# autonomousvision/LaRa

Hardware: AMD Instinct MI355X
Metric: novel-view frames/sec @512x512 (4-view in, 2DGS fwd+bwd) (higher is better)
Workload: dtype f32 raster + bf16-MFMA/f32-accumulate encoder (+ bf16-autocast coarse decoder MLP, as the reference's bf16-mixed)

## Files before the change

### include/lara_featvol.h

```cpp
#ifndef LARA_FEATVOL_H
#define LARA_FEATVOL_H

#include <stdint.h>

#ifdef __cplusplus
extern "C" {
#endif

#define LARA_FEATVOL_VOLUME 0
#define LARA_FEATVOL_TOKENS 1
#define LARA_FEATVOL_MAX_C 1024
#define LARA_FEATVOL_MAX_HW 8192

typedef struct {
    int32_t B, V, C, E, h, w, R;
    int32_t img_w, img_h;
    float eps;
    int64_t x_stride[4];
} lara_featvol_dims;

int64_t lara_featvol_workspace_bytes(const lara_featvol_dims *d);

int lara_featvol_forward(const lara_featvol_dims *d, const float *img_feats, const float *rays, const float *w2cs, const float *ixts,
                         const float *grid, const float *ln_w, const float *ln_b, const float *mlp_w, const float *mlp_b,
                         const float *view_embed, int32_t layout, void *out, void *workspace, void *stream);

int lara_featvol_backward(const lara_featvol_dims *d, const float *img_feats, const float *rays, const float *w2cs, const float *ixts,
                          const float *grid, const float *ln_w, const float *ln_b, const float *mlp_w, const float *mlp_b,
                          const float *grad, int32_t grad_layout, float *dx, float *d_ln_w, float *d_ln_b, float *d_mlp_w,
                          float *d_mlp_b, float *d_view_embed, void *workspace, void *stream);

#ifdef __cplusplus
}
#endif
#endif
```

### include/lara_groupattn.h

```cpp
#ifndef LARA_GROUPATTN_H
#define LARA_GROUPATTN_H

#include <stdint.h>

#ifdef __cplusplus
extern "C" {
#endif

int64_t lara_groupattn_workspace_bytes(int32_t G);

int lara_groupattn_forward(int32_t G, int32_t cond_dim, const float *x, const uint16_t *cond_bf16,
                           const float *ln_weight, const float *ln_bias, float eps,
                           const uint16_t *wq, const uint16_t *wkv, const uint16_t *wo, float *y,
                           void *workspace, void *stream);


typedef struct lara_groupblock_weights {
    const float *ln1_w, *ln1_b;
    const uint16_t *wq, *wkv, *wo;
    const float *ln2_w, *ln2_b;
    const uint16_t *w1;
    const float *b1;
    const uint16_t *w2;
    const float *b2;
    const float *ln3_w, *ln3_b;
    const uint16_t *wconv;
    float eps;
} lara_groupblock_weights;

int64_t lara_groupblock_workspace_bytes(int32_t scenes, int32_t R);

int lara_groupblock_forward(int32_t scenes, int32_t R, int32_t cond_dim, float *x,
                            const uint16_t *cond_bf16, const lara_groupblock_weights *w,
                            void *workspace, void *stream);

int lara_voltrans_head_forward(int32_t scenes, int32_t R, const float *x, const float *ln_w,
                               const float *ln_b, float eps, const uint16_t *wdeconv,
                               const float *bias, int32_t Cout, float *out, void *workspace,
                               void *stream);

int lara_tokens_from_volume(int32_t scenes, int32_t R, int32_t C, const float *volume, float *tokens,
                            void *stream);
int lara_volume_from_tokens(int32_t scenes, int32_t R, int32_t C, const float *tokens, float *volume,
                            void *stream);

int lara_gemm_nt_bf16(int32_t M, int32_t N, int32_t K, const uint16_t *A, const uint16_t *W, void *C, int32_t c_fp32,
                      void *stream);

int lara_batched_transpose(int32_t batch, int32_t rows, int32_t cols, const float *src, void *dst, int32_t dst_bf16,
                           void *stream);


typedef struct lara_groupblock_weights_t {
    const uint16_t *wq_t;
    const uint16_t *wkv_t;
    const uint16_t *wo_t;
    const uint16_t *w1_t;
    const uint16_t *w2_t;
    const uint16_t *wconv_t;
} lara_groupblock_weights_t;

typedef struct lara_groupblock_grads {
    float *ln1_w, *ln1_b, *wq, *wkv, *wo, *ln2_w, *ln2_b, *w1, *b1, *w2, *b2, *ln3_w, *ln3_b, *wconv;
} lara_groupblock_grads;

int64_t lara_groupblock_backward_workspace_bytes(int32_t scenes, int32_t R);
int64_t lara_groupblock_save_bytes(int32_t scenes, int32_t R);

int lara_groupblock_forward_train(int32_t scenes, int32_t R, int32_t cond_dim, const float *x_in, float *x_out,
                                  const uint16_t *cond_bf16, const lara_groupblock_weights *w, void *saved,
                                  void *stream);

int lara_groupblock_backward(int32_t scenes, int32_t R, int32_t cond_dim, const float *x_in,
                             const uint16_t *cond_bf16, const lara_groupblock_weights *w,
                             const lara_groupblock_weights_t *wt, const void *saved, float *g, float *dcond,
                             const lara_groupblock_grads *dw, int32_t chained, uint16_t *dkv, int32_t lddkv,
                             void *workspace, void *stream);

int64_t lara_voltrans_head_backward_workspace_bytes(int32_t scenes, int32_t R, int32_t Cout);
int lara_voltrans_head_backward(int32_t scenes, int32_t R, const float *x, const float *ln_w, const float *ln_b,
                                float eps, const uint16_t *wdeconv_t, int32_t Cout, const float *dout, float *g,
                                float *d_ln_w, float *d_ln_b, float *d_wdeconv, float *d_bias8, void *workspace,
                                void *stream);

int lara_groupblock_save_offsets(int32_t scenes, int32_t R, int64_t *offsets, int32_t n);
int64_t lara_gemm_tn_workspace_bytes(void);
int lara_gemm_tn_bf16(int32_t M, int32_t N, int32_t Kc, const uint16_t *A, const uint16_t *B, float *dst,
                      void *workspace, void *stream);
int lara_layernorm256_backward(int32_t rows, const float *dy, const float *x, const float *gamma, float eps,
                               const float *skip, float *dx, float *dgamma, float *dbeta, void *workspace,
                               void *stream);
int lara_groupattn_core_backward(int32_t G, const uint16_t *q, const uint16_t *kv, const uint16_t *d_o, uint16_t *dq,
                                 uint16_t *dkv, void *stream);

#ifdef __cplusplus
}
#endif
#endif
```

### lara_amd/_native.py

```python
from __future__ import annotations

import contextlib
import ctypes
import os
import re

import torch

_HERE = os.path.dirname(os.path.abspath(__file__))
LIB_PATH = os.environ.get("LARA2DGS_LIB") or os.path.join(_HERE, "liblara2dgs.so")
ABI_VERSION = 10

_vp, _i32, _i64, _f32 = ctypes.c_void_p, ctypes.c_int32, ctypes.c_int64, ctypes.c_float


def _struct(name, *groups):
    return type(name, (ctypes.Structure,), {"_fields_": [(n, t) for t, names in groups for n in names.split()]})


_BLOCK_FIELDS = "ln1_w ln1_b wq wkv wo ln2_w ln2_b w1 b1 w2 b2 ln3_w ln3_b wconv"

View = _struct("View", (_i32, "P sh_degree sh_coeffs image_height image_width"), (_f32, "tanfovx tanfovy scale_modifier"),
               (_i32, "prefiltered debug forward_only"), (_i64, "capacity"), (_vp, "bg viewmatrix projmatrix campos counts_out"))
StateLayout = _struct("StateLayout", (_i64, "header geom cullbox point_list ranges tile_order pair_base pair_pos final_T n_contrib "
                                            "seg_base seg_cnt bwd_order bwd_items ckpt pair_mask tile_maxc seg_cost total"))
Subset = _struct("Subset", (_vp, "coarse_state"), (_i64, "coarse_state_stride coarse_capacity"),
                 (_i32, "coarse_P coarse_forward_only"), (_vp, "inv"))
GradLayout = _struct("GradLayout", (_i64, "means3D means2D shs colors opacities scales rotations transmat total"))
FeatvolDims = _struct("FeatvolDims", (_i32, "B V C E h w R img_w img_h"), (_f32, "eps"), (_i64 * 4, "x_stride"))
BlockWeights = _struct("BlockWeights", (_vp, _BLOCK_FIELDS), (_f32, "eps"))
BlockWeightsT = _struct("BlockWeightsT", (_vp, "wq_t wkv_t wo_t w1_t w2_t wconv_t"))
BlockGrads = _struct("BlockGrads", (_vp, _BLOCK_FIELDS))
ImageView = _struct("ImageView", (_vp, "p"), (_i64, "sN sC sY sV sX"), (_i32, "Wv"))
LPIPS_MAX_LAYERS, LPIPS_TAPS = 16, 5
LpipsLayer = _struct("LpipsLayer", (_vp, "w bias"), (_i32, "cin cout k stride pad pool_k pool_s tap"))
LpipsNet = _struct("LpipsNet", (_i32, "n_layers"), (LpipsLayer * LPIPS_MAX_LAYERS, "layers"), (_vp * LPIPS_TAPS, "lin"),
                   (_f32 * 3, "shift"), (_f32 * 3, "scale"))
RowsItem = _struct("RowsItem", (_vp, "src dst"), (_i32, "width"))
VitDims = _struct("VitDims", (_i32, "N views H W C heads F depth"), (_f32, "eps"), (_i64 * 5, "img_stride"))

STRUCTS = {"lara2dgs_view": View, "lara2dgs_state_layout": StateLayout, "lara2dgs_subset": Subset,
           "lara2dgs_grad_layout": GradLayout, "lara_featvol_dims": FeatvolDims, "lara_groupblock_weights": BlockWeights,
           "lara_groupblock_weights_t": BlockWeightsT, "lara_groupblock_grads": BlockGrads, "lara_image_view": ImageView,
           "lara_lpips_layer": LpipsLayer, "lara_lpips_net": LpipsNet, "lara_rows_item": RowsItem, "lara_vit_dims": VitDims}

SIGNATURES = """
# include/lara2dgs.h
i lara2dgs_abi_version()
z lara2dgs_error_string(i)
i lara2dgs_last_hip_error()
l lara2dgs_state_bytes(i*3 l i)
l lara2dgs_scratch_bytes(i*3 l i)
i lara2dgs_get_state_layout(i*3 l i StateLayout)
i lara2dgs_forward(View p*12 s)
i lara2dgs_backward(View p*19 s)
i lara2dgs_forward_views(i View p*11 l p l s)
i lara2dgs_forward_views_subset(i View p*11 l p l Subset s)
i lara2dgs_get_grad_layout(i*6 GradLayout)
i lara2dgs_backward_views(i View p*10 l p l p s)
i lara2dgs_mark_visible(i p*4 s)
i lara2dgs_profile_enable(i)
i lara2dgs_selftest(i p p s)
i lara2dgs_profile_collect(p i p i)
# include/lara_batchfinish.h
i lara_batch_finish(p*4 l*4 p*3 s)
i lara_batch_finish_host(p*4 l*4 p*3)
# include/lara_coarsedec.h
l lara_coarse_decoder_padded_rows(l)
i lara_coarse_decoder_forward(i*3 p*7 f f p*5 s)
i lara_coarse_decoder_backward(i*3 p*19 s)
# include/lara_depthsurface.h
l lara_depthsurface_backproject_workspace_bytes(i*3)
i lara_depthsurface_backproject_count(i*3 p p i i f p p s)
i lara_depthsurface_backproject_emit(i*3 p p i i f p p i p f p*4 s)
l lara_depthsurface_thin_workspace_bytes(i i)
i lara_depthsurface_thin(i p p f i p*5 s)
i lara_depthsurface_observe(i p i*3 p p i f p p f i p s)
l lara_depthsurface_reduce_workspace_bytes(i)
i lara_depthsurface_reduce(i i p*5 i p*3 s)
# include/lara_eval.h
l lara_eval_workspace_doubles(i*6)
i lara_eval_scores(i*3 ImageView ImageView p i*3 p*3 i i p*3 s)
i lara_eval_quantize_frames(i*3 l l p*5 s)
# include/lara_featvol.h
l lara_featvol_workspace_bytes(FeatvolDims)
i lara_featvol_forward(FeatvolDims p*10 i p p s)
i lara_featvol_backward(FeatvolDims p*10 i p*7 s)
# include/lara_finedec.h
i lara_fine_decoder_forward(i p*8 s)
i lara_fine_decoder_backward(i p*14 s)
i lara_fine_wgrad_floats()
l lara_fine_wgrad_workspace_bytes(i)
i lara_fine_decoder_wgrad(i p*8 s)
i lara_fine_ln_blocks(i)
i lara_fine_ln_forward(i p*3 f p p s)
i lara_fine_ln_backward(i p*6 s)
# include/lara_groupattn.h
l lara_groupattn_workspace_bytes(i)
i lara_groupattn_forward(i i p*4 f p*5 s)
l lara_groupblock_workspace_bytes(i i)
i lara_groupblock_forward(i*3 p p BlockWeights p s)
i lara_voltrans_head_forward(i i p*3 f p p i p p s)
i lara_tokens_from_volume(i*3 p p s)
i lara_volume_from_tokens(i*3 p p s)
i lara_gemm_nt_bf16(i*3 p*3 i s)
i lara_batched_transpose(i*3 p p i s)
l lara_groupblock_backward_workspace_bytes(i i)
l lara_groupblock_save_bytes(i i)
i lara_groupblock_forward_train(i*3 p*3 BlockWeights p s)
i lara_groupblock_backward(i*3 p p BlockWeights BlockWeightsT p*3 BlockGrads i p i p s)
l lara_voltrans_head_backward_workspace_bytes(i*3)
i lara_voltrans_head_backward(i i p*3 f p i p*7 s)
i lara_groupblock_save_offsets(i i p i)
# ... 314 lines not shown
```

### lara_amd/csrc/attention.hip

```cpp
#include "mfma_gemm.h"
#include "group_attn.h"
#include "../../include/lara_groupattn.h"

extern "C" {

int64_t lara_groupattn_workspace_bytes(int32_t G) {
    if (G < 0) return LARA2DGS_E_INVALID;
    return (int64_t)G * (8 * 256 * 3 + 4 * 512) * 2 + 1024 + 262144;
}

int lara_groupattn_forward(int32_t G, int32_t cond_dim, const float *x, const uint16_t *cond_bf16,
                           const float *ln_weight, const float *ln_bias, float eps,
                           const uint16_t *wq, const uint16_t *wkv, const uint16_t *wo, float *y,
                           void *workspace, void *stream) {
    if (G < 0 || cond_dim <= 0 || (cond_dim % 32) != 0) return LARA2DGS_E_INVALID;
    if (G == 0) return LARA2DGS_OK;
    if (!x || !cond_bf16 || !ln_weight || !ln_bias || !wq || !wkv || !wo || !y || !workspace)
        return LARA2DGS_E_INVALID;
    hipStream_t s = (hipStream_t)stream;
    unsigned short *kvf = (unsigned short *)((char *)workspace + 262144) + (size_t)G * 8 * 256 * 2;
    {
        L2D_PROF("ga_gemm_kv", s);
        GemmP p{};
        p.A = cond_bf16; p.W = wkv; p.C = kvf; p.M = G * 4; p.N = 512; p.K = cond_dim;
        L2D_HIP(launch_gemm_ring<0, 0>(p, s));
    }
    {
        L2D_PROF("ga_fused", s);
        const int units = (G + 3) / 4;
        unsigned short *wqp = (unsigned short *)workspace, *wop = wqp + 65536;
        L2D_LAUNCH_IN_SCOPE(s, pack_weight_frag_kernel, dim3(64), dim3(256), 0, wq, wqp, wo, wop);
        L2D_LAUNCH_IN_SCOPE(s, group_attn_fused2_kernel<false>, dim3(units), dim3(64), 0, x, ln_weight, ln_bias, eps, wqp, kvf, wop, y, G,
                            (unsigned short *)nullptr, (unsigned short *)nullptr, (unsigned short *)nullptr);
    }
    return LARA2DGS_OK;
}

}
```

### lara_amd/csrc/encoder.hip

```cpp
#include <cstdlib>

#include "mfma_gemm.h"
#include "mlp_fused.h"
#include "../../include/lara_groupattn.h"

namespace {

__global__ void __launch_bounds__(256)
tokens_volume_kernel(const int R, const int C, const float *__restrict__ src, float *__restrict__ dst,
                     const int M, const int to_tokens) {
    const size_t i = (size_t)blockIdx.x * 256 + threadIdx.x;
    if (i >= (size_t)M * C) return;
    const int m = (int)(i / C), c = (int)(i - (size_t)m * C);
    int b, d, h, w;
    token_to_voxel(m, R, b, d, h, w);
    const size_t v = ((((size_t)b * C + c) * R + d) * R + h) * R + w;
    if (to_tokens) dst[i] = src[v];
    else dst[v] = src[i];
}

template <bool BF16>
__global__ void __launch_bounds__(256)
batched_transpose_kernel(const float *__restrict__ src, void *__restrict__ dst, const int rows, const int cols) {
    __shared__ float t[64][65];
    const int tx = threadIdx.x & 63, ty = threadIdx.x >> 6;
    const int c0 = blockIdx.x * 64, r0 = blockIdx.y * 64;
    const size_t base = (size_t)blockIdx.z * rows * cols;
#pragma unroll 4
    for (int k = 0; k < 16; k++) {
        const int r = r0 + ty * 16 + k, c = c0 + tx;
        t[ty * 16 + k][tx] = (r < rows && c < cols) ? src[base + (size_t)r * cols + c] : 0.f;
    }
    __syncthreads();
#pragma unroll 4
    for (int k = 0; k < 16; k++) {
        const int c = c0 + ty * 16 + k, r = r0 + tx;
        if (c < cols && r < rows) {
            const float v = t[tx][ty * 16 + k];
            if (BF16) ((unsigned short *)dst)[base + (size_t)c * rows + r] = f2bf(v);
            else ((float *)dst)[base + (size_t)c * rows + r] = v;
        }
    }
}

}

extern "C" {

int lara_batched_transpose(int32_t batch, int32_t rows, int32_t cols, const float *src, void *dst, int32_t dst_bf16,
                           void *stream) {
    if (batch < 0 || rows < 0 || cols < 0 || batch > 65535 || (rows + 63) / 64 > 65535) return LARA2DGS_E_INVALID;
    if (batch == 0 || rows == 0 || cols == 0) return LARA2DGS_OK;
    if (!src || !dst) return LARA2DGS_E_INVALID;
    const dim3 grid((cols + 63) / 64, (rows + 63) / 64, batch);
    if (dst_bf16) L2D_LAUNCH_IN_SCOPE((hipStream_t)stream, batched_transpose_kernel<true>, grid, dim3(256), 0, src, dst, rows, cols);
    else L2D_LAUNCH_IN_SCOPE((hipStream_t)stream, batched_transpose_kernel<false>, grid, dim3(256), 0, src, dst, rows, cols);
    return LARA2DGS_OK;
}

int64_t lara_groupblock_workspace_bytes(int32_t scenes, int32_t R) {
    if (scenes < 0 || R <= 0 || (R & 1)) return LARA2DGS_E_INVALID;
    const int64_t M = (int64_t)scenes * R * R * R;
    return M * 256 * 2 * 4 + M * 8 + 512 + 1024 + 262144;
}

int lara_groupblock_forward(int32_t scenes, int32_t R, int32_t cond_dim, float *x,
                            const uint16_t *cond_bf16, const lara_groupblock_weights *w,
                            void *workspace, void *stream) {
    if (scenes < 0 || R <= 0 || (R & 1) || cond_dim <= 0 || (cond_dim % 32) != 0 || !w) return LARA2DGS_E_INVALID;
    if (scenes == 0) return LARA2DGS_OK;
    if (!x || !cond_bf16 || !workspace || !w->ln1_w || !w->ln1_b || !w->wq || !w->wkv || !w->wo || !w->ln2_w ||
        !w->ln2_b || !w->w1 || !w->b1 || !w->w2 || !w->b2 || !w->ln3_w || !w->ln3_b || !w->wconv)
        return LARA2DGS_E_INVALID;
    const int64_t M64 = (int64_t)scenes * R * R * R;
    if (M64 * 2056 + 512 >= (1ll << 32)) return LARA2DGS_E_INVALID;
    const int M = (int)M64, G = M / 8;
    hipStream_t s = (hipStream_t)stream;
    int rc = lara_groupattn_forward(G, cond_dim, x, cond_bf16, w->ln1_w, w->ln1_b, w->eps, w->wq, w->wkv, w->wo,
                                    x, workspace, stream);
    if (rc) return rc;
    unsigned short *xn = (unsigned short *)workspace;
    float2 *stats = (float2 *)((char *)workspace + (size_t)M * 256 * 2 * 4);
    char *zero_row = (char *)xn + (size_t)M * 512;
    {
        L2D_PROF("gb_mlp_fused", s);
        MlpP p{};
        p.x1 = x; p.x2 = x; p.ln2_w = w->ln2_w; p.ln2_b = w->ln2_b; p.b1 = w->b1; p.b2 = w->b2; p.ln3_w = w->ln3_w; p.ln3_b = w->ln3_b;
        p.w1 = w->w1; p.w2 = w->w2; p.xn3 = xn; p.stats = stats; p.eps = w->eps; p.M = M;
        L2D_HIP(launch_mlp_fused<0>(p, s));
    }
    {
        L2D_PROF("gb_conv3d", s);
        GemmP p{};
        p.A = xn; p.W = w->wconv; p.C = x; p.resid = x; p.M = M; p.N = 256; p.K = 27 * 256;
        p.R = R; p.Cin = 256; p.stats = stats; p.gamma = w->ln3_w; p.beta = w->ln3_b;
        p.zero_off = (uint32_t)(zero_row - (char *)xn);
        L2D_HIP(launch_gemm_ring<1, 4>(p, s));
    }
    return LARA2DGS_OK;
}

int lara_voltrans_head_forward(int32_t scenes, int32_t R, const float *x, const float *ln_w,
                               const float *ln_b, float eps, const uint16_t *wdeconv,
                               const float *bias, int32_t Cout, float *out, void *workspace,
                               void *stream) {
    if (scenes < 0 || R <= 0 || (R & 1) || Cout <= 0 || (Cout & 3)) return LARA2DGS_E_INVALID;
    if (scenes == 0) return LARA2DGS_OK;
    if (!x || !ln_w || !ln_b || !wdeconv || !bias || !out || !workspace) return LARA2DGS_E_INVALID;
    const int M = scenes * R * R * R;
    hipStream_t s = (hipStream_t)stream;
    unsigned short *xn = (unsigned short *)workspace;
    L2D_LAUNCH("vt_ln", s, ln_cast_kernel, dim3((M + 3) / 4), dim3(256), 0, x, ln_w, ln_b, eps, xn,
               (float2 *)nullptr, M);
    {
        L2D_PROF("vt_deconv", s);
        GemmP p{};
        p.A = xn; p.W = wdeconv; p.C = out; p.bias = bias; p.M = M; p.N = 8 * Cout; p.K = 256;
        p.R = R; p.Cout = Cout;
        L2D_LAUNCH_IN_SCOPE(s, (gemm_bf16_nt_kernel<0, 5>), dim3((M + 127) / 128, (8 * Cout + 127) / 128), dim3(256), 0, p);
    }
    return LARA2DGS_OK;
}

static int tokens_volume(int32_t scenes, int32_t R, int32_t C, const float *src, float *dst, void *stream,
                         int to_tokens) {
    if (scenes < 0 || R <= 0 || (R & 1) || C <= 0) return LARA2DGS_E_INVALID;
    if (scenes == 0) return LARA2DGS_OK;
    if (!src || !dst) return LARA2DGS_E_INVALID;
    const int M = scenes * R * R * R;
    const size_t n = (size_t)M * C;
    L2D_LAUNCH_IN_SCOPE((hipStream_t)stream, tokens_volume_kernel, dim3((unsigned)((n + 255) / 256)), dim3(256), 0, R, C,
                        src, dst, M, to_tokens);
    return LARA2DGS_OK;
}

int lara_tokens_from_volume(int32_t scenes, int32_t R, int32_t C, const float *volume, float *tokens,
                            void *stream) {
    return tokens_volume(scenes, R, C, volume, tokens, stream, 1);
}

int lara_volume_from_tokens(int32_t scenes, int32_t R, int32_t C, const float *tokens, float *volume,
                            void *stream) {
    return tokens_volume(scenes, R, C, tokens, volume, stream, 0);
}

}
```

### lara_amd/csrc/encoder_bwd.hip

```cpp
#include <cstdlib>

#include "mfma_gemm.h"
#include "mlp_fused.h"
#include "group_attn.h"
#include "../../include/lara_groupattn.h"

namespace {

struct TnP {
    const unsigned short *A, *B;
    float *part;
    const int *nbr;
    int M, lda, ldb, N, Kc, T, chunk, tiles;
};
constexpr int TN_GROUP_MAX = 6;
struct TnGroup {
    TnP p[TN_GROUP_MAX];
    int first_slot[TN_GROUP_MAX + 1];
    int count;
};

__device__ __forceinline__ bf16x8 pack_lo(const uint32_t *w) {
    union { uint32_t u[4]; bf16x8 v; } r;
#pragma unroll
// ... 660 lines not shown
        for (int o = 32; o > 0; o >>= 1) s += __shfl_xor(s, o, 64);
        const float mean = s * (1.0f / 256.0f);
        const float c0 = v.x - mean, c1 = v.y - mean, c2 = v.z - mean, c3 = v.w - mean;
        float q = c0 * c0 + c1 * c1 + c2 * c2 + c3 * c3;
#pragma unroll
        for (int o = 32; o > 0; o >>= 1) q += __shfl_xor(q, o, 64);
        const float rstd = 1.0f / sqrtf(q * (1.0f / 256.0f) + eps);
        const float h0 = c0 * rstd, h1 = c1 * rstd, h2 = c2 * rstd, h3 = c3 * rstd;
        const float a0 = d.x * g.x, a1 = d.y * g.y, a2 = d.z * g.z, a3 = d.w * g.w;
        float sa = a0 + a1 + a2 + a3, sh = a0 * h0 + a1 * h1 + a2 * h2 + a3 * h3;
#pragma unroll
        for (int o = 32; o > 0; o >>= 1) { sa += __shfl_xor(sa, o, 64); sh += __shfl_xor(sh, o, 64); }
        sa *= (1.0f / 256.0f); sh *= (1.0f / 256.0f);
        const float4 r = make_float4(rstd * (a0 - sa - h0 * sh) + k.x, rstd * (a1 - sa - h1 * sh) + k.y,
                                     rstd * (a2 - sa - h2 * sh) + k.z, rstd * (a3 - sa - h3 * sh) + k.w);
        ((float4 *)(dx_out + (size_t)tok * 256))[lane] = r;
        if (dx_bf16) {
            ushort4 hb;
            hb.x = f2bf(r.x); hb.y = f2bf(r.y); hb.z = f2bf(r.z); hb.w = f2bf(r.w);
            ((ushort4 *)(dx_bf16 + (size_t)tok * 256))[lane] = hb;
        }
        pg[0] += d.x * h0; pg[1] += d.y * h1; pg[2] += d.z * h2; pg[3] += d.w * h3;
        pb[0] += d.x; pb[1] += d.y; pb[2] += d.z; pb[3] += d.w;
        po[0] += r.x; po[1] += r.y; po[2] += r.z; po[3] += r.w;
    }
#pragma unroll
    for (int c = 0; c < 4; c++) { red[wave][c][lane] = pg[c]; red[wave][4 + c][lane] = pb[c]; red[wave][8 + c][lane] = po[c]; }
    __syncthreads();
    if (wave == 0) {
#pragma unroll
        for (int k = 0; k < 12; k++) {
            const float t = (red[0][k][lane] + red[1][k][lane]) + (red[2][k][lane] + red[3][k][lane]);
            part[(size_t)blockIdx.x * 768 + (k >> 2) * 256 + 4 * lane + (k & 3)] = t;
        }
    }
}

__global__ void __launch_bounds__(256)
colsum_bf16_kernel(const unsigned short *__restrict__ src, float *__restrict__ part, const int rows, const int C) {
    const int r0 = blockIdx.x * 64, r1 = min(rows, r0 + 64);
    for (int c2 = threadIdx.x; c2 < C / 2; c2 += 256) {
        float s0 = 0.f, s1 = 0.f;
        for (int rr = r0; rr < r1; rr++) {
            const uint32_t w = *(const uint32_t *)(src + (size_t)rr * C + 2 * c2);
            s0 += __uint_as_float(w << 16);
            s1 += __uint_as_float(w & 0xffff0000u);
        }
        part[(size_t)blockIdx.x * C + 2 * c2] = s0;
        part[(size_t)blockIdx.x * C + 2 * c2 + 1] = s1;
    }
}

__global__ void __launch_bounds__(256)
cast_bf16_kernel(const float *__restrict__ src, unsigned short *__restrict__ dst, const size_t n4) {
    const size_t i = (size_t)blockIdx.x * 256 + threadIdx.x;
    if (i >= n4) return;
    const float4 v = ((const float4 *)src)[i];
    ushort4 h;
    h.x = f2bf(v.x); h.y = f2bf(v.y); h.z = f2bf(v.z); h.w = f2bf(v.w);
    ((ushort4 *)dst)[i] = h;
}

__global__ void __launch_bounds__(256)
deconv_grad_gather_kernel(const float *__restrict__ dout, unsigned short *__restrict__ dog, const int M, const int R,
                          const int Cout) {
    const int c4n = 2 * Cout;
    const size_t i = (size_t)blockIdx.x * 256 + threadIdx.x;
    if (i >= (size_t)M * c4n) return;
    const int m = (int)(i / c4n), c = (int)(i - (size_t)m * c4n) * 4;
    const int tap = c / Cout, co = c - tap * Cout;
    int b, d, h, w;
    token_to_voxel(m, R, b, d, h, w);
    const size_t R2 = 2 * (size_t)R;
    const size_t o = ((((size_t)b * R2 + 2 * d + (tap >> 2)) * R2 + 2 * h + ((tap >> 1) & 1)) * R2 + 2 * w + (tap & 1)) * Cout + co;
    const float4 v = *(const float4 *)(dout + o);
    ushort4 hb;
    hb.x = f2bf(v.x); hb.y = f2bf(v.y); hb.z = f2bf(v.z); hb.w = f2bf(v.w);
    *(ushort4 *)(dog + (size_t)m * 8 * Cout + c) = hb;
}

__global__ void __launch_bounds__(256)
group_attn_bwd_kernel(const unsigned short *__restrict__ Q, const unsigned short *__restrict__ KV,
                      const unsigned short *__restrict__ dO, unsigned short *__restrict__ dQ,
                      unsigned short *__restrict__ dKV, const int G, const int lddkv ) {
    __shared__ __attribute__((aligned(16))) unsigned short s_q[2][8 * 256], s_do[2][8 * 256], s_kv[2][4 * 512], s_dq[2][8 * 256];
    __shared__ float s_p[2][16 * 8 * 4], s_ds[2][16 * 8 * 4];
    const int gl = threadIdx.x >> 7, t = threadIdx.x & 127;
    const int g = blockIdx.x * 2 + gl;
    const bool active = g < G;
    if (active) {
        const uint4 *gq = (const uint4 *)(Q + (size_t)g * 8 * 256), *gd = (const uint4 *)(dO + (size_t)g * 8 * 256);
        const uint4 *gk = (const uint4 *)(KV + (size_t)g * 4 * 512);
        ((uint4 *)s_q[gl])[t] = gq[t]; ((uint4 *)s_q[gl])[t + 128] = gq[t + 128];
        ((uint4 *)s_do[gl])[t] = gd[t]; ((uint4 *)s_do[gl])[t + 128] = gd[t + 128];
        ((uint4 *)s_kv[gl])[t] = gk[t]; ((uint4 *)s_kv[gl])[t + 128] = gk[t + 128];
    }
    __syncthreads();
    if (active) {
        const int h = t >> 3, i = t & 7;
        float qv[16], dv[16];
#pragma unroll
        for (int d = 0; d < 16; d++) { qv[d] = bf2f(s_q[gl][i * 256 + h * 16 + d]); dv[d] = bf2f(s_do[gl][i * 256 + h * 16 + d]); }
        float sc[4], dp[4];
#pragma unroll
        for (int j = 0; j < 4; j++) {
            float a = 0.f, b = 0.f;
#pragma unroll
            for (int d = 0; d < 16; d++) {
                a += qv[d] * bf2f(s_kv[gl][j * 512 + h * 16 + d]);
                b += dv[d] * bf2f(s_kv[gl][j * 512 + 256 + h * 16 + d]);
            }
            sc[j] = a * 0.25f; dp[j] = b;
        }
        const float mx = fmaxf(fmaxf(sc[0], sc[1]), fmaxf(sc[2], sc[3]));
        float pr[4], sum = 0.f;
#pragma unroll
        for (int j = 0; j < 4; j++) { pr[j] = __expf(sc[j] - mx); sum += pr[j]; }
        const float inv = 1.0f / sum;
        float dot = 0.f;
#pragma unroll
        for (int j = 0; j < 4; j++) { pr[j] *= inv; dot += pr[j] * dp[j]; }
        float ds[4];
#pragma unroll
        for (int j = 0; j < 4; j++) {
            ds[j] = pr[j] * (dp[j] - dot) * 0.25f;
            s_p[gl][(h * 8 + i) * 4 + j] = pr[j];
            s_ds[gl][(h * 8 + i) * 4 + j] = ds[j];
        }
#pragma unroll
        for (int d = 0; d < 16; d++) {
            float a = 0.f;
#pragma unroll
            for (int j = 0; j < 4; j++) a += ds[j] * bf2f(s_kv[gl][j * 512 + h * 16 + d]);
            s_dq[gl][i * 256 + h * 16 + d] = f2bf(a);
        }
    }
    __syncthreads();
    float dk[8], dvv[8];
    const int h2 = t >> 3, j2 = (t >> 1) & 3, d0 = (t & 1) * 8;
    if (active) {
#pragma unroll
        for (int d = 0; d < 8; d++) { dk[d] = 0.f; dvv[d] = 0.f; }
#pragma unroll
        for (int i = 0; i < 8; i++) {
            const float dsv = s_ds[gl][(h2 * 8 + i) * 4 + j2], pv = s_p[gl][(h2 * 8 + i) * 4 + j2];
#pragma unroll
            for (int d = 0; d < 8; d++) {
                dk[d] += dsv * bf2f(s_q[gl][i * 256 + h2 * 16 + d0 + d]);
                dvv[d] += pv * bf2f(s_do[gl][i * 256 + h2 * 16 + d0 + d]);
            }
        }
    }
    __syncthreads();
    if (active) {
#pragma unroll
        for (int d = 0; d < 8; d++) {
            s_kv[gl][j2 * 512 + h2 * 16 + d0 + d] = f2bf(dk[d]);
            s_kv[gl][j2 * 512 + 256 + h2 * 16 + d0 + d] = f2bf(dvv[d]);
        }
    }
    __syncthreads();
    if (active) {
        uint4 *oq = (uint4 *)(dQ + (size_t)g * 8 * 256);
        unsigned short *ok = dKV + ((size_t)g * 4 + (t >> 6)) * lddkv + (t & 63) * 8;
        oq[t] = ((const uint4 *)s_dq[gl])[t]; oq[t + 128] = ((const uint4 *)s_dq[gl])[t + 128];
        *(uint4 *)ok = ((const uint4 *)s_kv[gl])[t]; *(uint4 *)(ok + 2 * (size_t)lddkv) = ((const uint4 *)s_kv[gl])[t + 128];
    }
}

constexpr size_t TN_PART_BYTES = 128ull << 20;

inline int cu_count() {
    static const int cus = [] {
        int dev = 0, v = 0;
        if (hipGetDevice(&dev) != hipSuccess || hipDeviceGetAttribute(&v, hipDeviceAttributeMultiprocessorCount, dev) != hipSuccess) v = 0;
        return v > 0 ? v : 256;
    }();
    return cus;
// ... 131 lines not shown
    AccGroup a{};
    g.count = a.count = count;
    size_t off_f = 0;
    for (;;) {
        off_f = 0;
        int slot = 0, wg = 0;
        for (int k = 0; k < count; k++) {
            const TnJob &j = jobs[k];
            int splits = base;
            while (splits > 8 && j.M / splits < 256) splits -= 8;
            const int tiles = ((j.N + 127) / 128) * ((j.Kc + 127) / 128), n = j.N * j.Kc;
            TnP &p = g.p[k];
            p.A = j.A; p.B = j.B; p.part = part + off_f; p.nbr = nullptr; p.M = j.M; p.lda = j.lda; p.ldb = j.ldb; p.N = j.N; p.Kc = j.Kc;
            p.T = 1; p.chunk = (((j.M + splits - 1) / splits) + 63) & ~63; p.tiles = tiles;
            g.first_slot[k] = slot;
            slot += tiles * splits / 8;
            a.dst[k] = j.dst; a.part[k] = part + off_f; a.n[k] = n; a.parts[k] = splits; a.first_wg[k] = wg;
            wg += (n / 4 + 63) / 64;
            off_f += (size_t)splits * n;
        }
        g.first_slot[count] = slot;
        a.first_wg[count] = wg;
        if (off_f * 4 <= TN_PART_BYTES || base == 8) break;
        base -= 8;
    }
    if (off_f * 4 > TN_PART_BYTES) return LARA2DGS_E_INVALID;
    L2D_LAUNCH_IN_SCOPE(s, (gemm_bf16_tn_lds_kernel<false>), dim3(g.first_slot[count] * 8), dim3(256), 0, g);
    L2D_LAUNCH_IN_SCOPE(s, accum_partials4_group_kernel, dim3(a.first_wg[count]), dim3(256), 0, a);
    return LARA2DGS_OK;
}

struct RedList {
    RedGroup g{};
    int wgs = 0;
    bool overflow = false;
    void add(float *dst, const float *part, int n, int parts, int stride) {
        if (!dst) return;
        if (g.count >= RED_GROUP_MAX) { overflow = true; return; }
        const int k = g.count++;
        g.dst[k] = dst; g.part[k] = part; g.n[k] = n; g.parts[k] = parts; g.stride[k] = stride; g.first_wg[k] = wgs;
        wgs += (n + 63) / 64;
        g.first_wg[g.count] = wgs;
    }
    int launch(hipStream_t s) {
        if (overflow) return LARA2DGS_E_INVALID;
        if (g.count) L2D_LAUNCH_IN_SCOPE(s, reduce_group_kernel, dim3(wgs), dim3(1024), 0, g);
        g.count = 0; wgs = 0;
        return LARA2DGS_OK;
    }
};

int ln_bwd(const void *dy, bool dy_bf16, const float *x, const float *gamma, float eps, const float *skip, float *dx,
           unsigned short *dx_bf16, float *dgamma, float *dbeta, float *part, int M, hipStream_t s, RedList *later = nullptr) {
    const int blocks = (M + LNB_ROWS - 1) / LNB_ROWS;
    if (dy_bf16) L2D_LAUNCH_IN_SCOPE(s, ln_bwd_kernel<true>, dim3(blocks), dim3(256), 0, dy, x, gamma, eps, skip, dx, dx_bf16, part, M);
    else L2D_LAUNCH_IN_SCOPE(s, ln_bwd_kernel<false>, dim3(blocks), dim3(256), 0, dy, x, gamma, eps, skip, dx, dx_bf16, part, M);
    if (later) {
        later->add(dgamma, part, 256, blocks, 768);
        later->add(dbeta, part + 256, 256, blocks, 768);
    } else {
        L2D_LAUNCH_IN_SCOPE(s, accum_ln_partials_kernel, dim3(4, 3), dim3(1024), 0, dgamma, dbeta, (float *)nullptr, part, blocks);
    }
    return LARA2DGS_OK;
}

int colsum_bf16(const unsigned short *src, int rows, int C, float *dst, float *part, hipStream_t s) {
    const int blocks = (rows + 63) / 64;
    L2D_LAUNCH_IN_SCOPE(s, colsum_bf16_kernel, dim3(blocks), dim3(256), 0, src, part, rows, C);
    L2D_LAUNCH_IN_SCOPE(s, accum_partials_kernel, dim3((C + 63) / 64), dim3(1024), 0, dst, part, C, blocks, (size_t)C);
    return LARA2DGS_OK;
}

template <int EPI>
int gemm_nt(const unsigned short *A, const unsigned short *W, void *C, int M, int N, int K, const float *resid, hipStream_t s) {
    GemmP p{};
    p.A = A; p.W = W; p.C = C; p.resid = resid; p.M = M; p.N = N; p.K = K;
    L2D_LAUNCH_IN_SCOPE(s, (gemm_bf16_nt_kernel<0, EPI>), dim3((M + 127) / 128, (N + 127) / 128), dim3(256), 0, p);
    return LARA2DGS_OK;
}

struct SaveWs {
    size_t xn1, q, kv, o, x1, xn2, z, h, x2, xn3, stats, wpack, total;
};
SaveWs save_layout(int64_t M) {
    SaveWs w{};
    size_t o = 0;
    auto take = [&](size_t bytes) { const size_t at = o; o = up256(o + bytes); return at; };
    const size_t b256 = (size_t)M * 512, f256 = (size_t)M * 1024, b512 = (size_t)M * 1024;
    w.xn1 = take(b256); w.q = take(b256); w.kv = take(b256); w.o = take(b256);
    w.x1 = take(f256); w.xn2 = take(b256); w.z = take(b512); w.h = take(b512); w.x2 = take(f256);
    w.xn3 = take(b256 + 512);
    w.stats = take((size_t)M * 8);
    w.wpack = take(2 * 256 * 256 * 2);
    w.total = o;
    return w;
}
struct BwdWs {
    size_t gb, tmpf, dzb, dq, dkv, dob, nbr, tnpart, save, gb3, gb2, lnpart4, total;
};
BwdWs bwd_layout(int64_t M) {
    BwdWs w{};
    size_t o = 0;
    auto take = [&](size_t bytes) { const size_t at = o; o = up256(o + bytes); return at; };
    const size_t b256 = (size_t)M * 512, f256 = (size_t)M * 1024, b512 = (size_t)M * 1024;
    w.gb = take(b256 + 512);
    w.tmpf = take(f256); w.dzb = take(b512); w.dq = take(b256); w.dkv = take(b256); w.dob = take(b256);
    w.nbr = take((size_t)27 * M * 4);
    take(((size_t)(M + 63) / 64) * 768 * 4);
    w.tnpart = take(TN_PART_BYTES);
    w.save = take(save_layout(M).total);
    w.gb3 = take(b256); w.gb2 = take(b256);
    w.lnpart4 = take(4 * ((size_t)(M + LNB_ROWS - 1) / LNB_ROWS) * 768 * 4);
    w.total = o;
    return w;
}

int block_forward_keep(int M, int cond_dim, const float *x_in, const unsigned short *cond_bf16,
                       const lara_groupblock_weights *w, char *save, hipStream_t s) {
    const SaveWs L = save_layout(M);
    const int G = M / 8, Mkv = G * 4;
    unsigned short *xn1 = (unsigned short *)(save + L.xn1), *q = (unsigned short *)(save + L.q), *kv = (unsigned short *)(save + L.kv);
    unsigned short *o = (unsigned short *)(save + L.o), *xn2 = (unsigned short *)(save + L.xn2), *z = (unsigned short *)(save + L.z);
    unsigned short *h = (unsigned short *)(save + L.h), *xn3 = (unsigned short *)(save + L.xn3);
    float *x1 = (float *)(save + L.x1), *x2 = (float *)(save + L.x2);
    {
        GemmP p{};
        p.A = cond_bf16; p.W = w->wkv; p.C = kv; p.M = Mkv; p.N = 512; p.K = cond_dim;
        L2D_HIP(launch_gemm_ring<0, 0>(p, s));
    }
    {
        unsigned short *wqp = (unsigned short *)(save + L.wpack), *wop = wqp + 65536;
        L2D_LAUNCH_IN_SCOPE(s, pack_weight_frag_kernel, dim3(64), dim3(256), 0, w->wq, wqp, w->wo, wop);
        L2D_LAUNCH_IN_SCOPE(s, group_attn_fused2_kernel<true>, dim3((G + 3) / 4), dim3(64), 0, x_in, w->ln1_w, w->ln1_b, w->eps, wqp, kv, wop,
                            x1, G, xn1, q, o);
    }
    {
        MlpP p{};
        p.x1 = x1; p.x2 = x2; p.ln2_w = w->ln2_w; p.ln2_b = w->ln2_b; p.b1 = w->b1; p.b2 = w->b2; p.ln3_w = w->ln3_w; p.ln3_b = w->ln3_b;
        p.w1 = w->w1; p.w2 = w->w2; p.xn3 = xn3; p.stats = (float2 *)(save + L.stats); p.xn2 = xn2; p.z = z; p.h = h; p.eps = w->eps; p.M = M;
        L2D_HIP(launch_mlp_fused<1>(p, s));
    }
    return LARA2DGS_OK;
}

bool block_weights_ok(const lara_groupblock_weights *w) {
    return w && w->ln1_w && w->ln1_b && w->wq && w->wkv && w->wo && w->ln2_w && w->ln2_b && w->w1 && w->b1 && w->w2 &&
           w->b2 && w->ln3_w && w->ln3_b && w->wconv;
}

}

extern "C" {

int64_t lara_groupblock_backward_workspace_bytes(int32_t scenes, int32_t R) {
    if (scenes < 0 || R < 4 || (R & 1)) return LARA2DGS_E_INVALID;
    return (int64_t)bwd_layout((int64_t)scenes * R * R * R).total;
}

int64_t lara_groupblock_save_bytes(int32_t scenes, int32_t R) {
    if (scenes < 0 || R < 4 || (R & 1)) return LARA2DGS_E_INVALID;
    return (int64_t)save_layout((int64_t)scenes * R * R * R).total;
}

int lara_groupblock_save_offsets(int32_t scenes, int32_t R, int64_t *offsets, int32_t n) {
    if (scenes < 0 || R < 4 || (R & 1) || !offsets || n != 11) return LARA2DGS_E_INVALID;
    const SaveWs L = save_layout((int64_t)scenes * R * R * R);
    const size_t at[11] = {L.xn1, L.q, L.kv, L.o, L.x1, L.xn2, L.z, L.h, L.x2, L.xn3, L.stats};
    for (int i = 0; i < 11; i++) offsets[i] = (int64_t)at[i];
    return LARA2DGS_OK;
}

int lara_groupblock_forward_train(int32_t scenes, int32_t R, int32_t cond_dim, const float *x_in, float *x_out,
                                  const uint16_t *cond_bf16, const lara_groupblock_weights *w, void *saved,
                                  void *stream) {
    if (scenes < 0 || R < 4 || (R & 1) || cond_dim <= 0 || (cond_dim % 32) != 0 || !block_weights_ok(w)) return LARA2DGS_E_INVALID;
    if (scenes == 0) return LARA2DGS_OK;
    if (!x_in || !x_out || x_in == x_out || !cond_bf16 || !saved) return LARA2DGS_E_INVALID;
    const int64_t M64 = (int64_t)scenes * R * R * R;
    if (M64 * 2056 + 512 >= (1ll << 32)) return LARA2DGS_E_INVALID;
    const int M = (int)M64;
    hipStream_t s = (hipStream_t)stream;
    const SaveWs L = save_layout(M);
    char *save = (char *)saved;
    {
        L2D_PROF("gbt_forward", s);
        L2D_TRY(block_forward_keep(M, cond_dim, x_in, cond_bf16, w, save, s));
    }
    {
        L2D_PROF("gb_conv3d", s);
        GemmP p{};
        p.A = (const unsigned short *)(save + L.xn3); p.W = w->wconv; p.C = x_out; p.resid = (const float *)(save + L.x2);
        p.M = M; p.N = 256; p.K = 27 * 256; p.R = R; p.Cin = 256; p.stats = (const float2 *)(save + L.stats);
        p.gamma = w->ln3_w; p.beta = w->ln3_b; p.zero_off = (uint32_t)((size_t)M * 512);
        L2D_HIP(launch_gemm_ring<1, 4>(p, s));
    }
    return LARA2DGS_OK;
}

int lara_groupblock_backward(int32_t scenes, int32_t R, int32_t cond_dim, const float *x_in,
                             const uint16_t *cond_bf16, const lara_groupblock_weights *w,
                             const lara_groupblock_weights_t *wt, const void *saved, float *g, float *dcond,
                             const lara_groupblock_grads *dw, int32_t chained, uint16_t *dkv_ext, int32_t lddkv,
                             void *workspace, void *stream) {
    if (scenes < 0 || R < 4 || (R & 1) || cond_dim <= 0 || (cond_dim % 32) != 0 || !block_weights_ok(w) || !wt || !dw)
        return LARA2DGS_E_INVALID;
    if (scenes == 0) return LARA2DGS_OK;
    if (!x_in || !cond_bf16 || !g || (!dcond && !dkv_ext) || !workspace) return LARA2DGS_E_INVALID;
    if (dkv_ext && (lddkv < 512 || (lddkv & 7))) return LARA2DGS_E_INVALID;
    constexpr int CONV_CIN = 256, CONV_K = 27 * CONV_CIN;
    static_assert(CONV_K % 128 == 0 && CONV_CIN % 128 == 0, "gemm_ring2_kernel's shapes (launch_gemm_ring has nothing else for a convolution)");
    if (!wt->wq_t || !wt->wkv_t || !wt->wo_t || !wt->w1_t || !wt->w2_t ||
        !wt->wconv_t || !dw->ln1_w || !dw->ln1_b || !dw->wq || !dw->wkv || !dw->wo || !dw->ln2_w || !dw->ln2_b ||
        !dw->w1 || !dw->b1 || !dw->w2 || !dw->b2 || !dw->ln3_w || !dw->ln3_b || !dw->wconv)
        return LARA2DGS_E_INVALID;
    const int64_t M64 = (int64_t)scenes * R * R * R;
    if (M64 * 2056 + 512 >= (1ll << 32)) return LARA2DGS_E_INVALID;
    const int M = (int)M64, G = M / 8, Mkv = G * 4;
    hipStream_t s = (hipStream_t)stream;
    const BwdWs L = bwd_layout(M);
    const SaveWs S = save_layout(M);
    char *ws = (char *)workspace;
    if (!saved) {
        L2D_PROF("gbb_recompute", s);
        L2D_TRY(block_forward_keep(M, cond_dim, x_in, cond_bf16, w, ws + L.save, s));
    }
    const char *sv = saved ? (const char *)saved : ws + L.save;
    const unsigned short *xn1 = (const unsigned short *)(sv + S.xn1), *q = (const unsigned short *)(sv + S.q);
    const unsigned short *kv = (const unsigned short *)(sv + S.kv), *o = (const unsigned short *)(sv + S.o);
    const unsigned short *xn2 = (const unsigned short *)(sv + S.xn2), *h = (const unsigned short *)(sv + S.h);
    const unsigned short *xn3 = (const unsigned short *)(sv + S.xn3);
    unsigned short *z = (unsigned short *)(sv + S.z);
    const float *x1 = (const float *)(sv + S.x1), *x2 = (const float *)(sv + S.x2);
    unsigned short *gb = (unsigned short *)(ws + L.gb);
    unsigned short *gb3 = (unsigned short *)(ws + L.gb3), *gb2 = (unsigned short *)(ws + L.gb2);
    unsigned short *dzb = (unsigned short *)(ws + L.dzb), *dq = (unsigned short *)(ws + L.dq);
    unsigned short *dkv = dkv_ext ? dkv_ext : (unsigned short *)(ws + L.dkv);
    const int ld_dkv = dkv_ext ? lddkv : 512;
    unsigned short *dob = (unsigned short *)(ws + L.dob);
    unsigned short *tmpb = (unsigned short *)(ws + L.tmpf);
    float *tnpart = (float *)(ws + L.tnpart);
    const size_t lnset = ((size_t)(M + LNB_ROWS - 1) / LNB_ROWS) * 768;
    float *lnp4 = (float *)(ws + L.lnpart4);
    RedList red;
    int *nbr = (int *)(ws + L.nbr);
    if (!chained) {
        L2D_HIP(hipMemsetAsync(gb + (size_t)M * 256, 0, 512, s));
        L2D_LAUNCH_IN_SCOPE(s, neighbour_table_kernel, dim3((M + 255) / 256), dim3(256), 0, nbr, M, R, M, 512);
        L2D_LAUNCH_IN_SCOPE(s, cast_bf16_kernel, dim3((unsigned)(((size_t)M * 64 + 255) / 256)), dim3(256), 0, g, gb, (size_t)M * 64);
    }
    {
        L2D_PROF("gbb_dw_conv", s);
        L2D_TRY(gemm_tn(gb, 256, 256, xn3, 256, 256, 27, nbr, M, dw->wconv, tnpart, s));
    }
    {
        L2D_PROF("gbb_dx_conv", s);
        GemmP p{};
        p.A = gb; p.W = wt->wconv_t; p.C = g; p.resid = g; p.M = M; p.N = 256; p.K = CONV_K;
        p.R = R; p.Cin = CONV_CIN; p.zero_off = (uint32_t)((size_t)M * 512);
        p.C2 = gb3; p.lnx = x2; p.stats = (const float2 *)(sv + S.stats); p.gamma = w->ln3_w; p.colsum = lnp4;
        L2D_HIP(launch_gemm_ring<1, 9>(p, s));
        const int tiles = (M + RT - 1) / RT;
        red.add(dw->ln3_w, lnp4, 256, tiles, 768);
        red.add(dw->ln3_b, lnp4 + 256, 256, tiles, 768);
        red.add(dw->b2, lnp4 + 512, 256, tiles, 768);
    }
    {
        L2D_PROF("gbb_dx_mlp", s);
        MlpP p{};
        p.gin = gb3; p.w1 = wt->w2_t; p.w2 = wt->w1_t; p.z = z; p.h = dzb; p.gout = tmpb; p.part_b1 = lnp4 + lnset; p.M = M;
        L2D_HIP(launch_mlp_fused<3>(p, s));
        red.add(dw->b1, lnp4 + lnset, 512, (M + 127) / 128, 512);
    }
    {
        L2D_PROF("gbb_ln_bwd", s);
        L2D_TRY(ln_bwd(tmpb, true, x1, w->ln2_w, w->eps, g, g, gb2, dw->ln2_w, dw->ln2_b, lnp4 + 2 * lnset, M, s, &red));
    }
    {
        L2D_PROF("gbb_dx_attn", s);
        L2D_TRY(gemm_nt<0>(gb2, wt->wo_t, dob, M, 256, 256, nullptr, s));
        L2D_LAUNCH_IN_SCOPE(s, group_attn_bwd_kernel, dim3((G + 1) / 2), dim3(256), 0, q, kv, dob, dq, dkv, G, ld_dkv);
        if (!dkv_ext) L2D_TRY(gemm_nt<1>(dkv, wt->wkv_t, dcond, Mkv, cond_dim, 512, dcond, s));
        L2D_TRY(gemm_nt<0>(dq, wt->wq_t, tmpb, M, 256, 256, nullptr, s));
    }
    {
        L2D_PROF("gbb_ln_bwd", s);
        L2D_TRY(ln_bwd(tmpb, true, x_in, w->ln1_w, w->eps, g, g, gb, dw->ln1_w, dw->ln1_b, lnp4 + 3 * lnset, M, s, &red));
        L2D_TRY(red.launch(s));
    }
    {
        L2D_PROF("gbb_dw_linear", s);
        const TnJob jobs[5] = {{gb3, 256, 256, h, 512, 512, M, dw->w2},
                               {dzb, 512, 512, xn2, 256, 256, M, dw->w1},
                               {gb2, 256, 256, o, 256, 256, M, dw->wo},
                               {dq, 256, 256, xn1, 256, 256, M, dw->wq},
                               {dkv, ld_dkv, 512, cond_bf16, cond_dim, cond_dim, Mkv, dw->wkv}};
        L2D_TRY(gemm_tn_group(jobs, 5, tnpart, s));
    }
    return LARA2DGS_OK;
}

int64_t lara_voltrans_head_backward_workspace_bytes(int32_t scenes, int32_t R, int32_t Cout) {
    if (scenes < 0 || R < 4 || (R & 1) || Cout <= 0 || (Cout & 15)) return LARA2DGS_E_INVALID;
    const size_t M = (size_t)scenes * R * R * R;
    return (int64_t)(up256(M * 512) + up256(M * 16 * Cout) + up256(M * 1024) + up256(((M + 63) / 64) * 4 * (size_t)max(768, 8 * Cout)) +
                     TN_PART_BYTES);
}

int lara_voltrans_head_backward(int32_t scenes, int32_t R, const float *x, const float *ln_w, const float *ln_b,
                                float eps, const uint16_t *wdeconv_t, int32_t Cout, const float *dout, float *g,
                                float *d_ln_w, float *d_ln_b, float *d_wdeconv, float *d_bias8, void *workspace,
                                void *stream) {
    if (scenes < 0 || R < 4 || (R & 1) || Cout <= 0 || (Cout & 15)) return LARA2DGS_E_INVALID;
    if (scenes == 0) return LARA2DGS_OK;
    if (!x || !ln_w || !ln_b || !wdeconv_t || !dout || !g || !d_ln_w || !d_ln_b || !d_wdeconv || !d_bias8 || !workspace)
        return LARA2DGS_E_INVALID;
    const int M = scenes * R * R * R, N8 = 8 * Cout;
    hipStream_t s = (hipStream_t)stream;
    char *ws = (char *)workspace;
    size_t off = 0;
    unsigned short *xn = (unsigned short *)(ws + off); off += up256((size_t)M * 512);
    unsigned short *dog = (unsigned short *)(ws + off); off += up256((size_t)M * 16 * Cout);
    float *tmpf = (float *)(ws + off); off += up256((size_t)M * 1024);
    float *lnpart = (float *)(ws + off); off += up256(((size_t)(M + 63) / 64) * 4 * (size_t)max(768, N8));
    float *tnpart = (float *)(ws + off);
    L2D_PROF("vtb_head", s);
    L2D_LAUNCH_IN_SCOPE(s, ln_cast_kernel, dim3((M + 3) / 4), dim3(256), 0, x, ln_w, ln_b, eps, xn, (float2 *)nullptr, M);
    {
        const size_t n = (size_t)M * 2 * Cout;
        L2D_LAUNCH_IN_SCOPE(s, deconv_grad_gather_kernel, dim3((unsigned)((n + 255) / 256)), dim3(256), 0, dout, dog, M, R, Cout);
    }
    L2D_TRY(colsum_bf16(dog, M, N8, d_bias8, lnpart, s));
    L2D_TRY(gemm_tn(dog, N8, N8, xn, 256, 256, 1, nullptr, M, d_wdeconv, tnpart, s));
    L2D_TRY(gemm_nt<0>(dog, wdeconv_t, tmpf, M, 256, N8, nullptr, s));
    L2D_TRY(ln_bwd(tmpf, true, x, ln_w, eps, nullptr, g, nullptr, d_ln_w, d_ln_b, lnpart, M, s));
    return LARA2DGS_OK;
}


int lara_gemm_nt_bf16(int32_t M, int32_t N, int32_t K, const uint16_t *A, const uint16_t *W, void *C, int32_t c_fp32,
                      void *stream) {
    if (M < 0 || N < 0 || K <= 0 || (K & 31)) return LARA2DGS_E_INVALID;
    if (M == 0 || N == 0) return LARA2DGS_OK;
    if (!A || !W || !C) return LARA2DGS_E_INVALID;
    if ((size_t)M * K * 2 >= (1ull << 32) || (size_t)N * K * 2 >= (1ull << 32)) return LARA2DGS_E_INVALID;
    GemmP p{};
    p.A = A; p.W = W; p.C = C; p.M = M; p.N = N; p.K = K;
    L2D_HIP(c_fp32 ? launch_gemm_ring<0, 8>(p, (hipStream_t)stream) : launch_gemm_ring<0, 0>(p, (hipStream_t)stream));
    return LARA2DGS_OK;
}

int lara_gemm_tn_bf16(int32_t M, int32_t N, int32_t Kc, const uint16_t *A, const uint16_t *B, float *dst,
                      void *workspace, void *stream) {
    if (M <= 0 || (M & 15) || N <= 0 || Kc <= 0 || !A || !B || !dst || !workspace) return LARA2DGS_E_INVALID;
    return gemm_tn(A, N, N, B, Kc, Kc, 1, nullptr, M, dst, (float *)workspace, (hipStream_t)stream);
}

int64_t lara_gemm_tn_workspace_bytes(void) { return (int64_t)TN_PART_BYTES; }

int lara_layernorm256_backward(int32_t rows, const float *dy, const float *x, const float *gamma, float eps,
                               const float *skip, float *dx, float *dgamma, float *dbeta, void *workspace,
                               void *stream) {
    if (rows <= 0 || !dy || !x || !gamma || !dx || !dgamma || !dbeta || !workspace) return LARA2DGS_E_INVALID;
    return ln_bwd(dy, false, x, gamma, eps, skip, dx, nullptr, dgamma, dbeta, (float *)workspace, rows, (hipStream_t)stream);
}

int lara_groupattn_core_backward(int32_t G, const uint16_t *q, const uint16_t *kv, const uint16_t *d_o, uint16_t *dq,
                                 uint16_t *dkv, void *stream) {
    if (G < 0) return LARA2DGS_E_INVALID;
    if (G == 0) return LARA2DGS_OK;
    if (!q || !kv || !d_o || !dq || !dkv) return LARA2DGS_E_INVALID;
    L2D_LAUNCH_IN_SCOPE((hipStream_t)stream, group_attn_bwd_kernel, dim3((G + 1) / 2), dim3(256), 0, q, kv, d_o, dq, dkv, G, 512);
    return LARA2DGS_OK;
}

}
```

### lara_amd/csrc/featvol.hip

```cpp
#include "common.h"
#include "mfma_gemm.h"
#include "../../include/lara_featvol.h"
#include "../../include/lara_groupattn.h"

namespace {

constexpr int FV_PTS = 32;
constexpr int FV_KA = 64;
constexpr int FV_TOK_BLOCKS = 1024;
constexpr int FV_EMB_BLOCKS = 64;

struct FvP {
    int B, V, C, E, h, w, R, S, hw, T, Tp;
    float img_w, img_h, eps;
    long long sx0, sx1, sx2, sx3;
    const float *x, *rays, *w2cs, *ixts, *grid, *ln_w, *ln_b, *mlp_w, *mlp_b, *embed;
};

__device__ __forceinline__ void rsh3(const float x, const float y, const float z, float *o) {
    const float x2 = x * x, y2 = y * y, z2 = z * z, xy = x * y, xz = x * z, yz = y * z;
    o[0] = 0.282094791773878f;
    o[1] = -0.48860251190292f * y;
    o[2] = 0.48860251190292f * z;
    o[3] = -0.48860251190292f * x;
// ... 69 lines not shown
    float s = 0.f;
#pragma unroll
    for (int q = 0; q < 4; q++)
#pragma unroll
        for (int i = 0; i < 4; i++) s += x[q][i];
    mean = wave_sum(s) / (float)p.C;
    float v = 0.f;
#pragma unroll
    for (int q = 0; q < 4; q++)
        if (4 * lane + 256 * q < p.C)
#pragma unroll
            for (int i = 0; i < 4; i++) v += (x[q][i] - mean) * (x[q][i] - mean);
    rstd = 1.f / sqrtf(wave_sum(v) / (float)p.C + p.eps);
}

__device__ __forceinline__ void load_mod(const FvP &p, const unsigned short *__restrict__ mod, const int t, const int lane,
                                         float (&sh)[4][4], float (&opm)[4][4]) {
    const unsigned short *row = mod + (size_t)t * 2 * p.C;
#pragma unroll
    for (int q = 0; q < 4; q++) {
        const int c = 4 * lane + 256 * q;
        if (c < p.C) {
            const s16x4 a = *(const s16x4 *)(row + c), b = *(const s16x4 *)(row + p.C + c);
#pragma unroll
            for (int i = 0; i < 4; i++) {
                sh[q][i] = bf2f((unsigned short)a[i]);
                opm[q][i] = bf2f(f2bf(1.f + bf2f((unsigned short)b[i])));
            }
        } else {
#pragma unroll
            for (int i = 0; i < 4; i++) sh[q][i] = opm[q][i] = 0.f;
        }
    }
}

template <bool CL>
__global__ void __launch_bounds__(256) modln_kernel(const FvP p, const unsigned short *__restrict__ mod, float *__restrict__ y) {
    const int lane = threadIdx.x & 63, t = blockIdx.x * 4 + (threadIdx.x >> 6);
    if (t >= p.T) return;
    float x[4][4], sh[4][4], opm[4][4], mean, rstd;
    load_x<CL>(p, t, lane, x);
    ln_stats(p, lane, x, mean, rstd);
    load_mod(p, mod, t, lane, sh, opm);
#pragma unroll
    for (int q = 0; q < 4; q++) {
        const int c = 4 * lane + 256 * q;
        if (c >= p.C) continue;
        float o[4];
#pragma unroll
        for (int i = 0; i < 4; i++) {
            const float n = (x[q][i] - mean) * rstd * p.ln_w[c + i] + p.ln_b[c + i];
            o[i] = n * opm[q][i] + sh[q][i];
        }
        *(float4 *)(y + (size_t)t * p.C + c) = make_float4(o[0], o[1], o[2], o[3]);
    }
}

__device__ __forceinline__ void map_pos(const FvP &p, const int bv, const int s, float &ix, float &iy) {
    const float *g = p.grid + (size_t)s * 3, *m = p.w2cs + (size_t)bv * 16, *k = p.ixts + (size_t)bv * 9;
    const float px = bfr(g[0]), py = bfr(g[1]), pz = bfr(g[2]);
    const float cx = bfr(px * bfr(m[0]) + py * bfr(m[1]) + pz * bfr(m[2])) + m[3];
    const float cy = bfr(px * bfr(m[4]) + py * bfr(m[5]) + pz * bfr(m[6])) + m[7];
    const float cz = bfr(px * bfr(m[8]) + py * bfr(m[9]) + pz * bfr(m[10])) + m[11];
    const float bx = bfr(cx), by = bfr(cy), bz = bfr(cz);
    const float qx = bfr(bx * bfr(k[0]) + by * bfr(k[1]) + bz * bfr(k[2]));
    const float qy = bfr(bx * bfr(k[3]) + by * bfr(k[4]) + bz * bfr(k[5]));
    const float qz = bfr(bx * bfr(k[6]) + by * bfr(k[7]) + bz * bfr(k[8]));
    const float gx = bfr(bfr(bfr(bfr(qx / qz) + 0.5f) / p.img_w) * 2.f) - 1.f, gy = bfr(bfr(bfr(bfr(qy / qz) + 0.5f) / p.img_h) * 2.f) - 1.f;
    ix = ((bfr(gx) + 1.f) * (float)p.w - 1.f) / 2.f;
    iy = ((bfr(gy) + 1.f) * (float)p.h - 1.f) / 2.f;
}

__device__ __forceinline__ int tap(const FvP &p, const float ix, const float iy, const int k, float &wgt) {
    const float fx = floorf(ix), fy = floorf(iy);
    if (!(fx >= -2.f && fx <= (float)p.w + 1.f && fy >= -2.f && fy <= (float)p.h + 1.f)) { wgt = 0.f; return -1; }
    const int xi = (int)fx + (k & 1), yi = (int)fy + (k >> 1);
    const float x1 = fx + 1.f, y1 = fy + 1.f;
    const float wx = (k & 1) ? ix - fx : x1 - ix, wy = (k >> 1) ? iy - fy : y1 - iy;
    wgt = wx * wy;
    return (xi >= 0 && xi < p.w && yi >= 0 && yi < p.h) ? yi * p.w + xi : -1;
}

template <bool TOKENS>
__global__ void __launch_bounds__(256) sample_kernel(const FvP p, const float *__restrict__ y, void *__restrict__ out) {
    __shared__ int s_idx[8][FV_PTS][4];
    __shared__ float s_wgt[8][FV_PTS][4];
    __shared__ float s_tile[TOKENS ? 1 : 256][FV_PTS + 1];
    const int lane = threadIdx.x & 63, wave = threadIdx.x >> 6, b = blockIdx.y, s0 = blockIdx.x * FV_PTS;
    const int npts = min(FV_PTS, p.S - s0), CE = p.C + p.E;
    for (int i = threadIdx.x; i < p.V * FV_PTS; i += 256) {
        const int v = i / FV_PTS, pt = i - v * FV_PTS;
        float ix = 0.f, iy = 0.f;
        if (pt < npts) map_pos(p, b * p.V + v, s0 + pt, ix, iy);
#pragma unroll
        for (int k = 0; k < 4; k++) {
            float wg = 0.f;
            const int id = pt < npts ? tap(p, ix, iy, k, wg) : -1;
            s_idx[v][pt][k] = id;
            s_wgt[v][pt][k] = wg;
        }
    }
    __syncthreads();
    for (int v = 0; v < p.V; v++) {
        const float *yv = y + (size_t)(b * p.V + v) * p.hw * p.C;
        for (int q = 0; 256 * q < p.C; q++) {
            const int c = 4 * lane + 256 * q;
            for (int pt = wave; pt < FV_PTS; pt += 4) {
                if (pt >= npts || c >= p.C) continue;
                float4 a = make_float4(0.f, 0.f, 0.f, 0.f);
#pragma unroll
                for (int k = 0; k < 4; k++) {
                    const int id = s_idx[v][pt][k];
                    if (id < 0) continue;
                    const float wg = s_wgt[v][pt][k];
                    const float4 g = *(const float4 *)(yv + (size_t)id * p.C + c);
                    a.x += wg * g.x; a.y += wg * g.y; a.z += wg * g.z; a.w += wg * g.w;
                }
                if (TOKENS) {
                    unsigned short *o = (unsigned short *)out + ((size_t)(b * p.S + s0 + pt) * p.V + v) * CE + c;
                    *(uint2 *)o = make_uint2(f2bf2(a.x, a.y), f2bf2(a.z, a.w));
                } else {
                    const int cl = 4 * lane;
                    s_tile[cl][pt] = a.x; s_tile[cl + 1][pt] = a.y; s_tile[cl + 2][pt] = a.z; s_tile[cl + 3][pt] = a.w;
                }
            }
            if (!TOKENS) {
                __syncthreads();
                const int nc = min(256, p.C - 256 * q);
                float *o = (float *)out + ((size_t)(b * p.V + v) * CE + 256 * q) * p.S + s0;
                for (int r = threadIdx.x / FV_PTS; r < nc; r += 256 / FV_PTS) {
                    const int pt = threadIdx.x % FV_PTS;
                    if (pt < npts) o[(size_t)r * p.S + pt] = s_tile[r][pt];
                }
                __syncthreads();
            }
        }
        for (int i = threadIdx.x; i < p.E * FV_PTS; i += 256) {
            if (TOKENS) {
                const int pt = i / p.E, e = i - pt * p.E;
                if (pt < npts)
                    ((unsigned short *)out)[((size_t)(b * p.S + s0 + pt) * p.V + v) * CE + p.C + e] = f2bf(p.embed[v * p.E + e]);
            } else {
                const int e = i / FV_PTS, pt = i - e * FV_PTS;
                if (pt < npts) ((float *)out)[((size_t)(b * p.V + v) * CE + p.C + e) * p.S + s0 + pt] = p.embed[v * p.E + e];
            }
        }
    }
}

__device__ __attribute__((noinline)) int entry_key(const FvP &p, const int bv, const int e, float &wg) {
    float ix, iy;
    map_pos(p, bv, e >> 2, ix, iy);
    return tap(p, ix, iy, e & 3, wg);
}

__global__ void __launch_bounds__(256) index_kernel(const FvP p, int *__restrict__ bins_all, int2 *__restrict__ ents_all) {
    __shared__ int s_cnt[LARA_FEATVOL_MAX_HW + 1];
    const int bv = blockIdx.x, n = 4 * p.S, lane = threadIdx.x & 63, wave = threadIdx.x >> 6;
    int *bins = bins_all + (size_t)bv * (p.hw + 1);
    int2 *ents = ents_all + (size_t)bv * n;
    for (int i = threadIdx.x; i <= p.hw; i += 256) s_cnt[i] = 0;
    __syncthreads();
    for (int e = threadIdx.x; e < n; e += 256) {
        float wg;
        const int id = entry_key(p, bv, e, wg);
        if (id >= 0) atomicAdd(&s_cnt[id], 1);
    }
    __syncthreads();
    if (wave == 0) {
        int carry = 0;
        for (int base = 0; base < p.hw; base += 64) {
            const int i = base + lane;
            const int c = i < p.hw ? s_cnt[i] : 0;
            int inc = c;
#pragma unroll
            for (int o = 1; o < 64; o <<= 1) {
                const int u = __shfl_up(inc, o, 64);
                if (lane >= o) inc += u;
            }
            if (i < p.hw) { s_cnt[i] = carry + inc - c; bins[i] = carry + inc - c; }
            carry += __shfl(inc, 63, 64);
        }
        if (lane == 0) bins[p.hw] = carry;
        volatile int *cur = s_cnt;
        int nbits = 0;
        while ((1 << nbits) < p.hw) nbits++;
        const unsigned long long lt = (1ull << lane) - 1ull;
        for (int base = 0; base < n; base += 64) {
            const int e = base + lane;
            float wg = 0.f;
            int id = -1;
            if (e < n) id = entry_key(p, bv, e, wg);
            unsigned long long same = __ballot(id >= 0);
            for (int bt = 0; bt < nbits; bt++) {
                const unsigned long long on = __ballot(id >= 0 && ((id >> bt) & 1));
                same &= ((id >> bt) & 1) ? on : ~on;
            }
            int pos = 0;
            if (id >= 0) pos = cur[id] + __popcll(same & lt);
            __builtin_amdgcn_wave_barrier();
            if (id >= 0) {
                if (pos < n) ents[pos] = make_int2(e, __float_as_int(wg));
                if ((same >> lane) == 1ull) cur[id] = cur[id] + __popcll(same);
            }
            __builtin_amdgcn_wave_barrier();
        }
    }
}

template <bool CL>
__global__ void __launch_bounds__(256) token_bwd_kernel(const FvP p, const unsigned short *__restrict__ mod, const int *__restrict__ bins_all,
                                                        const int2 *__restrict__ ents_all, const float *__restrict__ g,
                                                        float *__restrict__ dx, unsigned short *__restrict__ dmod,
                                                        float *__restrict__ part) {
    __shared__ float s_part[2 * LARA_FEATVOL_MAX_C];
    const int lane = threadIdx.x & 63, wave = threadIdx.x >> 6;
    const int nw = gridDim.x * 4, CE = p.C + p.E;
    float pg[4][4], pb[4][4];
#pragma unroll
    for (int q = 0; q < 4; q++)
#pragma unroll
        for (int i = 0; i < 4; i++) pg[q][i] = pb[q][i] = 0.f;
    for (int t = blockIdx.x * 4 + wave; t < p.T; t += nw) {
        const int bv = t / p.hw, pix = t - bv * p.hw, b = bv / p.V, v = bv - b * p.V;
// ... 106 lines not shown
}

__global__ void __launch_bounds__(256) split_dw_kernel(const float *__restrict__ prod, const int rows, float *__restrict__ dw, float *__restrict__ db) {
    const int i = blockIdx.x * 256 + threadIdx.x;
    if (i >= rows * 33) return;
    const int r = i / 33, j = i - r * 33;
    if (j < 32) dw[(size_t)r * 32 + j] = prod[(size_t)r * FV_KA + j];
    else db[r] = prod[(size_t)r * FV_KA + 32];
}

struct FvWs { int64_t act, wk, mod, y, gt, bins, ents, dmod, part, epart, prod, tn, total; };

bool dims_ok(const lara_featvol_dims *d) {
    if (!d) return false;
    if (d->B <= 0 || d->V <= 0 || d->V > 8 || d->C < 64 || d->C > LARA_FEATVOL_MAX_C || (d->C % 64) || d->E < 0 || d->E > 256 || (d->E % 4))
        return false;
    if (d->h <= 0 || d->w <= 0 || (int64_t)d->h * d->w > LARA_FEATVOL_MAX_HW || d->R <= 0 || d->img_w <= 0 || d->img_h <= 0) return false;
    const int64_t S = (int64_t)d->R * d->R * d->R, T = (int64_t)d->B * d->V * d->h * d->w;
    if (S * 4 >= (1ll << 30) || T >= (1ll << 30) || d->B > 65535) return false;
    if ((T + 255) / 256 * 256 * 2 * d->C * 2 >= (1ll << 32)) return false;
    return true;
}

FvWs ws_layout(const lara_featvol_dims *d) {
    const int64_t S = (int64_t)d->R * d->R * d->R, hw = (int64_t)d->h * d->w, BV = (int64_t)d->B * d->V, T = BV * hw;
    const int64_t Tp = (T + 255) / 256 * 256, C = d->C, CE = d->C + d->E;
    FvWs L{};
    int64_t o = 0;
    L.act = o;  o = align_up(o + Tp * FV_KA * 2, 256);
    L.wk = o;   o = align_up(o + 2 * C * FV_KA * 2, 256);
    L.mod = o;  o = align_up(o + Tp * 2 * C * 2, 256);
    const int64_t shared0 = o;
    L.y = o;    o = align_up(o + T * C * 4, 256);
    const int64_t fwd_end = o;
    o = shared0;
    L.gt = o;   o = align_up(o + (int64_t)d->B * S * d->V * CE * 4, 256);
    L.bins = o; o = align_up(o + BV * (hw + 1) * 4, 256);
    L.ents = o; o = align_up(o + BV * 4 * S * 8, 256);
    L.dmod = o; o = align_up(o + Tp * 2 * C * 2, 256);
    L.part = o; o = align_up(o + (int64_t)FV_TOK_BLOCKS * 2 * C * 4, 256);
    L.epart = o; o = align_up(o + (int64_t)FV_EMB_BLOCKS * d->V * d->E * 4 + 4, 256);
    L.prod = o; o = align_up(o + 2 * C * FV_KA * 4, 256);
    L.tn = o;   o = align_up(o + lara_gemm_tn_workspace_bytes(), 256);
    L.total = o > fwd_end ? o : fwd_end;
    return L;
}

FvP make_params(const lara_featvol_dims *d, const float *x, const float *rays, const float *w2cs, const float *ixts, const float *grid,
                const float *ln_w, const float *ln_b, const float *mlp_w, const float *mlp_b, const float *embed) {
    FvP p{};
    p.B = d->B; p.V = d->V; p.C = d->C; p.E = d->E; p.h = d->h; p.w = d->w; p.R = d->R;
    p.S = d->R * d->R * d->R; p.hw = d->h * d->w; p.T = p.B * p.V * p.hw; p.Tp = (p.T + 255) / 256 * 256;
    p.img_w = (float)d->img_w; p.img_h = (float)d->img_h; p.eps = d->eps;
    p.sx0 = d->x_stride[0]; p.sx1 = d->x_stride[1]; p.sx2 = d->x_stride[2]; p.sx3 = d->x_stride[3];
    p.x = x; p.rays = rays; p.w2cs = w2cs; p.ixts = ixts; p.grid = grid; p.ln_w = ln_w; p.ln_b = ln_b; p.mlp_w = mlp_w; p.mlp_b = mlp_b;
    p.embed = embed;
    return p;
}

bool channels_last(const FvP &p, const void *x, const void *dx) {
    return p.sx1 == 1 && p.sx0 % 4 == 0 && p.sx2 % 4 == 0 && p.sx3 % 4 == 0 && ((uintptr_t)x & 15) == 0 && ((uintptr_t)dx & 15) == 0;
}

int linear_fwd(const FvP &p, char *ws, const FvWs &L, hipStream_t s) {
    unsigned short *act = (unsigned short *)(ws + L.act), *wk = (unsigned short *)(ws + L.wk);
    L2D_LAUNCH_IN_SCOPE(s, act_kernel, dim3((p.Tp + 255) / 256), dim3(256), 0, p, act);
    L2D_LAUNCH_IN_SCOPE(s, wprep_kernel, dim3((2 * p.C * FV_KA + 255) / 256), dim3(256), 0, p, wk);
    return lara_gemm_nt_bf16(p.Tp, 2 * p.C, FV_KA, act, wk, ws + L.mod, 0, s);
}

}

extern "C" {

int64_t lara_featvol_workspace_bytes(const lara_featvol_dims *d) {
    if (!dims_ok(d)) return LARA2DGS_E_INVALID;
    return ws_layout(d).total;
}

int lara_featvol_forward(const lara_featvol_dims *d, const float *img_feats, const float *rays, const float *w2cs, const float *ixts,
                         const float *grid, const float *ln_w, const float *ln_b, const float *mlp_w, const float *mlp_b,
                         const float *view_embed, int32_t layout, void *out, void *workspace, void *stream) {
    if (!dims_ok(d) || (layout != LARA_FEATVOL_VOLUME && layout != LARA_FEATVOL_TOKENS)) return LARA2DGS_E_INVALID;
    if (!img_feats || !rays || !w2cs || !ixts || !grid || !ln_w || !ln_b || !mlp_w || !mlp_b || !out || !workspace) return LARA2DGS_E_INVALID;
    if (d->E > 0 && !view_embed) return LARA2DGS_E_INVALID;
    hipStream_t s = (hipStream_t)stream;
    const FvP p = make_params(d, img_feats, rays, w2cs, ixts, grid, ln_w, ln_b, mlp_w, mlp_b, view_embed);
    const FvWs L = ws_layout(d);
    char *ws = (char *)workspace;
    float *y = (float *)(ws + L.y);
    int rc;
    {
        L2D_PROF("featvol_linear", s);
        if ((rc = linear_fwd(p, ws, L, s)) != LARA2DGS_OK) return rc;
    }
    {
        L2D_PROF("featvol_modln", s);
        const unsigned short *mod = (const unsigned short *)(ws + L.mod);
        if (channels_last(p, img_feats, img_feats)) L2D_LAUNCH_IN_SCOPE(s, modln_kernel<true>, dim3((p.T + 3) / 4), dim3(256), 0, p, mod, y);
        else L2D_LAUNCH_IN_SCOPE(s, modln_kernel<false>, dim3((p.T + 3) / 4), dim3(256), 0, p, mod, y);
    }
    {
        L2D_PROF(layout == LARA_FEATVOL_TOKENS ? "featvol_sample_tokens" : "featvol_sample_volume", s);
        const dim3 grid2((p.S + FV_PTS - 1) / FV_PTS, p.B);
        if (layout == LARA_FEATVOL_TOKENS) L2D_LAUNCH_IN_SCOPE(s, sample_kernel<true>, grid2, dim3(256), 0, p, (const float *)y, out);
        else L2D_LAUNCH_IN_SCOPE(s, sample_kernel<false>, grid2, dim3(256), 0, p, (const float *)y, out);
    }
    return LARA2DGS_OK;
}

int lara_featvol_backward(const lara_featvol_dims *d, const float *img_feats, const float *rays, const float *w2cs, const float *ixts,
                          const float *grid, const float *ln_w, const float *ln_b, const float *mlp_w, const float *mlp_b,
                          const float *grad, int32_t grad_layout, float *dx, float *d_ln_w, float *d_ln_b, float *d_mlp_w,
                          float *d_mlp_b, float *d_view_embed, void *workspace, void *stream) {
    if (!dims_ok(d) || (grad_layout != LARA_FEATVOL_VOLUME && grad_layout != LARA_FEATVOL_TOKENS)) return LARA2DGS_E_INVALID;
    if (!img_feats || !rays || !w2cs || !ixts || !grid || !ln_w || !ln_b || !mlp_w || !mlp_b || !grad || !dx || !d_ln_w || !d_ln_b ||
        !d_mlp_w || !d_mlp_b || !workspace)
        return LARA2DGS_E_INVALID;
    hipStream_t s = (hipStream_t)stream;
    const FvP p = make_params(d, img_feats, rays, w2cs, ixts, grid, ln_w, ln_b, mlp_w, mlp_b, nullptr);
    const FvWs L = ws_layout(d);
    char *ws = (char *)workspace;
    const int CE = p.C + p.E;
    int rc;
    const float *g = grad;
    if (grad_layout == LARA_FEATVOL_VOLUME) {
        L2D_PROF("featvol_grad_transpose", s);
        if ((rc = lara_batched_transpose(p.B, p.V * CE, p.S, grad, ws + L.gt, 0, s)) != LARA2DGS_OK) return rc;
        g = (const float *)(ws + L.gt);
    }
    {
        L2D_PROF("featvol_linear", s);
        if ((rc = linear_fwd(p, ws, L, s)) != LARA2DGS_OK) return rc;
    }
    int *bins = (int *)(ws + L.bins);
    int2 *ents = (int2 *)(ws + L.ents);
    L2D_LAUNCH("featvol_index", s, index_kernel, dim3(p.B * p.V), dim3(256), 0, p, bins, ents);
    unsigned short *dmod = (unsigned short *)(ws + L.dmod);
    float *part = (float *)(ws + L.part);
    const int nblk = min(FV_TOK_BLOCKS, (p.T + 3) / 4);
    {
        L2D_PROF("featvol_token_bwd", s);
        if (p.Tp > p.T) L2D_HIP(hipMemsetAsync(dmod + (size_t)p.T * 2 * p.C, 0, (size_t)(p.Tp - p.T) * 2 * p.C * 2, s));
        const unsigned short *mod = (const unsigned short *)(ws + L.mod);
        if (channels_last(p, img_feats, dx))
            L2D_LAUNCH_IN_SCOPE(s, token_bwd_kernel<true>, dim3(nblk), dim3(256), 0, p, mod, bins, ents, g, dx, dmod, part);
        else L2D_LAUNCH_IN_SCOPE(s, token_bwd_kernel<false>, dim3(nblk), dim3(256), 0, p, mod, bins, ents, g, dx, dmod, part);
    }
    {
        L2D_PROF("featvol_param_grads", s);
        L2D_LAUNCH_IN_SCOPE(s, sum_parts_kernel, dim3((2 * p.C + 255) / 256), dim3(256), 0, (const float *)part, nblk, 2 * p.C, d_ln_w,
                            d_ln_b, p.C);
        if (d_view_embed && p.E > 0) {
            float *ep = (float *)(ws + L.epart);
            L2D_LAUNCH_IN_SCOPE(s, embed_part_kernel, dim3(FV_EMB_BLOCKS), dim3(256), 0, p, g, ep);
            L2D_LAUNCH_IN_SCOPE(s, sum_parts_kernel, dim3((p.V * p.E + 255) / 256), dim3(256), 0, (const float *)ep, FV_EMB_BLOCKS,
                                p.V * p.E, d_view_embed, d_view_embed, p.V * p.E);
        }
        float *prod = (float *)(ws + L.prod);
        L2D_HIP(hipMemsetAsync(prod, 0, (size_t)2 * p.C * FV_KA * 4, s));
        if ((rc = lara_gemm_tn_bf16(p.Tp, 2 * p.C, FV_KA, dmod, (const uint16_t *)(ws + L.act), prod, ws + L.tn, s)) != LARA2DGS_OK)
            return rc;
        L2D_LAUNCH_IN_SCOPE(s, split_dw_kernel, dim3((2 * p.C * 33 + 255) / 256), dim3(256), 0, (const float *)prod, 2 * p.C, d_mlp_w, d_mlp_b);
    }
    return LARA2DGS_OK;
}

}
```

### lara_amd/csrc/group_attn.h

```cpp
#pragma once
#include "mfma_gemm.h"

namespace {


__device__ __forceinline__ float wave_total(float x) {
    x += dpp_move<0xB1, 0xf>(x);
    x += dpp_move<0x4E, 0xf>(x);
    x += dpp_move<0x141, 0xf>(x);
    x += dpp_move<0x140, 0xf>(x);
    x += dpp_move<0x142, 0xa>(x);
    x += dpp_move<0x143, 0xc>(x);
    return __int_as_float(__builtin_amdgcn_readlane(__float_as_int(x), 63));
}


__global__ void __launch_bounds__(256) pack_weight_frag_kernel(const unsigned short *__restrict__ W0, unsigned short *__restrict__ out0,
                                                               const unsigned short *__restrict__ W1, unsigned short *__restrict__ out1) {
    const bool second = blockIdx.x >= 32;
    const unsigned short *W = second ? W1 : W0;
    unsigned short *out = second ? out1 : out0;
    const int t = (blockIdx.x & 31) * 256 + threadIdx.x;
    const int lane = t & 63, ks = (t >> 6) & 15, nt = t >> 10;
    *(uint4 *)(out + (size_t)t * 8) = *(const uint4 *)(W + (size_t)(nt * 32 + (lane & 31)) * 256 + ks * 16 + 8 * (lane >> 5));
}

template <bool KEEP>
__global__ void __launch_bounds__(64)
group_attn_fused2_kernel(const float *x , const float *__restrict__ gamma,
                        const float *__restrict__ beta, const float eps, const unsigned short *__restrict__ Wq ,
                        const unsigned short *__restrict__ KV, const unsigned short *__restrict__ Wo , float *y, const int G,
                        unsigned short *__restrict__ xn_out, unsigned short *__restrict__ q_out, unsigned short *__restrict__ o_out) {
    constexpr int GA_LDS = 24576;
    __shared__ __attribute__((aligned(16))) unsigned char lds_all[GA_LDS];
    const int lane = threadIdx.x & 63;
    const int unit = blockIdx.x, g0 = unit * 4;
    if (g0 >= G) return;
    unsigned char *R = lds_all, *KVr = R + 16384;
    const int c16 = lane & 15, q4 = lane >> 4;
    const int q_rows = min(32, (G - g0) * 8), kv_rows = min(16, (G - g0) * 4);
    const int srow = lane >> 4, sphys = lane & 15;
    const size_t row0 = (size_t)g0 * 8;

    {
        const float4 gm = ((const float4 *)gamma)[lane], bt = ((const float4 *)beta)[lane];
        const int hh = lane >> 5, chunk = (lane & 31) >> 1, sub = (lane & 1) * 8;
#pragma unroll 1
        for (int rb = 0; rb < 32; rb += 16) {
            float4 v[16];
#pragma unroll
            for (int i = 0; i < 16; i++) v[i] = ((const float4 *)(x + (row0 + min(rb + i, q_rows - 1)) * 256))[lane];
#pragma unroll
            for (int i = 0; i < 16; i++) {
                const int r = rb + i;
                const float mean = wave_total((v[i].x + v[i].y) + (v[i].z + v[i].w)) * (1.0f / 256.0f);
                const float a = v[i].x - mean, b = v[i].y - mean, c = v[i].z - mean, d4 = v[i].w - mean;
                const float rstd = 1.0f / sqrtf(wave_total(a * a + b * b + c * c + d4 * d4) * (1.0f / 256.0f) + eps);
                *(uint2 *)(R + hh * 8192 + r * 256 + ((chunk ^ (r & 15)) << 4) + sub) =
                    make_uint2(f2bf2(a * rstd * gm.x + bt.x, b * rstd * gm.y + bt.y), f2bf2(c * rstd * gm.z + bt.z, d4 * rstd * gm.w + bt.w));
            }
        }
    }
    const int frow = lane & 31, fk = 8 * (lane >> 5);
    auto load_rows = [&](bf16x8 (&bf)[16]) {
#pragma unroll
        for (int ks = 0; ks < 16; ks++) {
            const int f = ks * 16 + fk;
            bf[ks] = *(const bf16x8 *)(R + (f >> 7) * 8192 + frow * 256 + ((((f & 127) >> 3) ^ (frow & 15)) << 4));
        }
    };
#pragma unroll
    for (int i = 0; i < 4; i++) {
        const int row = 4 * i + srow, chunk = sphys ^ (row & 15);
        const unsigned short *src = KV + (size_t)(g0 * 4 + min(row, kv_rows - 1)) * 512 + chunk * 8;
        __builtin_amdgcn_global_load_lds((const __attribute__((address_space(1))) void *)src,
                                         (__attribute__((address_space(3))) void *)(KVr + i * 1024), 16, 0, 0);
        __builtin_amdgcn_global_load_lds((const __attribute__((address_space(1))) void *)(src + 256),
                                         (__attribute__((address_space(3))) void *)(KVr + 4096 + i * 1024), 16, 0, 0);
    }
    auto store_rows = [&](unsigned short *dst) {
        asm volatile("s_waitcnt lgkmcnt(0)" ::: "memory");
#pragma unroll 4
        for (int i = 0; i < 16; i++) {
            const int r = 2 * i + (lane >> 5), c = lane & 31;
            const uint4 v = *(const uint4 *)(R + (c >> 4) * 8192 + r * 256 + (((c & 15) ^ (r & 15)) << 4));
            if (r < q_rows) *(uint4 *)(dst + (row0 + r) * 256 + c * 8) = v;
        }
    };
    bf16x8 bf[16], wf[16];
    load_rows(bf);
    if (KEEP) store_rows(xn_out);
#pragma unroll
    for (int ks = 0; ks < 16; ks++) wf[ks] = *(const bf16x8 *)(Wq + ((size_t)ks * 64 + lane) * 8);
#pragma unroll 1
    for (int nt = 0; nt < 8; nt++) {
        const unsigned short *wnext = Wq + ((size_t)min(nt + 1, 7) * 1024 + lane) * 8;
        bf16x8 wn[16];
#pragma unroll
        for (int ks = 0; ks < 16; ks++) wn[ks] = *(const bf16x8 *)(wnext + ks * 512);
        f32x16 acc;
#pragma unroll
        for (int i = 0; i < 16; i++) acc[i] = 0.f;
#pragma unroll
        for (int ks = 0; ks < 16; ks++) acc = __builtin_amdgcn_mfma_f32_32x32x16_bf16(wf[ks], bf[ks], acc, 0, 0, 0);
#pragma unroll
        for (int g = 0; g < 4; g++) {
            const int f = nt * 32 + 8 * g + 4 * (lane >> 5);
            *(uint2 *)(R + (f >> 7) * 8192 + frow * 256 + ((((f & 127) >> 3) ^ (frow & 15)) << 4) + ((f & 7) << 1)) =
                make_uint2(f2bf2(acc[4 * g], acc[4 * g + 1]), f2bf2(acc[4 * g + 2], acc[4 * g + 3]));
        }
#pragma unroll
        for (int ks = 0; ks < 16; ks++) wf[ks] = wn[ks];
    }
    if (KEEP) store_rows(q_out);
    asm volatile("s_waitcnt vmcnt(0)" ::: "memory");
    uint4 pk[4], pv[4];
#pragma unroll
    for (int i = 0; i < 4; i++) {
        const int row = 4 * i + srow, chunk = sphys ^ (row & 15);
        const unsigned short *src = KV + (size_t)(g0 * 4 + min(row, kv_rows - 1)) * 512 + 128 + chunk * 8;
        pk[i] = *(const uint4 *)src;
        pv[i] = *(const uint4 *)(src + 256);
    }
    for (int hh = 0; hh < 2; hh++) {
        unsigned char *Qr = R + hh * 8192, *Kr = KVr, *Vr = KVr + 4096;
        asm volatile("s_waitcnt lgkmcnt(0)" ::: "memory");
        if (hh == 1) {
#pragma unroll
            for (int i = 0; i < 4; i++) {
                *(uint4 *)(Kr + i * 1024 + lane * 16) = pk[i];
                *(uint4 *)(Vr + i * 1024 + lane * 16) = pv[i];
            }
            asm volatile("s_waitcnt lgkmcnt(0)" ::: "memory");
        }
#pragma unroll 2
        for (int hl = 0; hl < 8; hl++) {
            const int ck = 2 * hl + (q4 >> 1), sub = (q4 & 1) * 8;
            const s16x4 kf = *(const s16x4 *)(Kr + c16 * 256 + ((ck ^ c16) << 4) + sub);
            s16x4 vf;
            const int cv = 2 * hl + (c16 >> 3), vb = (c16 & 7) * 2;
#pragma unroll
            for (int e = 0; e < 4; e++) {
                const int row = 4 * q4 + e;
                vf[e] = *(const short *)(Vr + row * 256 + ((cv ^ row) << 4) + vb);
            }
#pragma unroll
            for (int t = 0; t < 2; t++) {
                const int qrow = 16 * t + c16;
                const s16x4 qf = *(const s16x4 *)(Qr + qrow * 256 + ((ck ^ (qrow & 15)) << 4) + sub);
                f32x4 sc = {0.f, 0.f, 0.f, 0.f};
                sc = __builtin_amdgcn_mfma_f32_16x16x16bf16_1k(kf, qf, sc, 0, 0, 0);
                const bool valid = q4 == 2 * t + (c16 >> 3);
                const float s0 = sc[0] * 0.25f, s1 = sc[1] * 0.25f, s2 = sc[2] * 0.25f, s3 = sc[3] * 0.25f;
                const float mx = fmaxf(fmaxf(s0, s1), fmaxf(s2, s3));
                const float e0 = __expf(s0 - mx), e1 = __expf(s1 - mx), e2 = __expf(s2 - mx), e3 = __expf(s3 - mx);
                const float inv = valid ? 1.0f / (e0 + e1 + e2 + e3) : 0.f;
                const uint2 pp = make_uint2(f2bf2(e0 * inv, e1 * inv), f2bf2(e2 * inv, e3 * inv));
                s16x4 pf;
                __builtin_memcpy(&pf, &pp, 8);
                f32x4 o = {0.f, 0.f, 0.f, 0.f};
                o = __builtin_amdgcn_mfma_f32_16x16x16bf16_1k(pf, vf, o, 0, 0, 0);
                const unsigned o01 = f2bf2(o[0], o[1]), o23 = f2bf2(o[2], o[3]);
#pragma unroll
                for (int rr = 0; rr < 4; rr++) {
                    const int orow = 16 * t + 4 * q4 + rr;
                    const unsigned w = rr < 2 ? o01 : o23;
                    *(unsigned short *)(Qr + orow * 256 + ((cv ^ (orow & 15)) << 4) + vb) = (unsigned short)((rr & 1) ? (w >> 16) : w);
                }
            }
        }
    }
    asm volatile("s_waitcnt lgkmcnt(0)" ::: "memory");
    if (KEEP) store_rows(o_out);
    load_rows(bf);
#pragma unroll
    for (int ks = 0; ks < 16; ks++) wf[ks] = *(const bf16x8 *)(Wo + ((size_t)ks * 64 + lane) * 8);
    float *T = (float *)R;
    const int erow = lane >> 3, ec = (lane & 7) * 4;
    float4 xr[4], xn4[4];
#pragma unroll
    for (int p4 = 0; p4 < 4; p4++) xr[p4] = *(const float4 *)(x + (row0 + min(erow + 8 * p4, q_rows - 1)) * 256 + ec);
#pragma unroll 1
    for (int nt = 0; nt < 8; nt++) {
        const unsigned short *wnext = Wo + ((size_t)min(nt + 1, 7) * 1024 + lane) * 8;
        bf16x8 wn[16];
#pragma unroll
        for (int ks = 0; ks < 16; ks++) wn[ks] = *(const bf16x8 *)(wnext + ks * 512);
#pragma unroll
        for (int p4 = 0; p4 < 4; p4++) xn4[p4] = *(const float4 *)(x + (row0 + min(erow + 8 * p4, q_rows - 1)) * 256 + min(nt + 1, 7) * 32 + ec);
        f32x16 acc;
#pragma unroll
        for (int i = 0; i < 16; i++) acc[i] = 0.f;
#pragma unroll
        for (int ks = 0; ks < 16; ks++) acc = __builtin_amdgcn_mfma_f32_32x32x16_bf16(wf[ks], bf[ks], acc, 0, 0, 0);
#pragma unroll
        for (int g = 0; g < 4; g++)
            *(float4 *)(T + frow * 36 + 8 * g + 4 * (lane >> 5)) = make_float4(acc[4 * g], acc[4 * g + 1], acc[4 * g + 2], acc[4 * g + 3]);
#pragma unroll
        for (int p4 = 0; p4 < 4; p4++) {
            const int row = erow + 8 * p4;
            const float4 v = *(const float4 *)(T + row * 36 + ec);
            if (row < q_rows)
                *(float4 *)(y + (row0 + row) * 256 + nt * 32 + ec) = make_float4(v.x + xr[p4].x, v.y + xr[p4].y, v.z + xr[p4].z, v.w + xr[p4].w);
// ... 10 lines not shown
```

### lara_amd/csrc/mfma_gemm.h

```cpp
#pragma once
#include "common.h"
#include "wave.h"

namespace {

__global__ void __launch_bounds__(256)
ln_cast_kernel(const float *__restrict__ x, const float *__restrict__ gamma,
               const float *__restrict__ beta, const float eps, unsigned short *__restrict__ out,
               float2 *__restrict__ stats, const int tokens) {
    const int tok = blockIdx.x * 4 + (threadIdx.x >> 6), lane = threadIdx.x & 63;
    if (tok >= tokens) return;
    const float4 v = ((const float4 *)(x + (size_t)tok * 256))[lane];
    float s = v.x + v.y + v.z + v.w;
#pragma unroll
    for (int d = 32; d > 0; d >>= 1) s += __shfl_xor(s, d, 64);
    const float mean = s * (1.0f / 256.0f);
    const float a = v.x - mean, b = v.y - mean, c = v.z - mean, d4 = v.w - mean;
    float q = a * a + b * b + c * c + d4 * d4;
#pragma unroll
    for (int d = 32; d > 0; d >>= 1) q += __shfl_xor(q, d, 64);
    const float rstd = 1.0f / sqrtf(q * (1.0f / 256.0f) + eps);
    const float4 g = ((const float4 *)gamma)[lane], be = ((const float4 *)beta)[lane];
    ushort4 o;
    o.x = f2bf(a * rstd * g.x + be.x); o.y = f2bf(b * rstd * g.y + be.y);
    o.z = f2bf(c * rstd * g.z + be.z); o.w = f2bf(d4 * rstd * g.w + be.w);
    ((ushort4 *)(out + (size_t)tok * 256))[lane] = o;
    if (stats && lane == 0) stats[tok] = make_float2(mean, rstd);
}

constexpr int GK = 32;
constexpr int LROW = GK * 2 + 16;

struct GemmP {
    const unsigned short *A, *W;
    void *C;
    const float *resid;
    const float *bias;
    int M, N, K;
    int R, Cin;
    const float2 *stats;
    const float *gamma, *beta;
    int Cout;
    uint32_t zero_off;
    unsigned short *C2;
    float *colsum;
    const float *lnx;
};

__device__ __forceinline__ void token_to_voxel(const int m, const int R, int &b, int &d, int &h, int &w) {
    const int Gd = R >> 1, l = m & 7;
    int g = m >> 3;
    const int gw = g % Gd; g /= Gd;
    const int gh = g % Gd; g /= Gd;
    const int gd = g % Gd; b = g / Gd;
    d = 2 * gd + (l >> 2); h = 2 * gh + ((l >> 1) & 1); w = 2 * gw + (l & 1);
}
__device__ __forceinline__ int voxel_to_token(const int b, const int d, const int h, const int w, const int R) {
    const int Gd = R >> 1;
    return ((((b * Gd + (d >> 1)) * Gd + (h >> 1)) * Gd + (w >> 1)) << 3) | ((d & 1) << 2) | ((h & 1) << 1) | (w & 1);
}

__device__ __forceinline__ void xcd_tile(int &rt, int &ct) {
    const int rtiles = gridDim.x, nc = gridDim.y;
    const int L = blockIdx.x + rtiles * blockIdx.y;
    const int full = (rtiles >> 3) << 3, base = full * nc;
    if (L < base) {
        const int q = L / (8 * nc), rem = L - q * (8 * nc);
        ct = rem >> 3;
        rt = q * 8 + (rem & 7);
    } else {
        const int t = rtiles - full, l = L - base;
        ct = l / t;
        rt = full + (l - ct * t);
    }
}

template <int EPI>
__device__ __forceinline__ void gemm_epilogue(const GemmP &p, float4 v, const int row, const int col, const int N,
                                              const unsigned long long base_out) {
    static_assert(EPI == 0 || EPI == 1 || EPI == 4 || EPI == 5 || EPI == 8, "the epilogues that exist");
    const size_t o = (size_t)row * N + col;
    if (EPI == 0) {
        ushort4 h;
        h.x = f2bf(v.x); h.y = f2bf(v.y); h.z = f2bf(v.z); h.w = f2bf(v.w);
        *(ushort4 *)((unsigned short *)p.C + o) = h;
    } else if (EPI == 8) {
        *(float4 *)((float *)p.C + o) = v;
    } else if (EPI == 1) {
        const float4 rs = *(const float4 *)(p.resid + o);
        *(float4 *)((float *)p.C + o) = make_float4(v.x + rs.x, v.y + rs.y, v.z + rs.z, v.w + rs.w);
    } else if (EPI == 4) {
        const float4 rs = *(const float4 *)(p.resid + o);
        const float2 st = p.stats[row];
        const float4 ga = *(const float4 *)(p.gamma + col), be = *(const float4 *)(p.beta + col);
        *(float4 *)((float *)p.C + o) =
            make_float4(v.x + (rs.x - st.x) * st.y * ga.x + be.x, v.y + (rs.y - st.x) * st.y * ga.y + be.y,
                        v.z + (rs.z - st.x) * st.y * ga.z + be.z, v.w + (rs.w - st.x) * st.y * ga.w + be.w);
    } else {
        const int tap = col / p.Cout, co = col - tap * p.Cout;
        const size_t R2 = 2 * (size_t)p.R;
        const size_t oo = (base_out + ((size_t)(tap >> 2) * R2 + ((tap >> 1) & 1)) * R2 + (tap & 1)) * p.Cout + co;
        const float4 bs = *(const float4 *)(p.bias + co);
        *(float4 *)((float *)p.C + oo) = make_float4(v.x + bs.x, v.y + bs.y, v.z + bs.z, v.w + bs.w);
    }
}

template <int AMODE, int EPI, int GM = 128, int GN = 128>
__global__ void __launch_bounds__(256)
gemm_bf16_nt_kernel(const GemmP p) {
    static_assert(AMODE == 0 && GM == 128 && GN == 128, "dense A on 128 x 128 tiles; the convolution runs on the ring kernels");
    constexpr int MI = GM / 64;
    constexpr int NJ = GN / 64;
    constexpr int NA = GM / 64;
    constexpr int NS = (GM + GN) / 64;
    __shared__ __attribute__((aligned(16))) unsigned char lds[2][(GM + GN) * LROW];
    const unsigned short *__restrict__ A = p.A, *__restrict__ W = p.W;
    const int M = p.M, N = p.N, K = p.K;
    const int tid = threadIdx.x, wave = tid >> 6, lane = tid & 63;
    int rt_, ct_;
    xcd_tile(rt_, ct_);
    const int bm0 = rt_ * GM, bn0 = ct_ * GN;
// ... 24 lines not shown
    auto lstore = [&](int buf) {
        unsigned char *l = &lds[buf][0];
        *(uint4 *)(l + loff[0]) = st0; *(uint4 *)(l + loff[1]) = st1;
        *(uint4 *)(l + loff[2]) = st2; *(uint4 *)(l + loff[3]) = st3;
    };

    f32x16 acc[MI][NJ];
#pragma unroll
    for (int i = 0; i < MI; i++)
#pragma unroll
        for (int j = 0; j < NJ; j++)
#pragma unroll
            for (int e = 0; e < 16; e++) acc[i][j][e] = 0.f;

    gload(0);
    lstore(0);
    __syncthreads();
    for (int kt = 0; kt < ktiles; kt++) {
        const int buf = kt & 1;
        if (kt + 1 < ktiles) gload(kt + 1);
        const unsigned char *la = &lds[buf][(wm + r) * LROW + kh * 16];
        const unsigned char *lb = &lds[buf][(GM + wn + r) * LROW + kh * 16];
        bf16x8 a[2][MI], b[2][NJ];
#pragma unroll
        for (int i = 0; i < MI; i++) a[0][i] = *(const bf16x8 *)(la + i * 32 * LROW);
#pragma unroll
        for (int j = 0; j < NJ; j++) b[0][j] = *(const bf16x8 *)(lb + j * 32 * LROW);
#pragma unroll
        for (int s = 0; s < GK / 16; s++) {
            if (s + 1 < GK / 16) {
#pragma unroll
                for (int i = 0; i < MI; i++) a[(s + 1) & 1][i] = *(const bf16x8 *)(la + i * 32 * LROW + (s + 1) * 32);
#pragma unroll
                for (int j = 0; j < NJ; j++) b[(s + 1) & 1][j] = *(const bf16x8 *)(lb + j * 32 * LROW + (s + 1) * 32);
            }
#pragma unroll
            for (int i = 0; i < MI; i++)
#pragma unroll
                for (int j = 0; j < NJ; j++)
                    acc[i][j] = __builtin_amdgcn_mfma_f32_32x32x16_bf16(a[s & 1][i], b[s & 1][j], acc[i][j], 0, 0, 0);
        }
        if (kt + 1 < ktiles) lstore(buf ^ 1);
        __syncthreads();
    }
    float *ep = (float *)&lds[0][0] + wave * (32 * 68);
    unsigned long long *rowbase = (unsigned long long *)((float *)&lds[0][0] + 4 * (32 * 68)) + wave * 32;
#pragma unroll
    for (int ij = 0; ij < MI * (NJ / 2); ij++) {
        const int i = ij / (NJ / 2), jh = ij % (NJ / 2);
        __syncthreads();
#pragma unroll
        for (int j = 0; j < 2; j++)
#pragma unroll
            for (int e = 0; e < 16; e++)
                ep[((e & 3) + 8 * (e >> 2) + 4 * kh) * 68 + j * 32 + r] = acc[i][2 * jh + j][e];
        if (EPI == 5 && lane < 32) {
            int b, d, h, w;
            token_to_voxel(min(bm0 + wm + i * 32 + lane, M - 1), p.R, b, d, h, w);
            const size_t R2 = 2 * (size_t)p.R;
            rowbase[lane] = (((size_t)b * R2 + 2 * d) * R2 + 2 * h) * R2 + 2 * w;
        }
        __syncthreads();
#pragma unroll
        for (int q = 0; q < 8; q++) {
            const int idx = q * 64 + lane, lr = idx >> 4, c4 = (idx & 15) * 4;
            const int row = bm0 + wm + i * 32 + lr, col = bn0 + wn + jh * 64 + c4;
            if (row < M && col < N)
                gemm_epilogue<EPI>(p, *(const float4 *)(ep + lr * 68 + c4), row, col, N, EPI == 5 ? rowbase[lr] : 0ull);
        }
    }
}

constexpr int RT = 256;
constexpr int RING = 4;
constexpr int RTILE = 2 * RT * 64;

template <int EPI>
__device__ __forceinline__ void ring_epilogue(const GemmP &p, f32x16 (&acc)[4][2], unsigned char *ring, const int wave,
                                              const int lane, const int bm0, const int bn0, const int wr, const int wc) {
    const int M = p.M, N = p.N;
    const int r = lane & 31, kh = lane >> 5;
    float *ep = (float *)ring + wave * (32 * 68);
    unsigned long long *rowbase = (unsigned long long *)((float *)ring + 8 * (32 * 68)) + wave * 32;
#pragma unroll
    for (int i = 0; i < 4; i++) {
        __syncthreads();
#pragma unroll
        for (int j = 0; j < 2; j++)
#pragma unroll
            for (int e = 0; e < 16; e++)
                ep[((e & 3) + 8 * (e >> 2) + 4 * kh) * 68 + j * 32 + r] = acc[i][j][e];
        if (EPI == 5 && lane < 32) {
            int b, d, h, w;
            token_to_voxel(min(bm0 + wr * 128 + i * 32 + lane, M - 1), p.R, b, d, h, w);
            const size_t R2 = 2 * (size_t)p.R;
            rowbase[lane] = (((size_t)b * R2 + 2 * d) * R2 + 2 * h) * R2 + 2 * w;
        }
        __syncthreads();
#pragma unroll
        for (int q = 0; q < 8; q++) {
            const int idx = q * 64 + lane, lr = idx >> 4, c4 = (idx & 15) * 4;
            const int row = bm0 + wr * 128 + i * 32 + lr, col = bn0 + wc * 64 + c4;
            if (row < M && col < N)
                gemm_epilogue<EPI>(p, *(const float4 *)(ep + lr * 68 + c4), row, col, N, EPI == 5 ? rowbase[lr] : 0ull);
        }
    }
}

__device__ __forceinline__ float row16_total(float x) {
    x += __int_as_float(__builtin_amdgcn_update_dpp(0, __float_as_int(x), 0xB1, 0xf, 0xf, false));
    x += __int_as_float(__builtin_amdgcn_update_dpp(0, __float_as_int(x), 0x4E, 0xf, 0xf, false));
    x += __int_as_float(__builtin_amdgcn_update_dpp(0, __float_as_int(x), 0x141, 0xf, 0xf, false));
    x += __int_as_float(__builtin_amdgcn_update_dpp(0, __float_as_int(x), 0x140, 0xf, 0xf, false));
    return x;
}

__device__ __forceinline__ void ring_epilogue_lnbwd(const GemmP &p, f32x16 (&acc)[4][2], unsigned char *ring, const int wave,
                                                    const int lane, const int bm0, const int wr, const int wc) {
    const int M = p.M, tid = wave * 64 + lane;
    const int r = lane & 31, kh = lane >> 5;
    float *ep = (float *)ring + wave * (32 * 68);
    float2 *rowsum = (float2 *)((float *)ring + 8 * (32 * 68) + 512);
    const int lg = lane >> 4, c4 = (lane & 15) * 4, col = wc * 64 + c4;
    const float4 ga = *(const float4 *)(p.gamma + col);
    float cg[4] = {0.f, 0.f, 0.f, 0.f}, cb[4] = {0.f, 0.f, 0.f, 0.f}, co[4] = {0.f, 0.f, 0.f, 0.f};
#pragma unroll 1
    for (int i = 0; i < 4; i++) {
        __syncthreads();
#pragma unroll
        for (int j = 0; j < 2; j++)
#pragma unroll
            for (int e = 0; e < 16; e++)
                ep[((e & 3) + 8 * (e >> 2) + 4 * kh) * 68 + j * 32 + r] = i == 0 ? acc[0][j][e] : i == 1 ? acc[1][j][e] : i == 2 ? acc[2][j][e] : acc[3][j][e];
#pragma unroll 1
        for (int half = 0; half < 2; half++) {
            __syncthreads();
            float4 dy[4], xh[4];
            float rstd[4];
#pragma unroll
            for (int q = 0; q < 4; q++) {
                const int lr = 16 * half + 4 * q + lg, row = bm0 + wr * 128 + i * 32 + lr;
                const bool in = row < M;
                const size_t o = (size_t)(in ? row : 0) * 256 + col;
                const float4 v = *(const float4 *)(ep + lr * 68 + c4), rs = *(const float4 *)(p.resid + o), xx = *(const float4 *)(p.lnx + o);
                const float2 st = p.stats[in ? row : 0];
                const float m = in ? 1.f : 0.f;
                dy[q] = make_float4(m * (v.x + rs.x), m * (v.y + rs.y), m * (v.z + rs.z), m * (v.w + rs.w));
                xh[q] = make_float4((xx.x - st.x) * st.y, (xx.y - st.x) * st.y, (xx.z - st.x) * st.y, (xx.w - st.x) * st.y);
                rstd[q] = st.y;
                const float a0 = dy[q].x * ga.x, a1 = dy[q].y * ga.y, a2 = dy[q].z * ga.z, a3 = dy[q].w * ga.w;
                const float sa = row16_total((a0 + a1) + (a2 + a3));
                const float sh = row16_total((a0 * xh[q].x + a1 * xh[q].y) + (a2 * xh[q].z + a3 * xh[q].w));
                if ((lane & 15) == 0) rowsum[(wr * 32 + lr) * 4 + wc] = make_float2(sa, sh);
            }
            __syncthreads();
#pragma unroll
            for (int q = 0; q < 4; q++) {
                const int lr = 16 * half + 4 * q + lg, row = bm0 + wr * 128 + i * 32 + lr;
                const float4 s01 = *(const float4 *)(rowsum + (wr * 32 + lr) * 4), s23 = *(const float4 *)(rowsum + (wr * 32 + lr) * 4 + 2);
                const float sa = ((s01.x + s01.z) + (s23.x + s23.z)) * (1.0f / 256.0f), sh = ((s01.y + s01.w) + (s23.y + s23.w)) * (1.0f / 256.0f);
                const float a0 = dy[q].x * ga.x, a1 = dy[q].y * ga.y, a2 = dy[q].z * ga.z, a3 = dy[q].w * ga.w;
                const float4 dx = make_float4(rstd[q] * (a0 - sa - xh[q].x * sh), rstd[q] * (a1 - sa - xh[q].y * sh),
                                              rstd[q] * (a2 - sa - xh[q].z * sh), rstd[q] * (a3 - sa - xh[q].w * sh));
                if (row < M) {
                    const size_t o = (size_t)row * 256 + col;
                    *(float4 *)((float *)p.C + o) = dx;
                    ushort4 hb;
                    hb.x = f2bf(dx.x); hb.y = f2bf(dx.y); hb.z = f2bf(dx.z); hb.w = f2bf(dx.w);
                    *(ushort4 *)(p.C2 + o) = hb;
                    cg[0] += dy[q].x * xh[q].x; cg[1] += dy[q].y * xh[q].y; cg[2] += dy[q].z * xh[q].z; cg[3] += dy[q].w * xh[q].w;
                    cb[0] += dy[q].x; cb[1] += dy[q].y; cb[2] += dy[q].z; cb[3] += dy[q].w;
                    co[0] += dx.x; co[1] += dx.y; co[2] += dx.z; co[3] += dx.w;
                }
            }
        }
    }
#pragma unroll
    for (int c = 0; c < 4; c++) {
        cg[c] += __shfl_xor(cg[c], 16); cg[c] += __shfl_xor(cg[c], 32);
        cb[c] += __shfl_xor(cb[c], 16); cb[c] += __shfl_xor(cb[c], 32);
        co[c] += __shfl_xor(co[c], 16); co[c] += __shfl_xor(co[c], 32);
    }
    __syncthreads();
    float *cs = (float *)ring;
    if (lane < 16) {
        *(float4 *)(cs + (wr * 3 + 0) * 256 + col) = make_float4(cg[0], cg[1], cg[2], cg[3]);
        *(float4 *)(cs + (wr * 3 + 1) * 256 + col) = make_float4(cb[0], cb[1], cb[2], cb[3]);
        *(float4 *)(cs + (wr * 3 + 2) * 256 + col) = make_float4(co[0], co[1], co[2], co[3]);
    }
    __syncthreads();
    for (int k = tid; k < 768; k += 512) p.colsum[(size_t)(bm0 / RT) * 768 + k] = cs[k] + cs[768 + k];
}

template <int AMODE, int EPI>
__global__ void __launch_bounds__(512)
gemm_ring_kernel(const GemmP p) {
    static_assert(AMODE == 0 && EPI != 9, "dense A only: the convolution (AMODE 1; EPI 4, 9) runs on gemm_ring2_kernel");
    extern __shared__ __attribute__((aligned(16))) unsigned char ring[];
    const int tid = threadIdx.x, wave = tid >> 6, lane = tid & 63;
    const int M = p.M, N = p.N, K = p.K, Cin = AMODE ? p.Cin : 0;
    int rt_, ct_;
    xcd_tile(rt_, ct_);
    const int bm0 = rt_ * RT, bn0 = ct_ * RT;
    const int wr = wave >> 2, wc = wave & 3;
    const int r = lane & 31, kh = lane >> 5;
    const char *Ab = (const char *)p.A, *Wb = (const char *)p.W;

    int srow[2];
    uint32_t woff[2], noff[2];
    int vb[2], vd[2], vh[2], vw[2];
#pragma unroll
    for (int q = 0; q < 2; q++) {
        srow[q] = 32 * wave + 16 * q + (lane >> 2);
        const int chunk = (lane & 3) ^ ((srow[q] >> 2) & 3);
        woff[q] = (uint32_t)min(bn0 + srow[q], N - 1) * (uint32_t)(K * 2) + chunk * 16;
        if (AMODE == 1) {
            token_to_voxel(min(bm0 + srow[q], M - 1), p.R, vb[q], vd[q], vh[q], vw[q]);
            noff[q] = chunk * 16;
        } else {
            vb[q] = vd[q] = vh[q] = vw[q] = 0;
            noff[q] = (uint32_t)min(bm0 + srow[q], M - 1) * (uint32_t)(K * 2) + chunk * 16;
        }
    }
    const int ktiles = K / 32, kpt = AMODE ? Cin / 32 : 1;
    int cur_tap = -1;
    auto issue = [&](const int kt) {
        const int tap = AMODE ? kt / kpt : 0, kc = AMODE ? kt - tap * kpt : kt, ksrc = kt;
        if (AMODE == 1 && tap != cur_tap) {
            cur_tap = tap;
            const int dz = tap / 9 - 1, dy = (tap / 3) % 3 - 1, dx = tap % 3 - 1;
#pragma unroll
            for (int q = 0; q < 2; q++) {
                const int nd = vd[q] + dz, nh = vh[q] + dy, nw = vw[q] + dx;
                const bool in = (unsigned)nd < (unsigned)p.R && (unsigned)nh < (unsigned)p.R && (unsigned)nw < (unsigned)p.R;
                const int chunk = (lane & 3) ^ ((srow[q] >> 2) & 3);
                noff[q] = (in ? (uint32_t)voxel_to_token(vb[q], nd, nh, nw, p.R) * (uint32_t)(Cin * 2) : p.zero_off) + chunk * 16;
            }
        }
        unsigned char *buf = ring + (kt % RING) * RTILE;
#pragma unroll
        for (int q = 0; q < 2; q++) {
            __builtin_amdgcn_global_load_lds((const __attribute__((address_space(1))) void *)(Ab + (noff[q] + (uint32_t)kc * 64)),
                                             (__attribute__((address_space(3))) void *)(buf + (2 * wave + q) * 1024), 16, 0, 0);
            __builtin_amdgcn_global_load_lds((const __attribute__((address_space(1))) void *)(Wb + (woff[q] + (uint32_t)ksrc * 64)),
                                             (__attribute__((address_space(3))) void *)(buf + RT * 64 + (2 * wave + q) * 1024), 16, 0, 0);
        }
    };

    f32x16 acc[4][2];
#pragma unroll
    for (int i = 0; i < 4; i++)
#pragma unroll
        for (int j = 0; j < 2; j++)
#pragma unroll
            for (int e = 0; e < 16; e++) acc[i][j][e] = 0.f;

    int aoff[4][2], boff[2][2];
#pragma unroll
    for (int s = 0; s < 2; s++) {
#pragma unroll
        for (int i = 0; i < 4; i++) {
            const int row = wr * 128 + 32 * i + r;
            aoff[i][s] = row * 64 + (((2 * s + kh) ^ ((row >> 2) & 3)) << 4);
        }
#pragma unroll
        for (int j = 0; j < 2; j++) {
            const int row = wc * 64 + 32 * j + r;
            boff[j][s] = RT * 64 + row * 64 + (((2 * s + kh) ^ ((row >> 2) & 3)) << 4);
        }
    }

    bf16x8 fa[2][4], fb[2][2];
    auto fetch = [&](const int set, const int kt, const int step) {
        const unsigned char *buf = ring + (kt % RING) * RTILE;
#pragma unroll
        for (int i = 0; i < 4; i++) fa[set][i] = *(const bf16x8 *)(buf + aoff[i][step]);
#pragma unroll
        for (int j = 0; j < 2; j++) fb[set][j] = *(const bf16x8 *)(buf + boff[j][step]);
    };
    auto mac = [&](const int set, const int i0, const int i1) {
#pragma unroll
        for (int i = i0; i < i1; i++)
#pragma unroll
            for (int j = 0; j < 2; j++)
                acc[i][j] = __builtin_amdgcn_mfma_f32_32x32x16_bf16(fa[set][i], fb[set][j], acc[i][j], 0, 0, 0);
    };
    auto wait_tile = [&](const int younger) {
        if (younger >= 3) asm volatile("s_waitcnt vmcnt(12)" ::: "memory");
        else if (younger == 2) asm volatile("s_waitcnt vmcnt(8)" ::: "memory");
        else if (younger == 1) asm volatile("s_waitcnt vmcnt(4)" ::: "memory");
        else asm volatile("s_waitcnt vmcnt(0)" ::: "memory");
    };
    issue(0);
    if (1 < ktiles) issue(1);
    if (2 < ktiles) issue(2);
    if (3 < ktiles) issue(3);
    wait_tile(min(ktiles - 1, 3));
    __builtin_amdgcn_s_barrier();
    fetch(0, 0, 0);
    for (int kt = 0; kt < ktiles; kt++) {
        mac(0, 0, 1);
        __builtin_amdgcn_sched_barrier(0);
        fetch(1, kt, 1);
        __builtin_amdgcn_sched_barrier(0);
        mac(0, 1, 4);
        __builtin_amdgcn_sched_barrier(0);
        asm volatile("s_waitcnt lgkmcnt(0)" ::: "memory");
        if (kt + 1 < ktiles) {
            wait_tile(min(ktiles - 2 - kt, 2));
            __builtin_amdgcn_s_barrier();
        }
        __builtin_amdgcn_sched_barrier(0);
        mac(1, 0, 1);
        __builtin_amdgcn_sched_barrier(0);
        if (kt + 1 < ktiles) {
            if (kt + 4 < ktiles) issue(kt + 4);
            fetch(0, kt + 1, 0);
        }
        __builtin_amdgcn_sched_barrier(0);
        mac(1, 1, 4);
        __builtin_amdgcn_sched_barrier(0);
    }
    __syncthreads();

    ring_epilogue<EPI>(p, acc, ring, wave, lane, bm0, bn0, wr, wc);
}

template <int AMODE, int EPI>
__global__ void __launch_bounds__(512)
gemm_ring2_kernel(const GemmP p) {
    extern __shared__ __attribute__((aligned(16))) unsigned char ring[];
    const int tid = threadIdx.x, lane = tid & 63;
    const int wave = __builtin_amdgcn_readfirstlane(tid >> 6);
    const int M = p.M, N = p.N, K = p.K, Cin = AMODE ? p.Cin : 0;
    int rt_, ct_;
    xcd_tile(rt_, ct_);
    const int bm0 = rt_ * RT, bn0 = ct_ * RT;
    const int wr = wave >> 2, wc = wave & 3;
    const int r = lane & 31, kh = lane >> 5;
    const char *Ab = (const char *)p.A, *Wb = (const char *)p.W;

    int srow[2];
    uint32_t woff[2], noff[2];
    int vb[2], vd[2], vh[2], vw[2];
#pragma unroll
    for (int q = 0; q < 2; q++) {
        srow[q] = 32 * wave + 16 * q + (lane >> 2);
        const int chunk = (lane & 3) ^ ((srow[q] >> 2) & 3);
        woff[q] = (uint32_t)min(bn0 + srow[q], N - 1) * (uint32_t)(K * 2) + chunk * 16;
        if (AMODE == 1) {
            token_to_voxel(min(bm0 + srow[q], M - 1), p.R, vb[q], vd[q], vh[q], vw[q]);
            noff[q] = chunk * 16;
        } else {
            vb[q] = vd[q] = vh[q] = vw[q] = 0;
            noff[q] = (uint32_t)min(bm0 + srow[q], M - 1) * (uint32_t)(K * 2) + chunk * 16;
        }
    }
    auto set_tap = [&](const int tap) {
        const int dz = tap / 9 - 1, dy = (tap / 3) % 3 - 1, dx = tap % 3 - 1;
#pragma unroll
        for (int q = 0; q < 2; q++) {
            const int nd = vd[q] + dz, nh = vh[q] + dy, nw = vw[q] + dx;
            const bool in = (unsigned)nd < (unsigned)p.R && (unsigned)nh < (unsigned)p.R && (unsigned)nw < (unsigned)p.R;
            const int chunk = (lane & 3) ^ ((srow[q] >> 2) & 3);
            noff[q] = (in ? (uint32_t)voxel_to_token(vb[q], nd, nh, nw, p.R) * (uint32_t)(Cin * 2) : p.zero_off) + chunk * 16;
        }
    };
    const int gpt = AMODE ? Cin / 128 : 1;
    int g_in_tap = 0, tap_i = 0;
    if (AMODE == 1) set_tap(0);
    auto next_group = [&]() {
        woff[0] += 256; woff[1] += 256;
        if (AMODE == 1 && ++g_in_tap == gpt) {
            g_in_tap = 0;
            set_tap(++tap_i);
        } else {
            noff[0] += 256; noff[1] += 256;
        }
    };
    const uint32_t mine = (uint32_t)(size_t)(__attribute__((address_space(3))) unsigned char *)ring + wave * 2048;
#define R2_DMA(base, voff, lds, t)                                                                                   \
    asm volatile("s_mov_b32 m0, %0\n\ts_nop 0\n\tglobal_load_lds_dwordx4 %1, %2 offset:%3"                            \
                 :: "s"((uint32_t)((lds) - (t) * 64)), "v"(voff), "s"(base), "n"((t) * 64) : "memory")
#define R2_DMA_A(slot, t, q) R2_DMA(Ab, noff[q], mine + (slot) * RTILE + (q) * 1024, t)
#define R2_DMA_W(slot, t, q) R2_DMA(Wb, woff[q], mine + (slot) * RTILE + RT * 64 + (q) * 1024, t)

    f32x16 acc[4][2];
#pragma unroll
    for (int i = 0; i < 4; i++)
#pragma unroll
        for (int j = 0; j < 2; j++)
#pragma unroll
            for (int e = 0; e < 16; e++) acc[i][j][e] = 0.f;

    int aoff[2][2], boff[2][2];
#pragma unroll
    for (int s = 0; s < 2; s++) {
        const int ra = wr * 128 + r, rb = wc * 64 + r;
        aoff[s][0] = ra * 64 + (((2 * s + kh) ^ ((ra >> 2) & 3)) << 4);
        boff[s][0] = RT * 64 + rb * 64 + (((2 * s + kh) ^ ((rb >> 2) & 3)) << 4);
        aoff[s][1] = aoff[s][0] + 2 * RTILE;
        boff[s][1] = boff[s][0] + 2 * RTILE;
        asm volatile("" : "+v"(aoff[s][1]), "+v"(boff[s][1]));
    }
    bf16x8 fa[2][4], fb[2][2];
#define R2_SB __builtin_amdgcn_sched_barrier(0)
#define R2_M(set, i, j) acc[i][j] = __builtin_amdgcn_mfma_f32_32x32x16_bf16(fa[set][i], fb[set][j], acc[i][j], 0, 0, 0)
#define R2_RA(set, i, slot, step) fa[set][i] = *(const bf16x8 *)(ring + ((slot) & 1) * RTILE + aoff[step][(slot) >> 1] + (i) * 2048)
#define R2_RB(set, j, slot, step) fb[set][j] = *(const bf16x8 *)(ring + ((slot) & 1) * RTILE + boff[step][(slot) >> 1] + (j) * 2048)
#define R2_HALF(USE, READ, slot, step, MODE, it, q)                      \
    R2_M(USE, 0, 0); R2_SB;                                              \
    if (READ) R2_RA(USE ^ 1, 0, slot, step);                             \
    R2_SB; R2_M(USE, 0, 1); R2_SB;                                       \
    if (READ) R2_RB(USE ^ 1, 0, slot, step);                             \
    if ((MODE) == 2) R2_DMA_A(it, it, 0);                                \
    R2_SB; R2_M(USE, 1, 0); R2_SB;                                       \
    if (READ) R2_RB(USE ^ 1, 1, slot, step);                             \
    if ((MODE) == 1) R2_DMA_A(it, it, q);                                \
    if ((MODE) == 2) R2_DMA_W(it, it, 0);                                \
    R2_SB; R2_M(USE, 1, 1); R2_SB;                                       \
    if (READ) R2_RA(USE ^ 1, 1, slot, step);                             \
    if ((MODE) == 2) R2_DMA_A(it, it, 1);                                \
    R2_SB; R2_M(USE, 2, 0); R2_SB;                                       \
    if (READ) R2_RA(USE ^ 1, 2, slot, step);                             \
    if ((MODE) == 1) R2_DMA_W(it, it, q);                                \
    if ((MODE) == 2) R2_DMA_W(it, it, 1);                                \
    R2_SB; R2_M(USE, 2, 1); R2_SB;                                       \
    if (READ) R2_RA(USE ^ 1, 3, slot, step);                             \
    R2_SB; R2_M(USE, 3, 0); R2_M(USE, 3, 1); R2_SB;
#define R2_TILE(t, M1, M2, VM)                                                                  \
    R2_HALF(0, true, t, 1, M1, ((t) + 3) & 3, 0)                                                \
    if ((VM) >= 0) {                                                                            \
        asm volatile("s_waitcnt lgkmcnt(0)" ::: "memory");                                      \
        if ((VM) == 8) asm volatile("s_waitcnt vmcnt(8)" ::: "memory");                         \
        else if ((VM) == 6) asm volatile("s_waitcnt vmcnt(6)" ::: "memory");                    \
        else if ((VM) == 4) asm volatile("s_waitcnt vmcnt(4)" ::: "memory");                    \
        else asm volatile("s_waitcnt vmcnt(0)" ::: "memory");                                   \
        __builtin_amdgcn_s_barrier();                                                           \
// ... 66 lines not shown
```

### lara_amd/encoder.py

```python
from __future__ import annotations

import torch
from torch import nn

from ._native import BlockWeights as _BlockWeights, call, query, require_device


def _require_device(t: torch.Tensor):
    require_device(t)
    if t.requires_grad and torch.is_grad_enabled():
        raise RuntimeError("lara_amd.encoder holds the inference classes; use lara_amd.encoder_train.VolTransformer to train")


def volume_to_tokens(volume: torch.Tensor) -> torch.Tensor:
    _require_device(volume)
    B, C, R = volume.shape[0], volume.shape[1], volume.shape[2]
    v = volume.float().contiguous()
    out = torch.empty(B * R ** 3, C, dtype=torch.float32, device=v.device)
    call("lara_tokens_from_volume", v.device, B, R, C, v, out)
    return out


def tokens_to_volume(tokens: torch.Tensor, B: int, R: int) -> torch.Tensor:
    _require_device(tokens)
    C = tokens.shape[1]
    t = tokens.float().contiguous()
    out = torch.empty(B, C, R, R, R, dtype=torch.float32, device=t.device)
    call("lara_volume_from_tokens", t.device, B, R, C, t, out)
    return out


def cond_tokens(image_feats: torch.Tensor, n_group: int) -> torch.Tensor:
    B, V, C, D = image_feats.shape[:4]
    if D != n_group or V != 4:
        raise RuntimeError("kernels are specialised for one image-feature voxel per group and 4 input views "
                           "(configs/base.yaml: n_groups [16], 16^3 feature volume, n_views 4)")
    return image_feats.permute(0, 3, 4, 5, 1, 2).reshape(B * D ** 3, V, C).to(torch.bfloat16).contiguous()


class GroupAttBlock(nn.Module):

    def __init__(self, inner_dim: int, cond_dim: int, num_heads: int, eps: float = 1e-5,
                 attn_drop: float = 0., attn_bias: bool = False, mlp_ratio: float = 2., mlp_drop: float = 0.):
        super().__init__()
        if inner_dim != 256 or num_heads != 16 or attn_bias or mlp_ratio != 2.:
            raise ValueError("kernels are specialised for LaRa's 256-dim, 16-head, bias-free blocks "
                             "(configs/base.yaml:17-20)")
        self.inner_dim, self.cond_dim = inner_dim, cond_dim
        self.eps = 1e-5
        f = lambda *s: nn.Parameter(torch.zeros(*s))
        h = lambda *s: torch.zeros(*s, dtype=torch.bfloat16)
        self.ln1_w, self.ln1_b, self.ln2_w, self.ln2_b = f(256), f(256), f(256), f(256)
        self.ln3_w, self.ln3_b, self.b1, self.b2 = f(256), f(256), f(512), f(256)
        self.register_buffer("wq", h(256, 256))
        self.register_buffer("wkv", h(512, cond_dim))
        self.register_buffer("wo", h(256, 256))
        self.register_buffer("w1", h(512, 256))
        self.register_buffer("w2", h(256, 512))
        self.register_buffer("wconv", h(256, 27 * 256))
        self._ws = None

    @classmethod
    def from_reference(cls, block) -> "GroupAttBlock":
        mha = block.cross_attn
        m = cls(mha.embed_dim, mha.kdim, mha.num_heads)
        m.eps = float(block.norm1.eps)
        bf = torch.bfloat16
        with torch.no_grad():
            for dst, src in ((m.ln1_w, block.norm1.weight), (m.ln1_b, block.norm1.bias),
                             (m.ln2_w, block.norm2.weight), (m.ln2_b, block.norm2.bias),
                             (m.ln3_w, block.norm3.weight), (m.ln3_b, block.norm3.bias),
                             (m.b1, block.mlp[0].bias), (m.b2, block.mlp[3].bias)):
                dst.copy_(src)
            m.wq.copy_(mha.q_proj_weight.to(bf))
            m.wkv.copy_(torch.cat([mha.k_proj_weight, mha.v_proj_weight], 0).to(bf))
            m.wo.copy_(mha.out_proj.weight.to(bf))
            m.w1.copy_(block.mlp[0].weight.to(bf))
            m.w2.copy_(block.mlp[3].weight.to(bf))
            m.wconv.copy_(block.cnn.weight.permute(0, 2, 3, 4, 1).reshape(256, 27 * 256).to(bf))
        return m

    def _weights(self) -> _BlockWeights:
        w = _BlockWeights()
        for n in ("ln1_w", "ln1_b", "wq", "wkv", "wo", "ln2_w", "ln2_b", "w1", "b1", "w2", "b2", "ln3_w", "ln3_b", "wconv"):
            setattr(w, n, getattr(self, n).data_ptr())
        w.eps = self.eps
        return w

    def forward_tokens(self, x: torch.Tensor, cond_bf16: torch.Tensor, scenes: int, R: int) -> torch.Tensor:
        _require_device(x)
        if x.dtype != torch.float32 or not x.is_contiguous() or x.shape != (scenes * R ** 3, 256):
            raise RuntimeError("expected contiguous fp32 token rows [scenes * R^3, 256]")
        if cond_bf16.dtype != torch.bfloat16 or cond_bf16.shape != (scenes * (R // 2) ** 3, 4, self.cond_dim):
            raise RuntimeError("expected bf16 cond [scenes * (R/2)^3, 4, cond_dim]")
        need = query("lara_groupblock_workspace_bytes", scenes, R)
        if self._ws is None or self._ws.numel() < need or self._ws.device != x.device:
            self._ws = torch.empty(need, dtype=torch.uint8, device=x.device)
        call("lara_groupblock_forward", x.device, scenes, R, self.cond_dim, x, cond_bf16.contiguous(), self._weights(), self._ws)
        return x

    def forward(self, x: torch.Tensor, cond: torch.Tensor, group_axis: int, block_size: int) -> torch.Tensor:
        B, C, D = x.shape[0], x.shape[1], x.shape[2]
        if block_size != 2 or group_axis * block_size != D:
            raise RuntimeError("kernels are specialised for block_size 2 (configs/base.yaml: 32^3 volume, 16 groups per axis)")
        tok = volume_to_tokens(x)
        self.forward_tokens(tok, cond.to(torch.bfloat16), B, D)
        return tokens_to_volume(tok, B, D)


class VolTransformer(nn.Module):

    def __init__(self, embed_dim: int, image_feat_dim: int, n_groups: list, vol_low_res: int, vol_high_res: int,
                 out_dim: int, num_layers: int, num_heads: int, eps: float = 1e-6):
        super().__init__()
        if len(n_groups) != 1 or vol_low_res != 2 * n_groups[0] or vol_high_res != 2 * vol_low_res or out_dim % 4:
            raise ValueError("kernels are specialised for one group size with block_size 2 and a x2 deconvolution "
                             "(configs/base.yaml: n_groups [16], vol 32 -> 64)")
        self.vol_low_res, self.vol_high_res, self.out_dim, self.n_groups = vol_low_res, vol_high_res, out_dim, list(n_groups)
        self.embed_dim, self.eps = embed_dim, eps
        self.pos_embed = nn.Parameter(torch.zeros(1, embed_dim, vol_low_res, vol_low_res, vol_low_res))
        self.layers = nn.ModuleList([GroupAttBlock(embed_dim, image_feat_dim, num_heads) for _ in range(num_layers)])
        self.norm_w, self.norm_b = nn.Parameter(torch.ones(embed_dim)), nn.Parameter(torch.zeros(embed_dim))
        self.register_buffer("wdeconv", torch.zeros(8 * out_dim, embed_dim, dtype=torch.bfloat16))
        self.deconv_b = nn.Parameter(torch.zeros(out_dim))
        self._pos_tokens = None
        self._ws = None
        self._graphs = {}

    @classmethod
    def from_reference(cls, vt) -> "VolTransformer":
        mha = vt.layers[0].cross_attn
        m = cls(vt.embed_dim, mha.kdim, vt.n_groups, vt.vol_low_res, vt.vol_high_res, vt.out_dim, len(vt.layers),
                mha.num_heads, float(vt.norm.eps))
        with torch.no_grad():
            m.pos_embed.copy_(vt.pos_embed)
            m.layers = nn.ModuleList([GroupAttBlock.from_reference(b) for b in vt.layers])
            m.norm_w.copy_(vt.norm.weight)
            m.norm_b.copy_(vt.norm.bias)
            m.wdeconv.copy_(vt.deconv.weight.permute(2, 3, 4, 1, 0).reshape(8 * vt.out_dim, vt.embed_dim).to(torch.bfloat16))
            m.deconv_b.copy_(vt.deconv.bias)
        return m

    def _run(self, cond: torch.Tensor, x: torch.Tensor, out: torch.Tensor, B: int) -> None:
        R, dev = self.vol_low_res, cond.device
        x.view(B, -1, self.embed_dim).copy_(self._pos_tokens)
        for layer in self.layers:
            layer.forward_tokens(x, cond, B, R)
        call("lara_voltrans_head_forward", dev, B, R, x, self.norm_w, self.norm_b, float(self.eps), self.wdeconv, self.deconv_b,
             self.out_dim, out, self._ws)

    def forward(self, image_feats: torch.Tensor, use_graph: bool = False) -> torch.Tensor:
        _require_device(image_feats)
        B, R = image_feats.shape[0], self.vol_low_res
        dev = image_feats.device
        cond = cond_tokens(image_feats, self.n_groups[0])
        pos_key = (self.pos_embed.data_ptr(), self.pos_embed._version, dev)
        if self._pos_tokens is None or getattr(self, "_pos_key", None) != pos_key:
            with torch.no_grad():
                self._pos_tokens = volume_to_tokens(self.pos_embed.detach().to(dev))
            self._pos_key = pos_key
            self._graphs = {}
        need = B * R ** 3 * 512
        if self._ws is None or self._ws.numel() < need or self._ws.device != dev:
            self._ws = torch.empty(need, dtype=torch.uint8, device=dev)
            self._graphs = {}
        if not use_graph:
            x = torch.empty(B * R ** 3, self.embed_dim, dtype=torch.float32, device=dev)
            out = torch.empty(B, 2 * R, 2 * R, 2 * R, self.out_dim, dtype=torch.float32, device=dev)
            self._run(cond, x, out, B)
            return out
        key = (B, dev.index)
        entry = self._graphs.get(key)
        if entry is None:
            s_cond = torch.empty_like(cond)
            s_x = torch.empty(B * R ** 3, self.embed_dim, dtype=torch.float32, device=dev)
            s_out = torch.empty(B, 2 * R, 2 * R, 2 * R, self.out_dim, dtype=torch.float32, device=dev)
            s_cond.copy_(cond)
            side = torch.cuda.Stream(dev)
            side.wait_stream(torch.cuda.current_stream(dev))
            with torch.cuda.stream(side):
                self._run(s_cond, s_x, s_out, B)
            torch.cuda.current_stream(dev).wait_stream(side)
            graph = torch.cuda.CUDAGraph()
            with torch.cuda.graph(graph):
                self._run(s_cond, s_x, s_out, B)
            entry = (graph, s_cond, s_x, s_out)
            self._graphs[key] = entry
        graph, s_cond, s_x, s_out = entry
        s_cond.copy_(cond)
        graph.replay()
        return s_out.clone()
```

### lara_amd/encoder_train.py

```python
from __future__ import annotations

import math

import torch
from torch import nn

from ._native import (BlockGrads as _BlockGrads, BlockWeights as _BlockWeights, BlockWeightsT as _BlockWeightsT, call, query,
                      require_device)
from ._native import current_stream as _stream, load_library as _lib
from .encoder import tokens_to_volume, volume_to_tokens

_GRAD_FIELDS = ("ln1_w", "ln1_b", "wq", "wkv", "wo", "ln2_w", "ln2_b", "w1", "b1", "w2", "b2", "ln3_w", "ln3_b", "wconv")


def _keep_activations() -> bool:
    import os
    return os.environ.get("LARA_ENCODER_RECOMPUTE", "0") != "1"


_scratch = {}


def _workspace(dev, tag: str, nbytes: int) -> torch.Tensor:
    key = (dev.index, tag)
    t = _scratch.get(key)
    if t is None or t.numel() < nbytes:
        t = torch.empty(nbytes, dtype=torch.uint8, device=dev)
        _scratch[key] = t
    return t


_LAYER_PARAMS = ("norm1.weight", "norm1.bias", "cross_attn.q_proj_weight", "cross_attn.k_proj_weight",
                 "cross_attn.v_proj_weight", "cross_attn.out_proj.weight", "norm2.weight", "norm2.bias",
                 "mlp.0.weight", "mlp.0.bias", "mlp.3.weight", "mlp.3.bias", "norm3.weight", "norm3.bias", "cnn.weight")
_NLP = len(_LAYER_PARAMS)


_wcache = {}


def _layer_bf16(p):
    key = tuple((t.data_ptr(), t._version) for t in p)
    hit = _wcache.get(key)
    if hit is not None:
        return hit[1]
    (ln1w, ln1b, wq, wk, wv, wo, ln2w, ln2b, w1, b1, w2, b2, ln3w, ln3b, wc) = p
    bf = torch.bfloat16
    f = {"ln1_w": ln1w.float().contiguous(), "ln1_b": ln1b.float().contiguous(),
         "ln2_w": ln2w.float().contiguous(), "ln2_b": ln2b.float().contiguous(),
         "ln3_w": ln3w.float().contiguous(), "ln3_b": ln3b.float().contiguous(),
         "b1": b1.float().contiguous(), "b2": b2.float().contiguous(),
         "wq": wq.to(bf).contiguous(), "wkv": torch.cat([wk, wv], 0).to(bf).contiguous(), "wo": wo.to(bf).contiguous(),
         "w1": w1.to(bf).contiguous(), "w2": w2.to(bf).contiguous(),
         "wconv": wc.to(bf).permute(0, 2, 3, 4, 1).reshape(256, 27 * 256).contiguous()}
    if len(_wcache) >= 64:
        _wcache.clear()
    _wcache[key] = (list(p), f)
    return f


def invalidate_weight_cache():
    _wcache.clear()


def _layer_bf16_t(f):
    t = f.get("_t")
    if t is None:
        t = f["_t"] = _transposed(f)
    return t


def _transposed(f):
    return {"wq_t": f["wq"].t().contiguous(), "wkv_t": f["wkv"].t().contiguous(), "wo_t": f["wo"].t().contiguous(),
            "w1_t": f["w1"].t().contiguous(), "w2_t": f["w2"].t().contiguous(),
            "wconv_t": f["wconv"].view(256, 27, 256).flip(1).permute(2, 1, 0).reshape(256, 27 * 256).contiguous()}


def _fill(struct, tensors, names):
    for n in names:
        setattr(struct, n, tensors[n].data_ptr())
    return struct


def _forward_inference(image_feats, eps_block, eps_final, R, out_dim, pos_embed, norm_w, norm_b, deconv_w, deconv_b, *layer_params):
    require_device(image_feats)
    dev = image_feats.device
    B, V, cond_dim = image_feats.shape[:3]
    S = image_feats.shape[3] * image_feats.shape[4] * image_feats.shape[5]
    feats = image_feats.detach().float().contiguous()
    cond_bf = torch.empty(B * S, V, cond_dim, dtype=torch.bfloat16, device=dev)
    call("lara_batched_transpose", dev, B, V * cond_dim, S, feats, cond_bf, 1)
    return _inference_from_cond(cond_bf, B, cond_dim, eps_block, eps_final, R, out_dim, pos_embed, norm_w, norm_b, deconv_w, deconv_b,
                                *layer_params)


def _inference_from_cond(cond_bf, B, cond_dim, eps_block, eps_final, R, out_dim, pos_embed, norm_w, norm_b, deconv_w, deconv_b,
                         *layer_params):
    dev = cond_bf.device
    n_layers = len(layer_params) // _NLP
    M = B * R ** 3
    x = volume_to_tokens(pos_embed.detach().float()).repeat(B, 1)
    ws = _workspace(dev, "fwd", query("lara_groupblock_workspace_bytes", B, R))
    with torch.cuda.device(dev):
        for l in range(n_layers):
            f = _layer_bf16([t.detach() for t in layer_params[l * _NLP:(l + 1) * _NLP]])
            w = _fill(_BlockWeights(), f, _GRAD_FIELDS)
            w.eps = eps_block
            call("lara_groupblock_forward", dev, B, R, cond_dim, x, cond_bf, w, ws)
        wd = deconv_w.detach().permute(2, 3, 4, 1, 0).reshape(8 * out_dim, 256).to(torch.bfloat16).contiguous()
        nw, nb, db = norm_w.detach().float().contiguous(), norm_b.detach().float().contiguous(), deconv_b.detach().float().contiguous()
        out = torch.empty(B, 2 * R, 2 * R, 2 * R, out_dim, dtype=torch.float32, device=dev)
        hws = _workspace(dev, "head", M * 512)
        call("lara_voltrans_head_forward", dev, B, R, x, nw, nb, float(eps_final), wd, db, out_dim, out, hws)
    return out


_ws_owner = {}
_block_bwd_log = None


class _Sweep:

    def __init__(self, B, R, cond_dim, n_layers, eps_block, dev):
        self.B, self.R, self.cond_dim, self.n_layers, self.eps_block, self.dev = B, R, cond_dim, n_layers, eps_block, dev
        self.cond_bf = None
        self.fs = [None] * n_layers
        self.dkv_all = None
        self.flat = None
        self.offs = self.shapes = self.per_layer = None

    def accumulators(self, l):
        f = self.fs[l]
        if self.flat is None:
            self.shapes = {n: tuple(f[n].shape) for n in _GRAD_FIELDS}
            self.offs, o = {}, 0
            for n in _GRAD_FIELDS:
                self.offs[n] = o
                o += (math.prod(self.shapes[n]) + 63) // 64 * 64
            self.per_layer = o
            self.flat = torch.zeros(self.n_layers * o, dtype=torch.float32, device=self.dev)
        base = l * self.per_layer
        return {n: self.flat[base + self.offs[n]:base + self.offs[n] + math.prod(self.shapes[n])].view(self.shapes[n])
                for n in _GRAD_FIELDS}


class _CondFn(torch.autograd.Function):
    @staticmethod
    def forward(ctx, image_feats, sweep):
        dev = image_feats.device
        B, V, C = image_feats.shape[:3]
        S = image_feats.shape[3] * image_feats.shape[4] * image_feats.shape[5]
        feats = image_feats.detach().float().contiguous()
        cond_bf = torch.empty(B * S, V, C, dtype=torch.bfloat16, device=dev)
        call("lara_batched_transpose", dev, B, V * C, S, feats, cond_bf, 1)
        sweep.cond_bf = cond_bf
        ctx.sweep, ctx.feat_shape, ctx.feat_dtype = sweep, tuple(image_feats.shape), image_feats.dtype
        return torch.zeros(1, dtype=torch.float32, device=dev)

    @staticmethod
    def backward(ctx, g_token):
        sw = ctx.sweep
        if not ctx.needs_input_grad[0]:
            return None, None
        dev = sw.dev
        cond_bf = sw.cond_bf
        dcond = torch.empty(cond_bf.shape, dtype=torch.float32, device=dev)
        lddkv = sw.n_layers * 512
        with torch.cuda.device(dev):
            wkv_all_t = torch.cat([f["wkv"] for f in sw.fs], 0).t().contiguous()
            call("lara_gemm_nt_bf16", dev, sw.dkv_all.shape[0], sw.cond_dim, lddkv, sw.dkv_all, wkv_all_t, dcond, 1)
            Bf, V, C = ctx.feat_shape[:3]
            S = dcond.shape[0] // Bf
            d_feats = torch.empty(ctx.feat_shape, dtype=torch.float32, device=dev)
            call("lara_batched_transpose", dev, Bf, S, V * C, dcond, d_feats, 0)
        sw.dkv_all = sw.flat = None
        return (d_feats if ctx.feat_dtype == torch.float32 else d_feats.to(ctx.feat_dtype)), None


class _FeatCondFn(torch.autograd.Function):

    @staticmethod
    def forward(ctx, img_feats, ln_w, ln_b, mlp_w, mlp_b, embed, prep, sweep):
        from .featvol import TOKENS
        prep.params(ln_w, ln_b, mlp_w, mlp_b, embed)
        sweep.cond_bf = prep.forward(TOKENS)
        ctx.sweep, ctx.prep = sweep, prep
        return torch.zeros(1, dtype=torch.float32, device=img_feats.device)

    @staticmethod
    def backward(ctx, g_token):
        from .featvol import TOKENS
        sw = ctx.sweep
        if not any(ctx.needs_input_grad[:6]):
            return (None,) * 8
        dev = sw.dev
        dcond = torch.empty(sw.cond_bf.shape, dtype=torch.float32, device=dev)
        lddkv = sw.n_layers * 512
        with torch.cuda.device(dev):
            wkv_all_t = torch.cat([f["wkv"] for f in sw.fs], 0).t().contiguous()
            call("lara_gemm_nt_bf16", dev, sw.dkv_all.shape[0], sw.cond_dim, lddkv, sw.dkv_all, wkv_all_t, dcond, 1)
        sw.dkv_all = sw.flat = None
        dx, d_lnw, d_lnb, d_w, d_b, d_e = ctx.prep.backward(dcond, TOKENS, ctx.needs_input_grad[5])
        return dx, d_lnw, d_lnb, d_w, d_b, d_e, None, None


class _StartFn(torch.autograd.Function):
    @staticmethod
    def forward(ctx, pos_embed, token, B, R):
        ctx.B, ctx.R = B, R
        return volume_to_tokens(pos_embed.detach().float()).repeat(B, 1)

    @staticmethod
    def backward(ctx, g):
        return tokens_to_volume(g.view(ctx.B, ctx.R ** 3, 256).sum(0), 1, ctx.R), torch.zeros(1, dtype=torch.float32, device=g.device), None, None


class _BlockFn(torch.autograd.Function):
    @staticmethod
    def forward(ctx, x, sweep, l, *p):
        sw = sweep
        dev = x.device
        f = sw.fs[l] = _layer_bf16([t.detach() for t in p])
        w = _fill(_BlockWeights(), f, _GRAD_FIELDS)
        w.eps = sw.eps_block
        keep = _keep_activations()
        with torch.cuda.device(dev):
            if keep:
                act = torch.empty(query("lara_groupblock_save_bytes", sw.B, sw.R), dtype=torch.uint8, device=dev)
                x_out = torch.empty_like(x)
                call("lara_groupblock_forward_train", dev, sw.B, sw.R, sw.cond_dim, x, x_out, sw.cond_bf, w, act)
            else:
                act = None
                x_out = x.clone()
                ws = _workspace(dev, "fwd", query("lara_groupblock_workspace_bytes", sw.B, sw.R))
                call("lara_groupblock_forward", dev, sw.B, sw.R, sw.cond_dim, x_out, sw.cond_bf, w, ws)
        ctx.save_for_backward(x)
        ctx.sweep, ctx.l, ctx.act = sw, l, act
        return x_out

    @staticmethod
    def backward(ctx, g):
        sw, l = ctx.sweep, ctx.l
        (x_in,) = ctx.saved_tensors
        dev = sw.dev
        f = sw.fs[l]
        ft = _layer_bf16_t(f)
        w = _fill(_BlockWeights(), f, _GRAD_FIELDS)
        w.eps = sw.eps_block
        wt = _fill(_BlockWeightsT(), ft, ("wq_t", "wkv_t", "wo_t", "w1_t", "w2_t", "wconv_t"))
        lddkv = sw.n_layers * 512
        if sw.dkv_all is None:
            sw.dkv_all = torch.empty(sw.cond_bf.shape[0] * sw.cond_bf.shape[1], lddkv, dtype=torch.bfloat16, device=dev)
        gd = sw.accumulators(l)
        dw = _fill(_BlockGrads(), gd, _GRAD_FIELDS)
        g = g.float()
        if not g.is_contiguous():
            g = g.contiguous()
        chained = int(_ws_owner.get(dev.index) == (id(sw), l + 1))
        with torch.cuda.device(dev):
            ws = _workspace(dev, "block_bwd", query("lara_groupblock_backward_workspace_bytes", sw.B, sw.R))
            if _block_bwd_log is not None:
                _block_bwd_log.append(("block_backward_launch", l))
            call("lara_groupblock_backward", dev, sw.B, sw.R, sw.cond_dim, x_in, sw.cond_bf, w, wt, ctx.act, g, None, dw, chained,
                 sw.dkv_all.data_ptr() + l * 1024, lddkv, ws)
        _ws_owner[dev.index] = (id(sw), l)
        ctx.act = None
        return (g, None, None, gd["ln1_w"], gd["ln1_b"], gd["wq"], gd["wkv"][:256], gd["wkv"][256:], gd["wo"], gd["ln2_w"], gd["ln2_b"],
                gd["w1"], gd["b1"], gd["w2"], gd["b2"], gd["ln3_w"], gd["ln3_b"],
                gd["wconv"].view(256, 3, 3, 3, 256).permute(0, 4, 1, 2, 3))


class _HeadFn(torch.autograd.Function):
    @staticmethod
    def forward(ctx, x, norm_w, norm_b, deconv_w, deconv_b, sweep, eps_final, out_dim):
        sw = sweep
        dev = x.device
        M = sw.B * sw.R ** 3
        with torch.cuda.device(dev):
            wd = deconv_w.detach().permute(2, 3, 4, 1, 0).reshape(8 * out_dim, 256).to(torch.bfloat16).contiguous()
            nw, nb, db = norm_w.detach().float().contiguous(), norm_b.detach().float().contiguous(), deconv_b.detach().float().contiguous()
            out = torch.empty(sw.B, 2 * sw.R, 2 * sw.R, 2 * sw.R, out_dim, dtype=torch.float32, device=dev)
            hws = _workspace(dev, "head", M * 512)
            call("lara_voltrans_head_forward", dev, sw.B, sw.R, x, nw, nb, float(eps_final), wd, db, out_dim, out, hws)
        ctx.save_for_backward(x, norm_w, norm_b, deconv_w)
        ctx.sweep, ctx.eps_final, ctx.out_dim = sw, float(eps_final), out_dim
        return out

    @staticmethod
    def backward(ctx, dout):
        sw = ctx.sweep
        x_last, norm_w, norm_b, deconv_w = ctx.saved_tensors
        dev, out_dim = sw.dev, ctx.out_dim
        M = sw.B * sw.R ** 3
        f32 = dict(dtype=torch.float32, device=dev)
        dout = dout.float().contiguous()
        g = torch.empty(M, 256, **f32)
        d_nw, d_nb = torch.zeros(256, **f32), torch.zeros(256, **f32)
        d_wd, d_b8 = torch.zeros(8 * out_dim, 256, **f32), torch.zeros(8 * out_dim, **f32)
        with torch.cuda.device(dev):
            wd_t = deconv_w.detach().permute(2, 3, 4, 1, 0).reshape(8 * out_dim, 256).to(torch.bfloat16).t().contiguous()
            nw, nb = norm_w.detach().float().contiguous(), norm_b.detach().float().contiguous()
            hws = _workspace(dev, "head_bwd", query("lara_voltrans_head_backward_workspace_bytes", sw.B, sw.R, out_dim))
            call("lara_voltrans_head_backward", dev, sw.B, sw.R, x_last, nw, nb, ctx.eps_final, wd_t, out_dim, dout, g, d_nw, d_nb,
                 d_wd, d_b8, hws)
        _ws_owner.pop(dev.index, None)
        sw.flat = sw.dkv_all = None
        return (g, d_nw, d_nb, d_wd.view(2, 2, 2, out_dim, 256).permute(4, 3, 0, 1, 2), d_b8.view(8, out_dim).sum(0), None, None, None)


def _forward_per_block(module, image_feats):
    B, V, C = image_feats.shape[:3]
    sweep = _Sweep(B, module.vol_low_res, C, len(module.layers), float(module.layers[0].norm1.eps), image_feats.device)
    return _sweep_from(module, sweep, _CondFn.apply(image_feats, sweep))


def _sweep_from(module, sweep, token):
    B, R = sweep.B, module.vol_low_res
    x = _StartFn.apply(module.pos_embed, token, B, R)
    for l, layer in enumerate(module.layers):
        x = _BlockFn.apply(x, sweep, l, *layer.flat_params())
    return _HeadFn.apply(x, module.norm.weight, module.norm.bias, module.deconv.weight, module.deconv.bias, sweep,
                         float(module.norm.eps), module.out_dim)


class GroupAttBlock(nn.Module):

    def __init__(self, inner_dim: int, cond_dim: int, num_heads: int, eps: float = 1e-5, attn_drop: float = 0.,
                 attn_bias: bool = False, mlp_ratio: float = 2., mlp_drop: float = 0.):
        super().__init__()
        if inner_dim != 256 or num_heads != 16 or attn_bias or mlp_ratio != 2. or attn_drop or mlp_drop:
            raise ValueError("kernels are specialised for LaRa's 256-dim, 16-head, bias-free, dropout-free blocks "
                             "(configs/base.yaml:17-20)")
        if cond_dim == inner_dim:
            raise ValueError("cond_dim must differ from inner_dim (LaRa: 800 vs 256); the fused in_proj_weight "
                             "layout of nn.MultiheadAttention is not supported")
        self.norm1 = nn.LayerNorm(inner_dim)
        self.cross_attn = nn.MultiheadAttention(embed_dim=inner_dim, num_heads=num_heads, kdim=cond_dim, vdim=cond_dim,
                                                dropout=attn_drop, bias=attn_bias, batch_first=True)
        self.cnn = nn.Conv3d(inner_dim, inner_dim, kernel_size=3, padding=1, bias=False)
        self.norm2 = nn.LayerNorm(inner_dim)
        self.norm3 = nn.LayerNorm(inner_dim)
        self.mlp = nn.Sequential(nn.Linear(inner_dim, int(inner_dim * mlp_ratio)), nn.GELU(), nn.Dropout(mlp_drop),
                                 nn.Linear(int(inner_dim * mlp_ratio), inner_dim), nn.Dropout(mlp_drop))

    def flat_params(self):
        sd = dict(self.named_parameters())
        return [sd[n] for n in _LAYER_PARAMS]


class VolTransformer(nn.Module):

    def __init__(self, embed_dim: int, image_feat_dim: int, n_groups: list, vol_low_res: int, vol_high_res: int,
                 out_dim: int, num_layers: int, num_heads: int, eps: float = 1e-6):
        super().__init__()
        if len(n_groups) != 1 or vol_low_res != 2 * n_groups[0] or vol_high_res != 2 * vol_low_res or out_dim % 16:
            raise ValueError("kernels are specialised for one group size with block_size 2 and a x2 deconvolution "
                             "(configs/base.yaml: n_groups [16], vol 32 -> 64)")
        self.vol_low_res, self.vol_high_res, self.out_dim, self.n_groups = vol_low_res, vol_high_res, out_dim, list(n_groups)
        self.embed_dim = embed_dim
        self.pos_embed = nn.Parameter(torch.randn(1, embed_dim, vol_low_res, vol_low_res, vol_low_res) * (1. / embed_dim) ** 0.5)
        self.layers = nn.ModuleList([GroupAttBlock(inner_dim=embed_dim, cond_dim=image_feat_dim, num_heads=num_heads, eps=eps)
                                     for _ in range(num_layers)])
        self.norm = nn.LayerNorm(embed_dim, eps=eps)
        self.deconv = nn.ConvTranspose3d(embed_dim, out_dim, kernel_size=2, stride=2, padding=0)

    def forward(self, image_feats: torch.Tensor) -> torch.Tensor:
        require_device(image_feats)
        B, V, C, D = image_feats.shape[:4]
        if D != self.n_groups[0] or V != 4:
            raise RuntimeError("kernels are specialised for one image-feature voxel per group and 4 input views")
        if torch.is_grad_enabled():
            return _forward_per_block(self, image_feats)
        flat = [p for layer in self.layers for p in layer.flat_params()]
        return _forward_inference(image_feats, float(self.layers[0].norm1.eps), float(self.norm.eps), self.vol_low_res, self.out_dim,
                                 self.pos_embed, self.norm.weight, self.norm.bias, self.deconv.weight, self.deconv.bias, *flat)

    def forward_from_image_features(self, feat_volume, batch, img_feats: torch.Tensor, n_views_sel=None) -> torch.Tensor:
        prep = feat_volume.prepare(batch, img_feats, n_views_sel)
        if prep.V != 4 or feat_volume.R != self.n_groups[0]:
            raise RuntimeError("kernels are specialised for one image-feature voxel per group and 4 input views")
        B, C = prep.B, prep.C + prep.E
        args = feat_volume._args(prep.V)
        if torch.is_grad_enabled():
            sweep = _Sweep(B, self.vol_low_res, C, len(self.layers), float(self.layers[0].norm1.eps), img_feats.device)
            return _sweep_from(self, sweep, _FeatCondFn.apply(img_feats, *args, prep, sweep))
        from .featvol import TOKENS
        prep.params(*args)
        flat = [p for layer in self.layers for p in layer.flat_params()]
        return _inference_from_cond(prep.forward(TOKENS), B, C, float(self.layers[0].norm1.eps), float(self.norm.eps), self.vol_low_res,
                                    self.out_dim, self.pos_embed, self.norm.weight, self.norm.bias, self.deconv.weight,
                                    self.deconv.bias, *flat)
```

### lara_amd/featvol.py

```python
from __future__ import annotations

import torch
from torch import nn

from ._native import FeatvolDims as _Dims, alloc_bytes, call, query, require_device
from ._native import load_library as _lib

VOLUME, TOKENS = 0, 1
MAX_C, MAX_HW = 1024, 8192


class _ModLN(nn.Module):

    def __init__(self, inner_dim: int, mod_dim: int, eps: float):
        super().__init__()
        self.norm = nn.LayerNorm(inner_dim, eps=eps)
        self.mlp = nn.Sequential(nn.SiLU(), nn.Linear(mod_dim, inner_dim * 2))


def build_dense_grid(reso: int, scene_size: float = 0.5) -> torch.Tensor:
    a = torch.arange(reso)
    grid = torch.stack(torch.meshgrid(a, a, a, indexing="ij"), dim=-1)
    return ((grid + 0.5) / reso * 2 - 1).reshape(reso, reso, reso, 3) * scene_size


class _Prep:

    def __init__(self, fv, batch, img_feats, n_views_sel):
        require_device(img_feats)
        if img_feats.dim() != 4 or img_feats.dtype != torch.float32:
            raise ValueError(f"img_feats must be fp32 [B*V, C, h, w]; got {img_feats.dtype} {tuple(img_feats.shape)}")
        V = int(n_views_sel)
        rays = batch["tar_rays_down"]
        B = rays.shape[0]
        BV, C, h, w = img_feats.shape
        if not 1 <= V <= min(8, rays.shape[1]) or BV != B * V:
            raise ValueError(f"img_feats holds {BV} maps; expected B * n_views_sel = {B} * {V} (at most 8 and the batch's views)")
        if tuple(rays.shape[2:]) != (h, w, 6):
            raise ValueError(f"tar_rays_down {tuple(rays.shape)} does not match the feature map {h} x {w}")
        if C != fv.C or C % 64 or C > MAX_C or h * w > MAX_HW:
            raise ValueError(f"feature channels {C} (module: {fv.C}; a multiple of 64 up to {MAX_C}), map {h} x {w} (at most {MAX_HW} texels)")
        if V > fv.view_embed.shape[1] and fv.E > 0:
            raise ValueError(f"view_embed has {fv.view_embed.shape[1]} rows, n_views_sel = {V}")
        dev = img_feats.device
        f32 = lambda t: t.detach().to(device=dev, dtype=torch.float32).contiguous()
        self.x = img_feats.detach()
        self.rays = f32(rays[:, :V])
        self.w2c = f32(batch["tar_w2c"][:, :V])
        self.ixt = f32(batch["tar_ixt"][:, :V])
        self.grid = f32(fv.volume_grid.reshape(-1, 3))
        H, W = batch["tar_rgb"].shape[2:4]
        d = _Dims()
        d.B, d.V, d.C, d.E, d.h, d.w, d.R, d.img_w, d.img_h = B, V, C, fv.E, h, w, fv.R, int(W), int(H)
        d.eps = float(fv.dir_norm.norm.eps)
        for i, s in enumerate(img_feats.stride()):
            d.x_stride[i] = s
        self.d, self.dev, self.B, self.V, self.C, self.E, self.S = d, dev, B, V, C, fv.E, fv.R ** 3

    def params(self, ln_w, ln_b, mlp_w, mlp_b, embed):
        f = lambda t: None if t is None else t.detach().float().contiguous()
        self.p = (f(ln_w), f(ln_b), f(mlp_w), f(mlp_b), f(embed))

    def _ws(self):
        return alloc_bytes(query("lara_featvol_workspace_bytes", self.d), self.dev)

    def _inputs(self):
        return (self.x, self.rays, self.w2c, self.ixt, self.grid) + self.p[:4]

    def forward(self, layout):
        CE, R = self.C + self.E, self.d.R
        out = (torch.empty(self.B, self.V, CE, R, R, R, dtype=torch.float32, device=self.dev) if layout == VOLUME else
               torch.empty(self.B * self.S, self.V, CE, dtype=torch.bfloat16, device=self.dev))
        call("lara_featvol_forward", self.dev, self.d, *self._inputs(), self.p[4], layout, out, self._ws())
        return out

    def backward(self, grad, layout, want_embed=True):
        f32 = dict(dtype=torch.float32, device=self.dev)
        grad = grad.float().contiguous()
        dx = torch.empty_strided(self.x.shape, self.x.stride(), **f32)
        C = self.C
        d_lnw, d_lnb = torch.empty(C, **f32), torch.empty(C, **f32)
        d_w, d_b = torch.empty(2 * C, 32, **f32), torch.empty(2 * C, **f32)
        d_e = torch.empty(self.V, self.E, **f32) if (want_embed and self.E > 0) else None
        call("lara_featvol_backward", self.dev, self.d, *self._inputs(), grad, layout, dx, d_lnw, d_lnb, d_w, d_b, d_e, self._ws())
        return dx, d_lnw, d_lnb, d_w, d_b, d_e


class _FeatVolFn(torch.autograd.Function):

    @staticmethod
    def forward(ctx, img_feats, ln_w, ln_b, mlp_w, mlp_b, embed, prep):
        prep.params(ln_w, ln_b, mlp_w, mlp_b, embed)
        ctx.prep = prep
        return prep.forward(VOLUME)

    @staticmethod
    def backward(ctx, g):
        dx, d_lnw, d_lnb, d_w, d_b, d_e = ctx.prep.backward(g, VOLUME, ctx.needs_input_grad[5])
        return dx, d_lnw, d_lnb, d_w, d_b, d_e, None


class FeatureVolume(nn.Module):

    def __init__(self, C: int = 768, E: int = 32, R: int = 16, eps: float = 1e-6, scene_size: float = 0.5,
                 dir_norm: nn.Module = None, view_embed: nn.Parameter = None):
        super().__init__()
        self.C, self.E, self.R = C, E, R
        self.dir_norm = dir_norm if dir_norm is not None else _ModLN(C, 16 * 2, eps)
        if E > 0:
            self.view_embed = view_embed if view_embed is not None else nn.Parameter(torch.randn(1, 4, E, 1, 1, 1) * (1. / E) ** 0.5)
            if tuple(self.view_embed.shape[2:]) != (E, 1, 1, 1):
                raise ValueError(f"view_embed must be [1, n, {E}, 1, 1, 1]; got {tuple(self.view_embed.shape)}")
        else:
            self.view_embed = None
        lin = self.dir_norm.mlp[1]
        if tuple(lin.weight.shape) != (2 * C, 32) or lin.bias is None or self.dir_norm.norm.weight.shape[0] != C:
            raise ValueError("dir_norm must be ModLN(C, 32): norm = LayerNorm(C), mlp = Sequential(SiLU, Linear(32, 2C))")
        self.register_buffer("volume_grid", build_dense_grid(R, scene_size))

    def _args(self, V):
        n, lin = self.dir_norm.norm, self.dir_norm.mlp[1]
        embed = self.view_embed[0, :V, :, 0, 0, 0] if self.E > 0 else None
        return n.weight, n.bias, lin.weight, lin.bias, embed

    def prepare(self, batch, img_feats, n_views_sel=None):
        V = n_views_sel if n_views_sel is not None else img_feats.shape[0] // batch["tar_rays_down"].shape[0]
        return _Prep(self, batch, img_feats, V)

    def forward(self, batch, img_feats, n_views_sel=None):
        prep = self.prepare(batch, img_feats, n_views_sel)
        return _FeatVolFn.apply(img_feats, *self._args(prep.V), prep)
```

Measured before the change: 966.9.

## Batch all layers' KV projections into one GEMM with padded cond tokens

Computes K/V for every transformer layer up front with a single wide GEMM over the conditioning tokens, using concatenated per-layer wkv weights. Each block then reads its KV slice through a leading-dimension stride instead of running its own GEMM. The KV buffer is dropped from the saved activations. Conditioning tokens are padded to an aligned leading dimension, and a new transpose kernel zero-fills the pad. This removes per-layer small-GEMM launches and improves GEMM efficiency, but adds strided KV loads and holds KV for all layers in memory at once.

Result: slower. 953.6 (-1.4%).

```diff
diff --git a/include/lara_featvol.h b/include/lara_featvol.h
--- a/include/lara_featvol.h
+++ b/include/lara_featvol.h
@@ -17,6 +17,7 @@
     int32_t img_w, img_h;
     float eps;
     int64_t x_stride[4];
+    int32_t ld_tokens;
 } lara_featvol_dims;
 
 int64_t lara_featvol_workspace_bytes(const lara_featvol_dims *d);
diff --git a/include/lara_groupattn.h b/include/lara_groupattn.h
--- a/include/lara_groupattn.h
+++ b/include/lara_groupattn.h
@@ -26,6 +26,8 @@
     const float *ln3_w, *ln3_b;
     const uint16_t *wconv;
     float eps;
+    const uint16_t *kv;
+    int32_t ldkv, ldc;
 } lara_groupblock_weights;
 
 int64_t lara_groupblock_workspace_bytes(int32_t scenes, int32_t R);
diff --git a/lara_amd/_native.py b/lara_amd/_native.py
--- a/lara_amd/_native.py
+++ b/lara_amd/_native.py
@@ -27,8 +27,8 @@
 Subset = _struct("Subset", (_vp, "coarse_state"), (_i64, "coarse_state_stride coarse_capacity"),
                  (_i32, "coarse_P coarse_forward_only"), (_vp, "inv"))
 GradLayout = _struct("GradLayout", (_i64, "means3D means2D shs colors opacities scales rotations transmat total"))
-FeatvolDims = _struct("FeatvolDims", (_i32, "B V C E h w R img_w img_h"), (_f32, "eps"), (_i64 * 4, "x_stride"))
-BlockWeights = _struct("BlockWeights", (_vp, _BLOCK_FIELDS), (_f32, "eps"))
+FeatvolDims = _struct("FeatvolDims", (_i32, "B V C E h w R img_w img_h"), (_f32, "eps"), (_i64 * 4, "x_stride"), (_i32, "ld_tokens"))
+BlockWeights = _struct("BlockWeights", (_vp, _BLOCK_FIELDS), (_f32, "eps"), (_vp, "kv"), (_i32, "ldkv ldc"))
 BlockWeightsT = _struct("BlockWeightsT", (_vp, "wq_t wkv_t wo_t w1_t w2_t wconv_t"))
 BlockGrads = _struct("BlockGrads", (_vp, _BLOCK_FIELDS))
 ImageView = _struct("ImageView", (_vp, "p"), (_i64, "sN sC sY sV sX"), (_i32, "Wv"))
diff --git a/lara_amd/csrc/attention.hip b/lara_amd/csrc/attention.hip
--- a/lara_amd/csrc/attention.hip
+++ b/lara_amd/csrc/attention.hip
@@ -7,6 +7,17 @@
 int64_t lara_groupattn_workspace_bytes(int32_t G) {
     if (G < 0) return LARA2DGS_E_INVALID;
     return (int64_t)G * (8 * 256 * 3 + 4 * 512) * 2 + 1024 + 262144;
+}
+
+static int groupattn_fused(int32_t G, const float *x, const float *ln_weight, const float *ln_bias, float eps, const uint16_t *wq,
+                           const uint16_t *wo, const unsigned short *kv, int32_t ldkv, float *y, void *workspace, hipStream_t s) {
+    L2D_PROF("ga_fused", s);
+    const int units = (G + 3) / 4;
+    unsigned short *wqp = (unsigned short *)workspace, *wop = wqp + 65536;
+    L2D_LAUNCH_IN_SCOPE(s, pack_weight_frag_kernel, dim3(64), dim3(256), 0, wq, wqp, wo, wop);
+    L2D_LAUNCH_IN_SCOPE(s, group_attn_fused2_kernel<false>, dim3(units), dim3(64), 0, x, ln_weight, ln_bias, eps, wqp, kv, ldkv, wop, y, G,
+                        (unsigned short *)nullptr, (unsigned short *)nullptr, (unsigned short *)nullptr);
+    return LARA2DGS_OK;
 }
 
 int lara_groupattn_forward(int32_t G, int32_t cond_dim, const float *x, const uint16_t *cond_bf16,
@@ -25,15 +36,16 @@
         p.A = cond_bf16; p.W = wkv; p.C = kvf; p.M = G * 4; p.N = 512; p.K = cond_dim;
         L2D_HIP(launch_gemm_ring<0, 0>(p, s));
     }
-    {
-        L2D_PROF("ga_fused", s);
-        const int units = (G + 3) / 4;
-        unsigned short *wqp = (unsigned short *)workspace, *wop = wqp + 65536;
-        L2D_LAUNCH_IN_SCOPE(s, pack_weight_frag_kernel, dim3(64), dim3(256), 0, wq, wqp, wo, wop);
-        L2D_LAUNCH_IN_SCOPE(s, group_attn_fused2_kernel<false>, dim3(units), dim3(64), 0, x, ln_weight, ln_bias, eps, wqp, kvf, wop, y, G,
-                            (unsigned short *)nullptr, (unsigned short *)nullptr, (unsigned short *)nullptr);
-    }
-    return LARA2DGS_OK;
+    return groupattn_fused(G, x, ln_weight, ln_bias, eps, wq, wo, kvf, 512, y, workspace, s);
 }
 
 }
+
+int l2d_groupattn_forward_kv(int32_t G, const float *x, const float *ln_weight, const float *ln_bias, float eps,
+                             const uint16_t *wq, const uint16_t *wo, const uint16_t *kv, int32_t ldkv, float *y,
+                             void *workspace, void *stream) {
+    if (G < 0 || ldkv < 512 || (ldkv & 7)) return LARA2DGS_E_INVALID;
+    if (G == 0) return LARA2DGS_OK;
+    if (!x || !ln_weight || !ln_bias || !wq || !wo || !kv || !y || !workspace) return LARA2DGS_E_INVALID;
+    return groupattn_fused(G, x, ln_weight, ln_bias, eps, wq, wo, kv, ldkv, y, workspace, (hipStream_t)stream);
+}
diff --git a/lara_amd/csrc/encoder.hip b/lara_amd/csrc/encoder.hip
--- a/lara_amd/csrc/encoder.hip
+++ b/lara_amd/csrc/encoder.hip
@@ -43,16 +43,52 @@
     }
 }
 
+__global__ void __launch_bounds__(256)
+cond_tokens_kernel(const float *__restrict__ src, unsigned short *__restrict__ dst, const int V, const int C, const int S, const int ld) {
+    __shared__ float t[64][65];
+    const int tx = threadIdx.x & 63, ty = threadIdx.x >> 6;
+    const int c0 = blockIdx.x * 64, r0 = blockIdx.y * 64, rows = V * C;
+    const size_t base = (size_t)blockIdx.z * rows * S, obase = (size_t)blockIdx.z * S * V * ld;
+#pragma unroll 4
+    for (int k = 0; k < 16; k++) {
+        const int r = r0 + ty * 16 + k, c = c0 + tx;
+        t[ty * 16 + k][tx] = (r < rows && c < S) ? src[base + (size_t)r * S + c] : 0.f;
+    }
+    __syncthreads();
+    const int r = r0 + tx, v = r / C, ch = r - v * C;
+#pragma unroll 4
+    for (int k = 0; k < 16; k++) {
+        const int c = c0 + ty * 16 + k;
+        if (c < S && r < rows) dst[obase + ((size_t)c * V + v) * ld + ch] = f2bf(t[tx][ty * 16 + k]);
+    }
+    if (blockIdx.y == 0) {
+        const int pad = ld - C, per = V * pad;
+        for (int i = threadIdx.x; i < 64 * per; i += 256) {
+            const int c = c0 + i / per, rem = i % per, pv = rem / pad, e = rem - pv * pad;
+            if (c < S) dst[obase + ((size_t)c * V + pv) * ld + C + e] = 0;
+        }
+    }
 }
+
+}
+
+int l2d_groupattn_forward_kv(int32_t G, const float *x, const float *ln_weight, const float *ln_bias, float eps,
+                             const uint16_t *wq, const uint16_t *wo, const uint16_t *kv, int32_t ldkv, float *y,
+                             void *workspace, void *stream);
 
 extern "C" {
 
 int lara_batched_transpose(int32_t batch, int32_t rows, int32_t cols, const float *src, void *dst, int32_t dst_bf16,
                            void *stream) {
     if (batch < 0 || rows < 0 || cols < 0 || batch > 65535 || (rows + 63) / 64 > 65535) return LARA2DGS_E_INVALID;
+    if (dst_bf16 < 0 || (dst_bf16 > 1 && ((rows & 3) || dst_bf16 < rows / 4))) return LARA2DGS_E_INVALID;
     if (batch == 0 || rows == 0 || cols == 0) return LARA2DGS_OK;
     if (!src || !dst) return LARA2DGS_E_INVALID;
     const dim3 grid((cols + 63) / 64, (rows + 63) / 64, batch);
+    if (dst_bf16 > 1) {
+        L2D_LAUNCH_IN_SCOPE((hipStream_t)stream, cond_tokens_kernel, grid, dim3(256), 0, src, (unsigned short *)dst, 4, rows / 4, cols, dst_bf16);
+        return LARA2DGS_OK;
+    }
     if (dst_bf16) L2D_LAUNCH_IN_SCOPE((hipStream_t)stream, batched_transpose_kernel<true>, grid, dim3(256), 0, src, dst, rows, cols);
     else L2D_LAUNCH_IN_SCOPE((hipStream_t)stream, batched_transpose_kernel<false>, grid, dim3(256), 0, src, dst, rows, cols);
     return LARA2DGS_OK;
@@ -64,20 +100,24 @@
     return M * 256 * 2 * 4 + M * 8 + 512 + 1024 + 262144;
 }
 
-int lara_groupblock_forward(int32_t scenes, int32_t R, int32_t cond_dim, float *x,
-                            const uint16_t *cond_bf16, const lara_groupblock_weights *w,
-                            void *workspace, void *stream) {
+int lara_groupblock_forward(int32_t scenes, int32_t R, int32_t cond_dim, float *x, const uint16_t *cond_bf16,
+                            const lara_groupblock_weights *w, void *workspace, void *stream) {
     if (scenes < 0 || R <= 0 || (R & 1) || cond_dim <= 0 || (cond_dim % 32) != 0 || !w) return LARA2DGS_E_INVALID;
+    const uint16_t *kv = w->kv;
+    const int32_t ldkv = w->ldkv;
+    if (kv && (ldkv < 512 || (ldkv & 7))) return LARA2DGS_E_INVALID;
     if (scenes == 0) return LARA2DGS_OK;
-    if (!x || !cond_bf16 || !workspace || !w->ln1_w || !w->ln1_b || !w->wq || !w->wkv || !w->wo || !w->ln2_w ||
+    if (!x || !workspace || !w->ln1_w || !w->ln1_b || !w->wq || !w->wo || !w->ln2_w ||
         !w->ln2_b || !w->w1 || !w->b1 || !w->w2 || !w->b2 || !w->ln3_w || !w->ln3_b || !w->wconv)
         return LARA2DGS_E_INVALID;
+    if (!kv && (!cond_bf16 || !w->wkv)) return LARA2DGS_E_INVALID;
     const int64_t M64 = (int64_t)scenes * R * R * R;
     if (M64 * 2056 + 512 >= (1ll << 32)) return LARA2DGS_E_INVALID;
     const int M = (int)M64, G = M / 8;
     hipStream_t s = (hipStream_t)stream;
-    int rc = lara_groupattn_forward(G, cond_dim, x, cond_bf16, w->ln1_w, w->ln1_b, w->eps, w->wq, w->wkv, w->wo,
-                                    x, workspace, stream);
+    int rc = kv ? l2d_groupattn_forward_kv(G, x, w->ln1_w, w->ln1_b, w->eps, w->wq, w->wo, kv, ldkv, x, workspace, stream)
+                : lara_groupattn_forward(G, cond_dim, x, cond_bf16, w->ln1_w, w->ln1_b, w->eps, w->wq, w->wkv, w->wo,
+                                         x, workspace, stream);
     if (rc) return rc;
     unsigned short *xn = (unsigned short *)workspace;
     float2 *stats = (float2 *)((char *)workspace + (size_t)M * 256 * 2 * 4);
diff --git a/lara_amd/csrc/encoder_bwd.hip b/lara_amd/csrc/encoder_bwd.hip
--- a/lara_amd/csrc/encoder_bwd.hip
+++ b/lara_amd/csrc/encoder_bwd.hip
@@ -766,7 +766,8 @@
 __global__ void __launch_bounds__(256)
 group_attn_bwd_kernel(const unsigned short *__restrict__ Q, const unsigned short *__restrict__ KV,
                       const unsigned short *__restrict__ dO, unsigned short *__restrict__ dQ,
-                      unsigned short *__restrict__ dKV, const int G, const int lddkv ) {
+                      unsigned short *__restrict__ dKV, const int G, const int ldkv ,
+                      const int lddkv ) {
     __shared__ __attribute__((aligned(16))) unsigned short s_q[2][8 * 256], s_do[2][8 * 256], s_kv[2][4 * 512], s_dq[2][8 * 256];
     __shared__ float s_p[2][16 * 8 * 4], s_ds[2][16 * 8 * 4];
     const int gl = threadIdx.x >> 7, t = threadIdx.x & 127;
@@ -774,10 +775,10 @@
     const bool active = g < G;
     if (active) {
         const uint4 *gq = (const uint4 *)(Q + (size_t)g * 8 * 256), *gd = (const uint4 *)(dO + (size_t)g * 8 * 256);
-        const uint4 *gk = (const uint4 *)(KV + (size_t)g * 4 * 512);
+        const unsigned short *gk = KV + ((size_t)g * 4 + (t >> 6)) * ldkv + (t & 63) * 8;
         ((uint4 *)s_q[gl])[t] = gq[t]; ((uint4 *)s_q[gl])[t + 128] = gq[t + 128];
         ((uint4 *)s_do[gl])[t] = gd[t]; ((uint4 *)s_do[gl])[t + 128] = gd[t + 128];
-        ((uint4 *)s_kv[gl])[t] = gk[t]; ((uint4 *)s_kv[gl])[t + 128] = gk[t + 128];
+        ((uint4 *)s_kv[gl])[t] = *(const uint4 *)gk; ((uint4 *)s_kv[gl])[t + 128] = *(const uint4 *)(gk + 2 * (size_t)ldkv);
     }
     __syncthreads();
     if (active) {
@@ -1075,12 +1076,12 @@
 struct SaveWs {
     size_t xn1, q, kv, o, x1, xn2, z, h, x2, xn3, stats, wpack, total;
 };
-SaveWs save_layout(int64_t M) {
+SaveWs save_layout(int64_t M, bool with_kv = true) {
     SaveWs w{};
     size_t o = 0;
     auto take = [&](size_t bytes) { const size_t at = o; o = up256(o + bytes); return at; };
     const size_t b256 = (size_t)M * 512, f256 = (size_t)M * 1024, b512 = (size_t)M * 1024;
-    w.xn1 = take(b256); w.q = take(b256); w.kv = take(b256); w.o = take(b256);
+    w.xn1 = take(b256); w.q = take(b256); w.kv = take(with_kv ? b256 : 0); w.o = take(b256);
     w.x1 = take(f256); w.xn2 = take(b256); w.z = take(b512); w.h = take(b512); w.x2 = take(f256);
     w.xn3 = take(b256 + 512);
     w.stats = take((size_t)M * 8);
@@ -1109,22 +1110,24 @@
 }
 
 int block_forward_keep(int M, int cond_dim, const float *x_in, const unsigned short *cond_bf16,
-                       const lara_groupblock_weights *w, char *save, hipStream_t s) {
-    const SaveWs L = save_layout(M);
+                       const lara_groupblock_weights *w, char *save, const unsigned short *kv_ext, int ldkv, hipStream_t s) {
+    const SaveWs L = save_layout(M, !kv_ext);
     const int G = M / 8, Mkv = G * 4;
-    unsigned short *xn1 = (unsigned short *)(save + L.xn1), *q = (unsigned short *)(save + L.q), *kv = (unsigned short *)(save + L.kv);
+    unsigned short *xn1 = (unsigned short *)(save + L.xn1), *q = (unsigned short *)(save + L.q);
+    const unsigned short *kv = kv_ext ? kv_ext : (const unsigned short *)(save + L.kv);
+    if (!kv_ext) ldkv = 512;
     unsigned short *o = (unsigned short *)(save + L.o), *xn2 = (unsigned short *)(save + L.xn2), *z = (unsigned short *)(save + L.z);
     unsigned short *h = (unsigned short *)(save + L.h), *xn3 = (unsigned short *)(save + L.xn3);
     float *x1 = (float *)(save + L.x1), *x2 = (float *)(save + L.x2);
-    {
+    if (!kv_ext) {
         GemmP p{};
-        p.A = cond_bf16; p.W = w->wkv; p.C = kv; p.M = Mkv; p.N = 512; p.K = cond_dim;
+        p.A = cond_bf16; p.W = w->wkv; p.C = save + L.kv; p.M = Mkv; p.N = 512; p.K = cond_dim;
         L2D_HIP(launch_gemm_ring<0, 0>(p, s));
     }
     {
         unsigned short *wqp = (unsigned short *)(save + L.wpack), *wop = wqp + 65536;
         L2D_LAUNCH_IN_SCOPE(s, pack_weight_frag_kernel, dim3(64), dim3(256), 0, w->wq, wqp, w->wo, wop);
-        L2D_LAUNCH_IN_SCOPE(s, group_attn_fused2_kernel<true>, dim3((G + 3) / 4), dim3(64), 0, x_in, w->ln1_w, w->ln1_b, w->eps, wqp, kv, wop,
+        L2D_LAUNCH_IN_SCOPE(s, group_attn_fused2_kernel<true>, dim3((G + 3) / 4), dim3(64), 0, x_in, w->ln1_w, w->ln1_b, w->eps, wqp, kv, ldkv, wop,
                             x1, G, xn1, q, o);
     }
     {
@@ -1167,17 +1170,20 @@
                                   const uint16_t *cond_bf16, const lara_groupblock_weights *w, void *saved,
                                   void *stream) {
     if (scenes < 0 || R < 4 || (R & 1) || cond_dim <= 0 || (cond_dim % 32) != 0 || !block_weights_ok(w)) return LARA2DGS_E_INVALID;
+    const uint16_t *kv = w->kv;
+    const int32_t ldkv = w->ldkv;
+    if (kv && (ldkv < 512 || (ldkv & 7))) return LARA2DGS_E_INVALID;
     if (scenes == 0) return LARA2DGS_OK;
-    if (!x_in || !x_out || x_in == x_out || !cond_bf16 || !saved) return LARA2DGS_E_INVALID;
+    if (!x_in || !x_out || x_in == x_out || (!cond_bf16 && !kv) || !saved) return LARA2DGS_E_INVALID;
     const int64_t M64 = (int64_t)scenes * R * R * R;
     if (M64 * 2056 + 512 >= (1ll << 32)) return LARA2DGS_E_INVALID;
     const int M = (int)M64;
     hipStream_t s = (hipStream_t)stream;
-    const SaveWs L = save_layout(M);
+    const SaveWs L = save_layout(M, !kv);
     char *save = (char *)saved;
     {
         L2D_PROF("gbt_forward", s);
-        L2D_TRY(block_forward_keep(M, cond_dim, x_in, cond_bf16, w, save, s));
+        L2D_TRY(block_forward_keep(M, cond_dim, x_in, cond_bf16, w, save, kv, ldkv, s));
     }
     {
         L2D_PROF("gb_conv3d", s);
@@ -1197,6 +1203,10 @@
                              void *workspace, void *stream) {
     if (scenes < 0 || R < 4 || (R & 1) || cond_dim <= 0 || (cond_dim % 32) != 0 || !block_weights_ok(w) || !wt || !dw)
         return LARA2DGS_E_INVALID;
+    const uint16_t *kv_ext = w->kv;
+    const int32_t ldkv = w->ldkv, ldc = (kv_ext && w->ldc) ? w->ldc : cond_dim;
+    if (ldc < cond_dim || (ldc & 7)) return LARA2DGS_E_INVALID;
+    if (kv_ext && (ldkv < 512 || (ldkv & 7))) return LARA2DGS_E_INVALID;
     if (scenes == 0) return LARA2DGS_OK;
     if (!x_in || !cond_bf16 || !g || (!dcond && !dkv_ext) || !workspace) return LARA2DGS_E_INVALID;
     if (dkv_ext && (lddkv < 512 || (lddkv & 7))) return LARA2DGS_E_INVALID;
@@ -1211,15 +1221,16 @@
     const int M = (int)M64, G = M / 8, Mkv = G * 4;
     hipStream_t s = (hipStream_t)stream;
     const BwdWs L = bwd_layout(M);
-    const SaveWs S = save_layout(M);
+    const SaveWs S = save_layout(M, !kv_ext);
     char *ws = (char *)workspace;
     if (!saved) {
         L2D_PROF("gbb_recompute", s);
-        L2D_TRY(block_forward_keep(M, cond_dim, x_in, cond_bf16, w, ws + L.save, s));
+        L2D_TRY(block_forward_keep(M, cond_dim, x_in, cond_bf16, w, ws + L.save, kv_ext, ldkv, s));
     }
     const char *sv = saved ? (const char *)saved : ws + L.save;
     const unsigned short *xn1 = (const unsigned short *)(sv + S.xn1), *q = (const unsigned short *)(sv + S.q);
-    const unsigned short *kv = (const unsigned short *)(sv + S.kv), *o = (const unsigned short *)(sv + S.o);
+    const unsigned short *kv = kv_ext ? kv_ext : (const unsigned short *)(sv + S.kv), *o = (const unsigned short *)(sv + S.o);
+    const int ld_kv = kv_ext ? ldkv : 512;
     const unsigned short *xn2 = (const unsigned short *)(sv + S.xn2), *h = (const unsigned short *)(sv + S.h);
     const unsigned short *xn3 = (const unsigned short *)(sv + S.xn3);
     unsigned short *z = (unsigned short *)(sv + S.z);
@@ -1271,7 +1282,7 @@
     {
         L2D_PROF("gbb_dx_attn", s);
         L2D_TRY(gemm_nt<0>(gb2, wt->wo_t, dob, M, 256, 256, nullptr, s));
-        L2D_LAUNCH_IN_SCOPE(s, group_attn_bwd_kernel, dim3((G + 1) / 2), dim3(256), 0, q, kv, dob, dq, dkv, G, ld_dkv);
+        L2D_LAUNCH_IN_SCOPE(s, group_attn_bwd_kernel, dim3((G + 1) / 2), dim3(256), 0, q, kv, dob, dq, dkv, G, ld_kv, ld_dkv);
         if (!dkv_ext) L2D_TRY(gemm_nt<1>(dkv, wt->wkv_t, dcond, Mkv, cond_dim, 512, dcond, s));
         L2D_TRY(gemm_nt<0>(dq, wt->wq_t, tmpb, M, 256, 256, nullptr, s));
     }
@@ -1286,7 +1297,7 @@
                                {dzb, 512, 512, xn2, 256, 256, M, dw->w1},
                                {gb2, 256, 256, o, 256, 256, M, dw->wo},
                                {dq, 256, 256, xn1, 256, 256, M, dw->wq},
-                               {dkv, ld_dkv, 512, cond_bf16, cond_dim, cond_dim, Mkv, dw->wkv}};
+                               {dkv, ld_dkv, 512, cond_bf16, ldc, cond_dim, Mkv, dw->wkv}};
         L2D_TRY(gemm_tn_group(jobs, 5, tnpart, s));
     }
     return LARA2DGS_OK;
@@ -1362,7 +1373,7 @@
     if (G < 0) return LARA2DGS_E_INVALID;
     if (G == 0) return LARA2DGS_OK;
     if (!q || !kv || !d_o || !dq || !dkv) return LARA2DGS_E_INVALID;
-    L2D_LAUNCH_IN_SCOPE((hipStream_t)stream, group_attn_bwd_kernel, dim3((G + 1) / 2), dim3(256), 0, q, kv, d_o, dq, dkv, G, 512);
+    L2D_LAUNCH_IN_SCOPE((hipStream_t)stream, group_attn_bwd_kernel, dim3((G + 1) / 2), dim3(256), 0, q, kv, d_o, dq, dkv, G, 512, 512);
     return LARA2DGS_OK;
 }
 
diff --git a/lara_amd/csrc/featvol.hip b/lara_amd/csrc/featvol.hip
--- a/lara_amd/csrc/featvol.hip
+++ b/lara_amd/csrc/featvol.hip
@@ -175,7 +175,7 @@
 }
 
 template <bool TOKENS>
-__global__ void __launch_bounds__(256) sample_kernel(const FvP p, const float *__restrict__ y, void *__restrict__ out) {
+__global__ void __launch_bounds__(256) sample_kernel(const FvP p, const float *__restrict__ y, void *__restrict__ out, const int ld) {
     __shared__ int s_idx[8][FV_PTS][4];
     __shared__ float s_wgt[8][FV_PTS][4];
     __shared__ float s_tile[TOKENS ? 1 : 256][FV_PTS + 1];
@@ -210,7 +210,7 @@
                     a.x += wg * g.x; a.y += wg * g.y; a.z += wg * g.z; a.w += wg * g.w;
                 }
                 if (TOKENS) {
-                    unsigned short *o = (unsigned short *)out + ((size_t)(b * p.S + s0 + pt) * p.V + v) * CE + c;
+                    unsigned short *o = (unsigned short *)out + ((size_t)(b * p.S + s0 + pt) * p.V + v) * ld + c;
                     *(uint2 *)o = make_uint2(f2bf2(a.x, a.y), f2bf2(a.z, a.w));
                 } else {
                     const int cl = 4 * lane;
@@ -228,11 +228,13 @@
                 __syncthreads();
             }
         }
-        for (int i = threadIdx.x; i < p.E * FV_PTS; i += 256) {
+        const int tail = TOKENS ? ld - p.C : p.E;
+        for (int i = threadIdx.x; i < tail * FV_PTS; i += 256) {
             if (TOKENS) {
-                const int pt = i / p.E, e = i - pt * p.E;
+                const int pt = i / tail, e = i - pt * tail;
                 if (pt < npts)
-                    ((unsigned short *)out)[((size_t)(b * p.S + s0 + pt) * p.V + v) * CE + p.C + e] = f2bf(p.embed[v * p.E + e]);
+                    ((unsigned short *)out)[((size_t)(b * p.S + s0 + pt) * p.V + v) * ld + p.C + e] =
+                        e < p.E ? f2bf(p.embed[v * p.E + e]) : (unsigned short)0;
             } else {
                 const int e = i / FV_PTS, pt = i - e * FV_PTS;
                 if (pt < npts) ((float *)out)[((size_t)(b * p.V + v) * CE + p.C + e) * p.S + s0 + pt] = p.embed[v * p.E + e];
@@ -505,6 +507,8 @@
                          const float *grid, const float *ln_w, const float *ln_b, const float *mlp_w, const float *mlp_b,
                          const float *view_embed, int32_t layout, void *out, void *workspace, void *stream) {
     if (!dims_ok(d) || (layout != LARA_FEATVOL_VOLUME && layout != LARA_FEATVOL_TOKENS)) return LARA2DGS_E_INVALID;
+    const int32_t ld_tokens = d->ld_tokens ? d->ld_tokens : d->C + d->E;
+    if (layout == LARA_FEATVOL_TOKENS ? (ld_tokens < d->C + d->E || (ld_tokens & 3)) : ld_tokens != d->C + d->E) return LARA2DGS_E_INVALID;
     if (!img_feats || !rays || !w2cs || !ixts || !grid || !ln_w || !ln_b || !mlp_w || !mlp_b || !out || !workspace) return LARA2DGS_E_INVALID;
     if (d->E > 0 && !view_embed) return LARA2DGS_E_INVALID;
     hipStream_t s = (hipStream_t)stream;
@@ -526,8 +530,8 @@
     {
         L2D_PROF(layout == LARA_FEATVOL_TOKENS ? "featvol_sample_tokens" : "featvol_sample_volume", s);
         const dim3 grid2((p.S + FV_PTS - 1) / FV_PTS, p.B);
-        if (layout == LARA_FEATVOL_TOKENS) L2D_LAUNCH_IN_SCOPE(s, sample_kernel<true>, grid2, dim3(256), 0, p, (const float *)y, out);
-        else L2D_LAUNCH_IN_SCOPE(s, sample_kernel<false>, grid2, dim3(256), 0, p, (const float *)y, out);
+        if (layout == LARA_FEATVOL_TOKENS) L2D_LAUNCH_IN_SCOPE(s, sample_kernel<true>, grid2, dim3(256), 0, p, (const float *)y, out, (int)ld_tokens);
+        else L2D_LAUNCH_IN_SCOPE(s, sample_kernel<false>, grid2, dim3(256), 0, p, (const float *)y, out, (int)ld_tokens);
     }
     return LARA2DGS_OK;
 }
diff --git a/lara_amd/csrc/group_attn.h b/lara_amd/csrc/group_attn.h
--- a/lara_amd/csrc/group_attn.h
+++ b/lara_amd/csrc/group_attn.h
@@ -29,8 +29,8 @@
 __global__ void __launch_bounds__(64)
 group_attn_fused2_kernel(const float *x , const float *__restrict__ gamma,
                         const float *__restrict__ beta, const float eps, const unsigned short *__restrict__ Wq ,
-                        const unsigned short *__restrict__ KV, const unsigned short *__restrict__ Wo , float *y, const int G,
-                        unsigned short *__restrict__ xn_out, unsigned short *__restrict__ q_out, unsigned short *__restrict__ o_out) {
+                        const unsigned short *__restrict__ KV, const int ldkv ,
+                        const unsigned short *__restrict__ Wo , float *y, const int G, unsigned short *__restrict__ xn_out, unsigned short *__restrict__ q_out, unsigned short *__restrict__ o_out) {
     constexpr int GA_LDS = 24576;
     __shared__ __attribute__((aligned(16))) unsigned char lds_all[GA_LDS];
     const int lane = threadIdx.x & 63;
@@ -72,7 +72,7 @@
 #pragma unroll
     for (int i = 0; i < 4; i++) {
         const int row = 4 * i + srow, chunk = sphys ^ (row & 15);
-        const unsigned short *src = KV + (size_t)(g0 * 4 + min(row, kv_rows - 1)) * 512 + chunk * 8;
+        const unsigned short *src = KV + (size_t)(g0 * 4 + min(row, kv_rows - 1)) * ldkv + chunk * 8;
         __builtin_amdgcn_global_load_lds((const __attribute__((address_space(1))) void *)src,
                                          (__attribute__((address_space(3))) void *)(KVr + i * 1024), 16, 0, 0);
         __builtin_amdgcn_global_load_lds((const __attribute__((address_space(1))) void *)(src + 256),
@@ -118,7 +118,7 @@
 #pragma unroll
     for (int i = 0; i < 4; i++) {
         const int row = 4 * i + srow, chunk = sphys ^ (row & 15);
-        const unsigned short *src = KV + (size_t)(g0 * 4 + min(row, kv_rows - 1)) * 512 + 128 + chunk * 8;
+        const unsigned short *src = KV + (size_t)(g0 * 4 + min(row, kv_rows - 1)) * ldkv + 128 + chunk * 8;
         pk[i] = *(const uint4 *)src;
         pv[i] = *(const uint4 *)(src + 256);
     }
diff --git a/lara_amd/csrc/mfma_gemm.h b/lara_amd/csrc/mfma_gemm.h
--- a/lara_amd/csrc/mfma_gemm.h
+++ b/lara_amd/csrc/mfma_gemm.h
@@ -37,6 +37,9 @@
     const float *resid;
     const float *bias;
     int M, N, K;
+    int lda;
+    int cblk, ldc;
+    size_t cstride;
     int R, Cin;
     const float2 *stats;
     const float *gamma, *beta;
@@ -227,6 +230,9 @@
     const int r = lane & 31, kh = lane >> 5;
     float *ep = (float *)ring + wave * (32 * 68);
     unsigned long long *rowbase = (unsigned long long *)((float *)ring + 8 * (32 * 68)) + wave * 32;
+    const int cb = (EPI == 0 && p.cblk) ? bn0 / p.cblk : 0;
+    unsigned short *const ctile = (unsigned short *)p.C + (size_t)cb * p.cstride + (bn0 - cb * p.cblk);
+    const size_t crow = (EPI == 0 && p.cblk) ? (size_t)p.ldc : (size_t)N;
 #pragma unroll
     for (int i = 0; i < 4; i++) {
         __syncthreads();
@@ -246,8 +252,16 @@
         for (int q = 0; q < 8; q++) {
             const int idx = q * 64 + lane, lr = idx >> 4, c4 = (idx & 15) * 4;
             const int row = bm0 + wr * 128 + i * 32 + lr, col = bn0 + wc * 64 + c4;
-            if (row < M && col < N)
-                gemm_epilogue<EPI>(p, *(const float4 *)(ep + lr * 68 + c4), row, col, N, EPI == 5 ? rowbase[lr] : 0ull);
+            if (row < M && col < N) {
+                if (EPI == 0) {
+                    const float4 v = *(const float4 *)(ep + lr * 68 + c4);
+                    ushort4 h;
+                    h.x = f2bf(v.x); h.y = f2bf(v.y); h.z = f2bf(v.z); h.w = f2bf(v.w);
+                    *(ushort4 *)(ctile + (size_t)row * crow + (wc * 64 + c4)) = h;
+                } else {
+                    gemm_epilogue<EPI>(p, *(const float4 *)(ep + lr * 68 + c4), row, col, N, EPI == 5 ? rowbase[lr] : 0ull);
+                }
+            }
         }
     }
 }
@@ -364,7 +378,7 @@
             noff[q] = chunk * 16;
         } else {
             vb[q] = vd[q] = vh[q] = vw[q] = 0;
-            noff[q] = (uint32_t)min(bm0 + srow[q], M - 1) * (uint32_t)(K * 2) + chunk * 16;
+            noff[q] = (uint32_t)min(bm0 + srow[q], M - 1) * (uint32_t)((p.lda ? p.lda : K) * 2) + chunk * 16;
         }
     }
     const int ktiles = K / 32, kpt = AMODE ? Cin / 32 : 1;
@@ -498,7 +512,7 @@
             noff[q] = chunk * 16;
         } else {
             vb[q] = vd[q] = vh[q] = vw[q] = 0;
-            noff[q] = (uint32_t)min(bm0 + srow[q], M - 1) * (uint32_t)(K * 2) + chunk * 16;
+            noff[q] = (uint32_t)min(bm0 + srow[q], M - 1) * (uint32_t)((p.lda ? p.lda : K) * 2) + chunk * 16;
         }
     }
     auto set_tap = [&](const int tap) {
diff --git a/lara_amd/encoder.py b/lara_amd/encoder.py
--- a/lara_amd/encoder.py
+++ b/lara_amd/encoder.py
@@ -30,12 +30,17 @@
     return out
 
 
-def cond_tokens(image_feats: torch.Tensor, n_group: int) -> torch.Tensor:
+def cond_tokens(image_feats: torch.Tensor, n_group: int, ld: int = None) -> torch.Tensor:
     B, V, C, D = image_feats.shape[:4]
     if D != n_group or V != 4:
         raise RuntimeError("kernels are specialised for one image-feature voxel per group and 4 input views "
                            "(configs/base.yaml: n_groups [16], 16^3 feature volume, n_views 4)")
-    return image_feats.permute(0, 3, 4, 5, 1, 2).reshape(B * D ** 3, V, C).to(torch.bfloat16).contiguous()
+    rows = image_feats.permute(0, 3, 4, 5, 1, 2).reshape(B * D ** 3, V, C)
+    if ld is None or ld == C:
+        return rows.to(torch.bfloat16).contiguous()
+    out = torch.zeros(B * D ** 3, V, ld, dtype=torch.bfloat16, device=image_feats.device)
+    out[:, :, :C] = rows
+    return out
 
 
 class GroupAttBlock(nn.Module):
@@ -126,6 +131,17 @@
         self._pos_tokens = None
         self._ws = None
         self._graphs = {}
+        self._wkv_all = self._wkv_key = None
+        self._kv_all = None
+
+    def _wkv_operand(self, dev) -> torch.Tensor:
+        key = tuple((layer.wkv.data_ptr(), layer.wkv._version) for layer in self.layers) + (dev,)
+        if self._wkv_key != key:
+            C = self.layers[0].cond_dim
+            w = torch.zeros(len(self.layers) * 512, (C + 127) // 128 * 128, dtype=torch.bfloat16, device=dev)
+            w[:, :C] = torch.cat([layer.wkv for layer in self.layers], 0)
+            self._wkv_all, self._wkv_key, self._graphs = w, key, {}
+        return self._wkv_all
 
     @classmethod
     def from_reference(cls, vt) -> "VolTransformer":
@@ -143,9 +159,14 @@
 
     def _run(self, cond: torch.Tensor, x: torch.Tensor, out: torch.Tensor, B: int) -> None:
         R, dev = self.vol_low_res, cond.device
+        L, ld = len(self.layers), cond.shape[-1]
+        rows = cond.shape[0] * cond.shape[1]
+        call("lara_gemm_nt_bf16", dev, rows, L * 512, ld, cond, self._wkv_all, self._kv_all, 0)
         x.view(B, -1, self.embed_dim).copy_(self._pos_tokens)
-        for layer in self.layers:
-            layer.forward_tokens(x, cond, B, R)
+        for l, layer in enumerate(self.layers):
+            w = layer._weights()
+            w.kv, w.ldkv = self._kv_all.data_ptr() + l * 1024, L * 512
+            call("lara_groupblock_forward", dev, B, R, layer.cond_dim, x, None, w, self._ws)
         call("lara_voltrans_head_forward", dev, B, R, x, self.norm_w, self.norm_b, float(self.eps), self.wdeconv, self.deconv_b,
              self.out_dim, out, self._ws)
 
@@ -153,16 +174,21 @@
         _require_device(image_feats)
         B, R = image_feats.shape[0], self.vol_low_res
         dev = image_feats.device
-        cond = cond_tokens(image_feats, self.n_groups[0])
+        wkv_all = self._wkv_operand(dev)
+        cond = cond_tokens(image_feats, self.n_groups[0], wkv_all.shape[1])
         pos_key = (self.pos_embed.data_ptr(), self.pos_embed._version, dev)
         if self._pos_tokens is None or getattr(self, "_pos_key", None) != pos_key:
             with torch.no_grad():
                 self._pos_tokens = volume_to_tokens(self.pos_embed.detach().to(dev))
             self._pos_key = pos_key
             self._graphs = {}
-        need = B * R ** 3 * 512
+        need = max(B * R ** 3 * 512, query("lara_groupblock_workspace_bytes", B, R))
         if self._ws is None or self._ws.numel() < need or self._ws.device != dev:
             self._ws = torch.empty(need, dtype=torch.uint8, device=dev)
+            self._graphs = {}
+        kv_need = cond.shape[0] * cond.shape[1] * len(self.layers) * 512
+        if self._kv_all is None or self._kv_all.numel() < kv_need or self._kv_all.device != dev:
+            self._kv_all = torch.empty(kv_need, dtype=torch.bfloat16, device=dev)
             self._graphs = {}
         if not use_graph:
             x = torch.empty(B * R ** 3, self.embed_dim, dtype=torch.float32, device=dev)
diff --git a/lara_amd/encoder_train.py b/lara_amd/encoder_train.py
--- a/lara_amd/encoder_train.py
+++ b/lara_amd/encoder_train.py
@@ -5,8 +5,8 @@
 import torch
 from torch import nn
 
-from ._native import (BlockGrads as _BlockGrads, BlockWeights as _BlockWeights, BlockWeightsT as _BlockWeightsT, call, query,
-                      require_device)
+from ._native import (BlockGrads as _BlockGrads, BlockWeights as _BlockWeights, BlockWeightsT as _BlockWeightsT, call, host_array,
+                      query, require_device)
 from ._native import current_stream as _stream, load_library as _lib
 from .encoder import tokens_to_volume, volume_to_tokens
 
@@ -59,6 +59,46 @@
     return f
 
 
+def _padded(cond_dim: int) -> int:
+    return (cond_dim + 127) // 128 * 128
+
+
+def _wkv_all(layers_p, cond_dim, dev):
+    ws = [t.detach() for p in layers_p for t in (p[3], p[4])]
+    K = _padded(cond_dim)
+    key = ("wkv_all", K) + tuple((t.data_ptr(), t._version) for t in ws)
+    hit = _wcache.get(key)
+    if hit is not None:
+        return hit[1]
+    out = torch.empty(len(layers_p) * 512, K, dtype=torch.bfloat16, device=dev)
+    if ws:
+        out[:, :cond_dim].copy_(torch.cat(ws, 0))
+        out[:, cond_dim:].zero_()
+    if len(_wcache) >= 64:
+        _wcache.clear()
+    _wcache[key] = (ws, out)
+    return out
+
+
+def _kv_all(cond_bf, layers_p, cond_dim):
+    dev, K, L = cond_bf.device, cond_bf.shape[-1], len(layers_p)
+    rows = cond_bf.numel() // K
+    kv = torch.empty(rows, L * 512, dtype=torch.bfloat16, device=dev)
+    if L:
+        call("lara_gemm_nt_bf16", dev, rows, L * 512, K, cond_bf, _wkv_all(layers_p, cond_dim, dev), kv, 0)
+    return kv
+
+
+def _kv_of(kv_all, l):
+    return kv_all.data_ptr() + l * 1024, kv_all.shape[1]
+
+
+def _save_bytes(B, R, dev):
+    offs = host_array("l", 11)
+    call("lara_groupblock_save_offsets", None, B, R, offs, 11)
+    return query("lara_groupblock_save_bytes", B, R) - (offs[3] - offs[2])
+
+
 def invalidate_weight_cache():
     _wcache.clear()
 
@@ -88,8 +128,9 @@
     B, V, cond_dim = image_feats.shape[:3]
     S = image_feats.shape[3] * image_feats.shape[4] * image_feats.shape[5]
     feats = image_feats.detach().float().contiguous()
-    cond_bf = torch.empty(B * S, V, cond_dim, dtype=torch.bfloat16, device=dev)
-    call("lara_batched_transpose", dev, B, V * cond_dim, S, feats, cond_bf, 1)
+    ldc = _padded(cond_dim)
+    cond_bf = torch.empty(B * S, V, ldc, dtype=torch.bfloat16, device=dev)
+    call("lara_batched_transpose", dev, B, V * cond_dim, S, feats, cond_bf, ldc if ldc > cond_dim else 1)
     return _inference_from_cond(cond_bf, B, cond_dim, eps_block, eps_final, R, out_dim, pos_embed, norm_w, norm_b, deconv_w, deconv_b,
                                 *layer_params)
 
@@ -102,11 +143,14 @@
     x = volume_to_tokens(pos_embed.detach().float()).repeat(B, 1)
     ws = _workspace(dev, "fwd", query("lara_groupblock_workspace_bytes", B, R))
     with torch.cuda.device(dev):
+        layers_p = [[t.detach() for t in layer_params[l * _NLP:(l + 1) * _NLP]] for l in range(n_layers)]
+        kv_all = _kv_all(cond_bf, layers_p, cond_dim)
         for l in range(n_layers):
-            f = _layer_bf16([t.detach() for t in layer_params[l * _NLP:(l + 1) * _NLP]])
+            f = _layer_bf16(layers_p[l])
             w = _fill(_BlockWeights(), f, _GRAD_FIELDS)
             w.eps = eps_block
-            call("lara_groupblock_forward", dev, B, R, cond_dim, x, cond_bf, w, ws)
+            w.kv, w.ldkv = _kv_of(kv_all, l)
+            call("lara_groupblock_forward", dev, B, R, cond_dim, x, None, w, ws)
         wd = deconv_w.detach().permute(2, 3, 4, 1, 0).reshape(8 * out_dim, 256).to(torch.bfloat16).contiguous()
         nw, nb, db = norm_w.detach().float().contiguous(), norm_b.detach().float().contiguous(), deconv_b.detach().float().contiguous()
         out = torch.empty(B, 2 * R, 2 * R, 2 * R, out_dim, dtype=torch.float32, device=dev)
@@ -123,7 +167,9 @@
 
     def __init__(self, B, R, cond_dim, n_layers, eps_block, dev):
         self.B, self.R, self.cond_dim, self.n_layers, self.eps_block, self.dev = B, R, cond_dim, n_layers, eps_block, dev
+        self.ldc = _padded(cond_dim)
         self.cond_bf = None
+        self.kv_all = None
         self.fs = [None] * n_layers
         self.dkv_all = None
         self.flat = None
@@ -151,8 +197,8 @@
         B, V, C = image_feats.shape[:3]
         S = image_feats.shape[3] * image_feats.shape[4] * image_feats.shape[5]
         feats = image_feats.detach().float().contiguous()
-        cond_bf = torch.empty(B * S, V, C, dtype=torch.bfloat16, device=dev)
-        call("lara_batched_transpose", dev, B, V * C, S, feats, cond_bf, 1)
+        cond_bf = torch.empty(B * S, V, sweep.ldc, dtype=torch.bfloat16, device=dev)
+        call("lara_batched_transpose", dev, B, V * C, S, feats, cond_bf, sweep.ldc if sweep.ldc > C else 1)
         sweep.cond_bf = cond_bf
         ctx.sweep, ctx.feat_shape, ctx.feat_dtype = sweep, tuple(image_feats.shape), image_feats.dtype
         return torch.zeros(1, dtype=torch.float32, device=dev)
@@ -163,8 +209,7 @@
         if not ctx.needs_input_grad[0]:
             return None, None
         dev = sw.dev
-        cond_bf = sw.cond_bf
-        dcond = torch.empty(cond_bf.shape, dtype=torch.float32, device=dev)
+        dcond = torch.empty(sw.cond_bf.shape[:2] + (sw.cond_dim,), dtype=torch.float32, device=dev)
         lddkv = sw.n_layers * 512
         with torch.cuda.device(dev):
             wkv_all_t = torch.cat([f["wkv"] for f in sw.fs], 0).t().contiguous()
@@ -183,7 +228,7 @@
     def forward(ctx, img_feats, ln_w, ln_b, mlp_w, mlp_b, embed, prep, sweep):
         from .featvol import TOKENS
         prep.params(ln_w, ln_b, mlp_w, mlp_b, embed)
-        sweep.cond_bf = prep.forward(TOKENS)
+        sweep.cond_bf = prep.forward(TOKENS, sweep.ldc)
         ctx.sweep, ctx.prep = sweep, prep
         return torch.zeros(1, dtype=torch.float32, device=img_feats.device)
 
@@ -194,7 +239,7 @@
         if not any(ctx.needs_input_grad[:6]):
             return (None,) * 8
         dev = sw.dev
-        dcond = torch.empty(sw.cond_bf.shape, dtype=torch.float32, device=dev)
+        dcond = torch.empty(sw.cond_bf.shape[:2] + (sw.cond_dim,), dtype=torch.float32, device=dev)
         lddkv = sw.n_layers * 512
         with torch.cuda.device(dev):
             wkv_all_t = torch.cat([f["wkv"] for f in sw.fs], 0).t().contiguous()
@@ -224,16 +269,17 @@
         w = _fill(_BlockWeights(), f, _GRAD_FIELDS)
         w.eps = sw.eps_block
         keep = _keep_activations()
+        w.kv, w.ldkv = _kv_of(sw.kv_all, l)
         with torch.cuda.device(dev):
             if keep:
-                act = torch.empty(query("lara_groupblock_save_bytes", sw.B, sw.R), dtype=torch.uint8, device=dev)
+                act = torch.empty(_save_bytes(sw.B, sw.R, dev), dtype=torch.uint8, device=dev)
                 x_out = torch.empty_like(x)
                 call("lara_groupblock_forward_train", dev, sw.B, sw.R, sw.cond_dim, x, x_out, sw.cond_bf, w, act)
             else:
                 act = None
                 x_out = x.clone()
                 ws = _workspace(dev, "fwd", query("lara_groupblock_workspace_bytes", sw.B, sw.R))
-                call("lara_groupblock_forward", dev, sw.B, sw.R, sw.cond_dim, x_out, sw.cond_bf, w, ws)
+                call("lara_groupblock_forward", dev, sw.B, sw.R, sw.cond_dim, x_out, None, w, ws)
         ctx.save_for_backward(x)
         ctx.sweep, ctx.l, ctx.act = sw, l, act
         return x_out
@@ -247,6 +293,7 @@
         ft = _layer_bf16_t(f)
         w = _fill(_BlockWeights(), f, _GRAD_FIELDS)
         w.eps = sw.eps_block
+        (w.kv, w.ldkv), w.ldc = _kv_of(sw.kv_all, l), sw.ldc
         wt = _fill(_BlockWeightsT(), ft, ("wq_t", "wkv_t", "wo_t", "w1_t", "w2_t", "wconv_t"))
         lddkv = sw.n_layers * 512
         if sw.dkv_all is None:
@@ -317,8 +364,11 @@
 def _sweep_from(module, sweep, token):
     B, R = sweep.B, module.vol_low_res
     x = _StartFn.apply(module.pos_embed, token, B, R)
-    for l, layer in enumerate(module.layers):
-        x = _BlockFn.apply(x, sweep, l, *layer.flat_params())
+    layers_p = [layer.flat_params() for layer in module.layers]
+    with torch.cuda.device(sweep.dev):
+        sweep.kv_all = _kv_all(sweep.cond_bf, layers_p, sweep.cond_dim)
+    for l, p in enumerate(layers_p):
+        x = _BlockFn.apply(x, sweep, l, *p)
     return _HeadFn.apply(x, module.norm.weight, module.norm.bias, module.deconv.weight, module.deconv.bias, sweep,
                          float(module.norm.eps), module.out_dim)
 
@@ -387,6 +437,6 @@
         from .featvol import TOKENS
         prep.params(*args)
         flat = [p for layer in self.layers for p in layer.flat_params()]
-        return _inference_from_cond(prep.forward(TOKENS), B, C, float(self.layers[0].norm1.eps), float(self.norm.eps), self.vol_low_res,
+        return _inference_from_cond(prep.forward(TOKENS, _padded(C)), B, C, float(self.layers[0].norm1.eps), float(self.norm.eps), self.vol_low_res,
                                     self.out_dim, self.pos_embed, self.norm.weight, self.norm.bias, self.deconv.weight,
                                     self.deconv.bias, *flat)
diff --git a/lara_amd/featvol.py b/lara_amd/featvol.py
--- a/lara_amd/featvol.py
+++ b/lara_amd/featvol.py
@@ -67,11 +67,14 @@
     def _inputs(self):
         return (self.x, self.rays, self.w2c, self.ixt, self.grid) + self.p[:4]
 
-    def forward(self, layout):
+    def forward(self, layout, ld=None):
         CE, R = self.C + self.E, self.d.R
+        ld = CE if ld is None else ld
         out = (torch.empty(self.B, self.V, CE, R, R, R, dtype=torch.float32, device=self.dev) if layout == VOLUME else
-               torch.empty(self.B * self.S, self.V, CE, dtype=torch.bfloat16, device=self.dev))
+               torch.empty(self.B * self.S, self.V, ld, dtype=torch.bfloat16, device=self.dev))
+        self.d.ld_tokens = ld if layout == TOKENS else 0
         call("lara_featvol_forward", self.dev, self.d, *self._inputs(), self.p[4], layout, out, self._ws())
+        self.d.ld_tokens = 0
         return out
 
     def backward(self, grad, layout, want_embed=True):
```
